# rojas-diego/tokengeex

Hardware: AMD Instinct MI355X
Metric: MB/s raw bytes encoded (and tokens/s) at 32K/64K vocab, 1/2/4/8 GPUs (higher is better)
Workload: dtype f64

## Files before the change

tokengeex_amd/_lib.py:

```python
from __future__ import annotations

import ctypes as C
import os

import numpy as np

_HERE = os.path.dirname(os.path.abspath(__file__))
LIB_PATH = os.path.join(_HERE, "libtgx.so")

OK, ERR_IO, ERR_JSON, ERR_TOKEN_ID_OOB, ERR_NO_PATH, ERR_DEVICE, ERR_Z_NOT_NORMAL, ERR_INVALID, \
    ERR_UNSUPPORTED = range(9)
MAX_TOKEN_LEN = 64
MAX_NBEST = 16
ESTEP_SNIPPET_LEN = 81920
NO_ID = 0xFFFFFFFF
LAYOUT_PAD_LEFT, LAYOUT_TRUNC_LEFT, LAYOUT_I64 = 1, 2, 4
FRONT_CRLF = 1
SPAN_CHARS = 8
SELECT_ROWS_DEVICE = 1

_vp, _u64, _u32, _i, _d = C.c_void_p, C.c_uint64, C.c_uint32, C.c_int, C.c_double
_pvp, _pu64 = C.POINTER(C.c_void_p), C.POINTER(C.c_uint64)
SYMBOLS = {
    "tgx_last_error": (C.c_char_p, []),
# ... 40 lines not shown
    "tgx_count_pairs_top": (_i, [_vp, _vp, _u64, _pvp, _pvp, _pu64, _pu64]),
    "tgx_estep": (_i, [_vp, _vp, _u64, _d, _u64, _vp, C.POINTER(C.c_double)]),
    "tgx_split_specials": (_i, [_vp, _vp, _u64, _vp, _vp, _u32, _vp, _pvp, _pvp, _pvp, _pu64]),
    "tgx_pack_segments": (_i, [_vp, _vp, _vp, _vp, _u64, _i, _vp, _vp, _pu64]),
    "tgx_normalize_segments": (_i, [_u32, _vp, _vp, _vp, _u64, _pvp, _pvp]),
    "tgx_unidata_version": (C.c_char_p, []),
    "tgx_assemble_ids": (_i, [_vp, _vp, _u64, _vp, _vp, _u32, _vp, _vp]),
    "tgx_decode_batch": (_i, [_vp, _vp, _u32, _vp, _vp, _u32, _vp, _vp, _u64, _i, _pvp, _vp, _pu64, _pu64]),
    "tgx_utf8_lossy": (_u64, [_vp, _u64, _vp]),
    "tgx_substring_df": (_i, [_i, _vp, _u64, _vp, _vp, _vp, _vp, _u64, _u32, _d, _u64, _pvp, _pvp, _pvp, _pu64, _pu64, _pu64]),
    "tgx_substring_df_top": (_i, [_i, _vp, _u64, _vp, _vp, _vp, _vp, _u64, _u32, _d, _u64, _u64, _pvp, _pvp, _pvp, _pu64, _pu64, _pu64,
                                  _pu64, C.POINTER(C.c_uint32)]),
    "tgx_generate_u01": (_d, [_u64, _u64, _u64]),
    "tgx_free": (None, [_vp]),
    "tgx_pool_trim": (None, [_i]),
    "tgx_pool_filled_bytes": (_u64, []),
    "tgx_host_alloc": (_vp, [_u64]),
    "tgx_host_free": (None, [_vp]),
    "tgx_digamma": (_d, [_d]),
    "tgx_prune_m_step": (_i, [_vp, _vp, _u32, _vp, _vp, C.POINTER(C.c_uint32)]),
    "tgx_prune_alternatives": (_i, [_vp, _vp, _vp, _vp, _u32, _vp, _vp, _pvp]),
    "tgx_model_prune_alternatives": (_i, [_vp, _vp, _vp, _pvp]),
    "tgx_prune_select": (_i, [_vp, _vp, _vp, _vp, _vp, _vp, _u32, _u64, _u32, _vp, C.POINTER(C.c_uint32)]),
    "tgx_last_kernel_times": (_i, [_vp, C.POINTER(C.c_char_p), C.POINTER(C.c_float), _i]),
    "tgx_last_algorithmic_bytes": (_u64, [_vp]),
    "tgx_last_encode_waves_per_cu": (_u32, [_vp]),
    "tgx_last_encode_redo_samples": (_u64, [_vp]),
    "tgx_model_score_values": (_u32, [_vp]),
    "tgx_last_encode_hot_values": (_u32, [_vp]),
    "tgx_last_encode_lean_items": (_u32, [_vp]),
    "tgx_last_encode_ids_in_place": (_i, [_vp]),
    "tgx_last_encode_top_table": (_i, [_vp]),
    "tgx_last_encode_long_samples": (_u64, [_vp]),
    "tgx_last_estep_pieces": (_u64, [_vp]),
    "tgx_last_estep_redo": (_u64, [_vp]),
    "tgx_last_encode_corun_cus": (_u32, [_vp]),
    "tgx_encode_corun_timeouts": (_u32, [_vp]),
    "tgx_sample_u01": (_d, [_u64, _u64, _u64, _u32]),
    "tgx_encode_batch_sample": (_i, [_vp, _vp, _vp, _u64, _d, _u64, _vp, _pvp]),
    "tgx_encode_corpus_sample": (_i, [_vp, _vp, _d, _u64, _vp, _pvp]),
    "tgx_lattice_stats_corpus": (_i, [_vp, _vp, _d, _vp, _vp, _vp, _pu64]),
    "tgx_lattice_stats_batch": (_i, [_vp, _vp, _vp, _u64, _d, _vp, _vp, _vp, _pu64]),
    "tgx_lattice_stats_host": (_i, [_vp, _vp, _vp, _u32, _vp, _vp, _u64, _d, _vp, _vp, _vp, _pu64]),
    "tgx_encode_batch_nbest": (_i, [_vp, _vp, _vp, _u64, _u32, _vp, _vp, _pvp]),
    "tgx_encode_corpus_nbest": (_i, [_vp, _vp, _u32, _vp, _vp, _pvp]),
    "tgx_result_device": (_i, [_vp]),
    "tgx_result_layout_info": (_i, [_vp, _u32, _u32, _pu64, _pu64]),
    "tgx_result_pad_device": (_i, [_vp, _u32, _u32, _u32, _u32, _u32, _vp, _vp, _vp, _vp, _pu64]),
    "tgx_result_pack_device": (_i, [_vp, _u32, _u32, _u32, _u32, _u32, _vp, _vp, _vp, _vp, _pu64]),
    "tgx_layout_pad_host": (_i, [_vp, _vp, _u64, _u32, _u32, _u32, _u32, _u32, _vp, _vp, _vp, _pu64]),
    "tgx_layout_pack_host": (_i, [_vp, _vp, _u64, _u32, _u32, _u32, _u32, _u32, _vp, _vp, _vp, _pu64]),
    "tgx_assemble_result": (_i, [_vp, _vp, _vp, _vp, _u64, _u32, _pvp]),
    "tgx_result_vocab_size": (_u32, [_vp]),
    "tgx_assemble_host": (_i, [_vp, _vp, _u64, _vp, _vp, _u64, _u32, _u32, _vp, _u64, _vp]),
    "tgx_decode_result": (_i, [_vp, _vp, _vp, _vp, _u32, _i, _vp, _pvp, _pu64, _pu64]),
    "tgx_decode_padded": (_i, [_vp, _vp, _u64, _u64, _u32, _vp, _vp, _u32, _vp, _vp, _u32, _i, _vp, _pvp, _pu64, _pu64]),
    "tgx_text_num_rows": (_u64, [_vp]),
    "tgx_text_num_bytes": (_u64, [_vp]),
    "tgx_text_num_replaced": (_u64, [_vp]),
    "tgx_text_device": (_i, [_vp]),
    "tgx_text_copy_bytes": (_i, [_vp, _vp, _u64]),
    "tgx_text_copy_offsets": (_i, [_vp, _vp, _u64]),
    "tgx_text_bytes_device": (_vp, [_vp]),
    "tgx_text_offsets_device": (_vp, [_vp]),
    "tgx_text_free": (None, [_vp]),
    "tgx_corpus_from_text": (_i, [_vp, _pvp]),
    "tgx_decode_rows_host": (_i, [_vp, _vp, _u32, _vp, _vp, _u32, _vp, _u32, _vp, _u64, _u64, _vp, _vp, _u32, _i, _pvp, _vp, _pu64,
                                  _pu64, _pu64]),
    "tgx_result_spans_device": (_i, [_vp, _vp, _vp, _vp, _u32, _u32, _vp, _vp]),
    "tgx_result_pad_spans_device": (_i, [_vp, _vp, _vp, _vp, _u32, _u32, _u32, _u32, _u32, _vp, _vp]),
    "tgx_spans_host": (_i, [_vp, _vp, _u32, _vp, _vp, _u32, _vp, _vp, _u64, _u32, _u32, _u32, _u32, _vp]),
    "tgx_result_window_info": (_i, [_vp, _u32, _u32, _u32, _u32, _u32, _pu64]),
    "tgx_result_window_pad_device": (_i, [_vp, _u32, _u32, _u32, _u32, _u32, _u32, _vp, _u64, _vp, _vp, _vp, _vp, _vp]),
    "tgx_result_window_spans_device": (_i, [_vp, _vp, _vp, _vp, _u32, _u32, _u32, _u32, _u32, _u32, _vp, _u64, _vp]),
    "tgx_layout_windows_host": (_i, [_vp, _vp, _u64, _u32, _u32, _u32, _u32, _u32, _u32, _u64, _vp, _vp, _vp, _vp, _vp, _pu64]),
    "tgx_window_spans_host": (_i, [_vp, _vp, _u32, _vp, _vp, _u32, _vp, _vp, _u64, _u32, _u32, _u32, _u32, _u32, _u64, _vp, _pu64]),
    "tgx_corpus_split_specials": (_i, [_vp, _vp, _vp, _u32, _u32, _pvp, _pvp]),
    "tgx_plan_num_samples": (_u64, [_vp]),
    "tgx_plan_num_segments": (_u64, [_vp]),
    "tgx_plan_num_encoded": (_u64, [_vp]),
    "tgx_plan_device": (_i, [_vp]),
    "tgx_plan_copy": (_i, [_vp, _vp, _u64, _vp, _u64]),
    "tgx_plan_free": (None, [_vp]),
    "tgx_assemble_result_plan": (_i, [_vp, _vp, _vp, _u32, _pvp]),
    "tgx_front_last_times": (_i, [C.POINTER(C.c_char_p), C.POINTER(C.c_float), _i]),
    "tgx_corpus_copy_text": (_i, [_vp, _vp, _u64]),
    "tgx_corpus_copy_offsets": (_i, [_vp, _vp, _u64]),
    "tgx_front_host": (_i, [_vp, _vp, _u64, _vp, _vp, _u32, _u32, _vp, _pvp, _pu64, _pvp, _pvp, _pu64]),
    "tgx_corpus_normalize": (_i, [_vp, _u32, _pvp, _pu64]),
    "tgx_normalize_host": (_i, [_u32, _vp, _vp, _u64, _pvp, _pvp, _pu64]),
    "tgx_norm_last_times": (_i, [C.POINTER(C.c_char_p), C.POINTER(C.c_float), _i]),
    "tgx_fim_u01": (_d, [_u64, _u64, _u64]),
    "tgx_result_fim": (_i, [_vp, _u32, _u32, _u32, _d, _d, _u64, _u64, _vp, _vp, _vp, _pu64, _pvp]),
    "tgx_fim_host": (_i, [_vp, _vp, _u64, _u32, _u32, _u32, _u32, _d, _d, _u64, _u64, _vp, _u64, _vp, _vp, _vp, _pu64]),
    "tgx_result_from_ids": (_i, [_i, _vp, _vp, _u64, _u32, _pvp]),
    "tgx_fim_last_times": (_i, [C.POINTER(C.c_char_p), C.POINTER(C.c_float), _i]),
    "tgx_select_last_times": (_i, [C.POINTER(C.c_char_p), C.POINTER(C.c_float), _i]),
    "tgx_result_select": (_i, [_vp, _vp, _u64, _u32, _vp, _pvp]),
    "tgx_result_lengths_device": (_i, [_vp, _vp, _vp]),
    "tgx_corpus_select": (_i, [_vp, _vp, _u64, _u32, _vp, _pvp]),
    "tgx_shuffle_key": (_u64, [_u64, _u64]),
    "tgx_shuffled_rows_device": (_i, [_i, _u64, _u64, _vp, _vp]),
    "tgx_shuffled_rows_host": (_i, [_u64, _u64, _vp]),
    "tgx_select_host": (_i, [_vp, _vp, _u64, _vp, _u64, _vp, _u64, _vp]),
    "tgx_select_text_host": (_i, [_vp, _vp, _u64, _vp, _u64, _vp, _u64, _vp]),
    "tgx_corpus_first_equal_device": (_i, [_vp, _u32, _vp, _vp, C.POINTER(C.c_uint64)]),
    "tgx_result_first_equal_device": (_i, [_vp, _u32, _vp, _vp, C.POINTER(C.c_uint64)]),
    "tgx_row_hash": (_u64, [_vp, _u64, _u64]),
    "tgx_corpus_row_hashes_device": (_i, [_vp, _u64, _vp, _vp]),
    "tgx_result_row_hashes_device": (_i, [_vp, _u64, _vp, _vp]),
    "tgx_first_equal_host": (_i, [_vp, _u32, _vp, _u64, _u32, _vp, C.POINTER(C.c_uint64), C.POINTER(C.c_uint32)]),
    "tgx_dedup_last_times": (_i, [C.POINTER(C.c_char_p), C.POINTER(C.c_float), _i]),
    "tgx_dedup_last_rounds": (_u32, []),
    "tgx_result_minhash_device": (_i, [_vp, _u32, _u32, _u64, _u32, _vp, _vp]),
    "tgx_corpus_minhash_device": (_i, [_vp, _u32, _u32, _u64, _u32, _vp, _vp]),
    "tgx_minhash_value": (_u32, [_u64, _u32, _u64]),
    "tgx_minhash_bands_device": (_i, [_i, _vp, _u64, _u32, _u32, _u64, _vp, _vp, _vp]),
    "tgx_minhash_near_first_device": (_i, [_i, _vp, _u64, _u32, _vp, _u32, _u32, _vp, _vp, C.POINTER(C.c_uint64)]),
    "tgx_minhash_host": (_i, [_vp, _u32, _vp, _u64, _u32, _u32, _u64, _vp]),
    "tgx_minhash_bands_host": (_i, [_vp, _u64, _u32, _u32, _u64, _vp, _vp]),
    "tgx_minhash_near_first_host": (_i, [_vp, _u64, _u32, _vp, _u32, _u32, _vp, C.POINTER(C.c_uint64)]),
    "tgx_minhash_last_times": (_i, [C.POINTER(C.c_char_p), C.POINTER(C.c_float), _i]),
    "tgx_gram_key": (_u64, [_vp, _u64, _u64]),
    "tgx_result_gramset_create": (_i, [_vp, _u32, _u64, _u32, _vp, _vp]),
    "tgx_corpus_gramset_create": (_i, [_vp, _u32, _u64, _u32, _vp, _vp]),
    "tgx_gramset_create_from_keys": (_i, [_i, _vp, _u64, _u32, _u32, _u64, _vp]),
    "tgx_gramset_size": (_u64, [_vp]),
    "tgx_gramset_info": (_i, [_vp, C.POINTER(C.c_uint32), C.POINTER(C.c_uint32), C.POINTER(C.c_uint64), C.POINTER(C.c_int), C.POINTER(C.c_uint32)]),
    "tgx_gramset_keys": (_i, [_vp, _vp]),
    "tgx_gramset_free": (None, [_vp]),
    "tgx_result_gram_hits_device": (_i, [_vp, _vp, _u32, _vp, _vp, _vp]),
    "tgx_corpus_gram_hits_device": (_i, [_vp, _vp, _u32, _vp, _vp, _vp]),
    "tgx_gram_keys_host": (_i, [_vp, _u32, _vp, _u64, _u32, _u64, _vp, C.POINTER(C.c_uint64)]),
    "tgx_gram_hits_host": (_i, [_vp, _u32, _vp, _u64, _u32, _u64, _vp, _u64, _vp, _vp]),
    "tgx_gram_contains_host": (_i, [_vp, _u64, _vp, _u64, _vp]),
    "tgx_gram_last_times": (_i, [C.POINTER(C.c_char_p), C.POINTER(C.c_float), _i]),
    "tgx_corpus_text_stats_device": (_i, [_vp, _u64, _u32, _vp, _vp, _vp]),
    "tgx_corpus_lines": (_i, [_vp, _u32, _vp, _vp]),
    "tgx_text_stats_host": (_i, [_vp, _vp, _u64, _u64, _u32, _vp, _vp]),
    "tgx_lines_host": (_i, [_vp, _vp, _u64, _vp, _u64, C.POINTER(C.c_uint64)]),
    "tgx_textstat_last_times": (_i, [C.POINTER(C.c_char_p), C.POINTER(C.c_float), _i]),
    "tgx_result_repeat_stats_device": (_i, [_vp, _u32, _u64, _u32, _vp, _vp, _vp]),
    "tgx_corpus_repeat_stats_device": (_i, [_vp, _u32, _u64, _u32, _vp, _vp, _vp]),
    "tgx_repeat_stats_host": (_i, [_vp, _u32, _vp, _u64, _u32, _u64, _vp, _vp]),
    "tgx_repeat_last_times": (_i, [C.POINTER(C.c_char_p), C.POINTER(C.c_float), _i]),
}

WORD_SYMBOLS = {
    "tgx_corpus_word_stats_device": (_i, [_vp, _u64, _vp, _vp, _u32, _u32, _vp, _vp, _vp]),
    "tgx_word_stats_host": (_i, [_vp, _vp, _u64, _u64, _vp, _vp, _u32, _u32, _vp, _vp]),
    "tgx_wordstat_last_times": (_i, [C.POINTER(C.c_char_p), C.POINTER(C.c_float), _i]),
}

PHRASE_SYMBOLS = {
    "tgx_phraseset_create": (_i, [_i, _vp, _vp, _u32, _u32, _u32, _vp]),
    "tgx_phraseset_info": (_i, [_vp, C.POINTER(C.c_uint32), C.POINTER(C.c_uint32), C.POINTER(C.c_uint32), C.POINTER(C.c_uint32),
                                C.POINTER(C.c_uint32), C.POINTER(C.c_int), C.POINTER(C.c_uint64)]),
    "tgx_phraseset_free": (None, [_vp]),
    "tgx_corpus_phrase_hits_device": (_i, [_vp, _vp, _u32, _vp, _vp, _vp, _vp]),
    "tgx_result_phrase_hits_device": (_i, [_vp, _vp, _u32, _vp, _vp, _vp, _vp]),
    "tgx_phrase_hits_host": (_i, [_vp, _u32, _vp, _u64, _vp, _vp, _u32, _u32, _vp, _vp, _vp]),
    "tgx_phrase_last_times": (_i, [C.POINTER(C.c_char_p), C.POINTER(C.c_float), _i]),
}


class TokenGeeXError(Exception):

    def __init__(self, message: str, status: int = -1, sample: int | None = None,
                 pos: int | None = None, length: int | None = None):
        super().__init__(message)
        self.status, self.sample, self.pos, self.length = status, sample, pos, length


def _share_torch_hip_runtime() -> None:
    import sys
    if os.environ.get("TGX_HIP_RUNTIME", "") == "system" or "torch" in sys.modules:
        return
    import importlib.util
    try:
        spec = importlib.util.find_spec("torch")
    except (ImportError, ValueError):
        return
    for root in (spec.submodule_search_locations or []) if spec else []:
        path = os.path.join(root, "lib", "libamdhip64.so")
        if os.path.exists(path):
            try:
                C.CDLL(path, mode=C.RTLD_GLOBAL)
            except OSError:
                pass
            return


def _load() -> C.CDLL:
    if not os.path.exists(LIB_PATH):
        raise ImportError(
            f"{LIB_PATH} is missing: the HIP extension is mandatory (no CPU fallback). "
            "Build it with `python tokengeex_amd/build.py`.")
    _share_torch_hip_runtime()
    lib = C.CDLL(LIB_PATH)
    for name, (res, args) in list(SYMBOLS.items()) + list(WORD_SYMBOLS.items()) + list(PHRASE_SYMBOLS.items()):
        fn = getattr(lib, name)
        fn.restype = res
        fn.argtypes = args
    if lib.tgx_abi_version() != 1:
        raise ImportError("libtgx.so ABI version mismatch")
    return lib


lib = _load()


def check(status: int) -> None:
    if status == OK:
        return
    msg = (lib.tgx_last_error() or b"").decode("utf-8", "replace")
    if status in (ERR_NO_PATH, ERR_Z_NOT_NORMAL):
        s, p, l = C.c_uint64(), C.c_uint64(), C.c_uint64()
        lib.tgx_last_error_detail(C.byref(s), C.byref(p), C.byref(l))
        raise TokenGeeXError(msg, status, s.value, p.value, l.value)
    raise TokenGeeXError(msg, status)


class _PinnedBlock:

    def __init__(self, nbytes: int):
        self.nbytes = int(nbytes)
        self.addr = lib.tgx_host_alloc(self.nbytes)
        if not self.addr:
            raise TokenGeeXError(lib.tgx_last_error().decode("utf-8", "replace"))
        self.buf = (C.c_ubyte * max(1, self.nbytes)).from_address(self.addr)

    def __del__(self):
        addr, self.addr = getattr(self, "addr", None), None
        if addr:
            lib.tgx_host_free(addr)


def pinned_empty(shape, dtype) -> np.ndarray:
    dt = np.dtype(dtype)
    n = int(np.prod(shape))
    blk = _PinnedBlock(n * dt.itemsize)
    arr = np.frombuffer(blk.buf, dtype=dt, count=n).reshape(shape)
    blk.buf._tgx_owner = blk
    return arr


def pool_trim(device: int = -1) -> None:
    lib.tgx_pool_trim(device)


def pool_filled_bytes() -> int:
    return int(lib.tgx_pool_filled_bytes())


def device_count() -> int:
    return lib.tgx_device_count()


def ptr(a: np.ndarray | None):
    return None if a is None else a.ctypes.data_as(C.c_void_p)


class Packed:

    __slots__ = ("flat", "offs")

    def __init__(self, flat: np.ndarray, offs: np.ndarray):
        self.flat, self.offs = flat, offs

    @classmethod
    def of(cls, items) -> "Packed":
        return items if isinstance(items, Packed) else cls(*pack(items))

    def __len__(self) -> int:
        return int(self.offs.shape[0]) - 1

    def take(self, idx) -> "Packed":
        idx = np.asarray(idx, dtype=np.int64)
        beg, end = self.offs[:-1][idx].astype(np.int64), self.offs[1:][idx].astype(np.int64)
        lens = end - beg
        offs = np.zeros(idx.shape[0] + 1, np.uint64)
        np.cumsum(lens, out=offs[1:])
        total = int(offs[-1])
        src = np.repeat(beg - offs[:-1].astype(np.int64), lens) + np.arange(total, dtype=np.int64)
        return Packed(self.flat[src] if total else np.zeros(0, np.uint8), offs)

    def tolist(self) -> list[bytes]:
        raw, o = self.flat.tobytes(), self.offs.tolist()
        return [raw[o[i]:o[i + 1]] for i in range(len(o) - 1)]


def pack(items) -> tuple[np.ndarray, np.ndarray]:
    if isinstance(items, Packed):
        return items.flat, items.offs
    offs = np.zeros(len(items) + 1, dtype=np.uint64)
    if len(items):
        np.cumsum(np.fromiter((len(t) for t in items), dtype=np.uint64, count=len(items)), out=offs[1:])
    flat = np.frombuffer(b"".join(items), dtype=np.uint8)
    return flat, offs


def _take(ptr_, n, ctype, dtype):
    if not ptr_ or n == 0:
        if ptr_:
            lib.tgx_free(ptr_)
        return np.zeros(0, dtype)
    a = np.ctypeslib.as_array(C.cast(ptr_, C.POINTER(ctype)), shape=(n,)).copy()
    lib.tgx_free(ptr_)
    return a


def split_specials_flat(flat: np.ndarray, offs: np.ndarray, specials: list[bytes]):
    sflat, soffs = pack(specials)
    n = offs.shape[0] - 1
    seg_offs = np.zeros(n + 1, np.uint64)
    sb, se, ss, m = C.c_void_p(), C.c_void_p(), C.c_void_p(), C.c_uint64()
    check(lib.tgx_split_specials(ptr(flat) if flat.size else None, ptr(offs), n, ptr(sflat) if sflat.size else None, ptr(soffs),
                                 len(specials), ptr(seg_offs), C.byref(sb), C.byref(se), C.byref(ss), C.byref(m)))
    k = m.value
    return seg_offs, _take(sb, k, C.c_uint64, np.uint64), _take(se, k, C.c_uint64, np.uint64), _take(ss, k, C.c_int32, np.int32)


def pack_segments(flat: np.ndarray, seg_begin: np.ndarray, seg_end: np.ndarray, seg_special, crlf: bool):
    n = seg_begin.shape[0]
    total = int((seg_end.astype(np.int64) - seg_begin.astype(np.int64)).sum()) if n else 0
    out = np.empty(max(total, 1), np.uint8)
    out_offs = np.zeros(n + 1, np.uint64)
    m = C.c_uint64()
    check(lib.tgx_pack_segments(ptr(flat) if flat.size else None, ptr(seg_begin), ptr(seg_end),
                                None if seg_special is None else ptr(seg_special), n, 1 if crlf else 0, ptr(out), ptr(out_offs),
                                C.byref(m)))
    out_offs = out_offs[: m.value + 1]
    return out[: int(out_offs[-1])], out_offs


NORMAL_FORMS = {"nfd": 0, "nfc": 1, "nfkd": 2, "nfkc": 3}


def normalize_flat(form: str, flat: np.ndarray, offs: np.ndarray):
    flat = np.ascontiguousarray(flat, dtype=np.uint8)
    offs = np.ascontiguousarray(offs, dtype=np.uint64)
    n = offs.shape[0] - 1
    beg, end = np.ascontiguousarray(offs[:-1]), np.ascontiguousarray(offs[1:])
    ot, oo = C.c_void_p(), C.c_void_p()
    check(lib.tgx_normalize_segments(NORMAL_FORMS[form], ptr(flat) if flat.size else None, ptr(beg) if n else None, ptr(end) if n else None, n,
                                     C.byref(ot), C.byref(oo)))
    out_offs = _take(oo, n + 1, C.c_uint64, np.uint64)
    return _take(ot, int(out_offs[-1]), C.c_uint8, np.uint8), out_offs


def unidata_version() -> str:
    return lib.tgx_unidata_version().decode()

# ... 1392 lines not shown

    def assemble_plan(self, segs: "NativeResult | None", plan: NativePlan, n_specials: int) -> NativeResult:
        h = C.c_void_p()
        check(lib.tgx_assemble_result_plan(self._h, None if segs is None else segs._h, plan._h, _u32_arg(n_specials, "n_specials"), C.byref(h)))
        return NativeResult(h)

    @staticmethod
    def _specials(special_flat, special_offs):
        sf = np.ascontiguousarray(special_flat, dtype=np.uint8)
        so = np.ascontiguousarray(special_offs, dtype=np.uint64)
        return sf, so, so.shape[0] - 1

    def decode_result(self, result: NativeResult, special_flat, special_offs, include_special: bool, stream: int = 0) -> "NativeText":
        sf, so, n = self._specials(special_flat, special_offs)
        h, bs, bi = C.c_void_p(), C.c_uint64(), C.c_uint64()
        st = lib.tgx_decode_result(self._h, result._h, ptr(sf) if sf.size else None, ptr(so), n, 1 if include_special else 0,
                                   stream or None, C.byref(h), C.byref(bs), C.byref(bi))
        if st != OK:
            _raise_decode(st, bs.value, bi.value)
        return NativeText(h)

    def decode_padded(self, ids_ptr: int, n_rows: int, row_len: int, i64: bool, *, mask_ptr: int = 0, lengths_ptr: int = 0,
                      skip_id: int | None = None, special_flat=(), special_offs=(0,), include_special: bool = True,
                      stream: int = 0) -> "NativeText":
        sf, so, n = self._specials(special_flat, special_offs)
        h, bs, bi = C.c_void_p(), C.c_uint64(), C.c_uint64()
        st = lib.tgx_decode_padded(self._h, ids_ptr or None, int(n_rows), int(row_len), LAYOUT_I64 if i64 else 0, mask_ptr or None,
                                   lengths_ptr or None, _id_or_none(skip_id), ptr(sf) if sf.size else None, ptr(so), n,
                                   1 if include_special else 0, stream or None, C.byref(h), C.byref(bs), C.byref(bi))
        if st != OK:
            _raise_decode(st, bs.value, bi.value)
        return NativeText(h)

    def result_spans(self, result: NativeResult, special_flat, special_offs, spans_ptr: int, *, flags: int = 0, stream: int = 0) -> None:
        sf, so, n = self._specials(special_flat, special_offs)
        check(lib.tgx_result_spans_device(self._h, result._h, ptr(sf) if sf.size else None, ptr(so), n, _u32_arg(flags, "flags"),
                                          stream or None, spans_ptr or None))

    def result_pad_spans(self, result: NativeResult, special_flat, special_offs, row_len: int, spans_ptr: int, *, bos_id: int | None = None,
                         eos_id: int | None = None, flags: int = 0, stream: int = 0) -> None:
        sf, so, n = self._specials(special_flat, special_offs)
        check(lib.tgx_result_pad_spans_device(self._h, result._h, ptr(sf) if sf.size else None, ptr(so), n, _u32_arg(row_len, "row_len"),
                                              _id_or_none(bos_id), _id_or_none(eos_id), _u32_arg(flags, "flags"), stream or None,
                                              spans_ptr or None))

    def encode_corpus_sample(self, corpus: NativeCorpus, alpha: float, seed: int, return_logz: bool = False):
        n = corpus.num_samples
        logz = np.zeros(max(n, 1), np.float64) if return_logz else None
        h = C.c_void_p()
        check(lib.tgx_encode_corpus_sample(self._h, corpus._h, float(alpha), seed & (2**64 - 1),
                                           ptr(logz) if return_logz else None, C.byref(h)))
        return (NativeResult(h), logz[:n]) if return_logz else NativeResult(h)

    def encode_batch_nbest_flat(self, flat: np.ndarray, offs: np.ndarray, nbest: int):
        flat = np.ascontiguousarray(flat, dtype=np.uint8)
        offs = np.ascontiguousarray(offs, dtype=np.uint64)
        n = offs.shape[0] - 1
        scores = np.empty(max(n * int(nbest), 1), np.float64)
        n_found = np.empty(max(n, 1), np.uint32)
        h = C.c_void_p()
        check(lib.tgx_encode_batch_nbest(self._h, ptr(flat) if flat.size else None, ptr(offs), n, int(nbest), ptr(scores),
                                         ptr(n_found), C.byref(h)))
        return NativeResult(h), scores[:n * int(nbest)], n_found[:n]

    def encode_corpus_nbest(self, corpus: NativeCorpus, nbest: int):
        n = corpus.num_samples
        scores = np.empty(max(n * int(nbest), 1), np.float64)
        n_found = np.empty(max(n, 1), np.uint32)
        h = C.c_void_p()
        check(lib.tgx_encode_corpus_nbest(self._h, corpus._h, int(nbest), ptr(scores), ptr(n_found), C.byref(h)))
        return NativeResult(h), scores[:n * int(nbest)], n_found[:n]

    def count_tokens(self, corpus: NativeCorpus, freq: np.ndarray | None = None) -> np.ndarray:
        if freq is None:
            freq = np.zeros(self.vocab_size, np.uint64)
        assert freq.dtype == np.uint64 and freq.shape[0] == self.vocab_size and freq.flags.c_contiguous
        check(lib.tgx_count_tokens(self._h, corpus._h, ptr(freq)))
        return freq

    def count_pairs(self, corpus: NativeCorpus) -> tuple[np.ndarray, np.ndarray]:
        keys, counts, n = C.c_void_p(), C.c_void_p(), C.c_uint64()
        check(lib.tgx_count_pairs(self._h, corpus._h, C.byref(keys), C.byref(counts), C.byref(n)))
        k = n.value
        ka = np.ctypeslib.as_array(C.cast(keys, C.POINTER(C.c_uint64)), shape=(max(k, 1),))[:k].copy()
        ca = np.ctypeslib.as_array(C.cast(counts, C.POINTER(C.c_uint64)), shape=(max(k, 1),))[:k].copy()
        lib.tgx_free(keys)
        lib.tgx_free(counts)
        return ka, ca

    def count_pairs_top(self, corpus: NativeCorpus, max_pairs: int) -> tuple[np.ndarray, np.ndarray, int]:
        keys, counts, n, tot = C.c_void_p(), C.c_void_p(), C.c_uint64(), C.c_uint64()
        check(lib.tgx_count_pairs_top(self._h, corpus._h, int(max_pairs), C.byref(keys), C.byref(counts),
                                      C.byref(n), C.byref(tot)))
        k = n.value
        ka = np.ctypeslib.as_array(C.cast(keys, C.POINTER(C.c_uint64)), shape=(max(k, 1),))[:k].copy()
        ca = np.ctypeslib.as_array(C.cast(counts, C.POINTER(C.c_uint64)), shape=(max(k, 1),))[:k].copy()
        lib.tgx_free(keys)
        lib.tgx_free(counts)
        return ka, ca, tot.value

    def estep(self, corpus: NativeCorpus, snippet_len: int = ESTEP_SNIPPET_LEN, dropout: float = 0.0,
              seed: int = 0, expected: np.ndarray | None = None) -> tuple[np.ndarray, float]:
        if expected is None:
            expected = np.zeros(self.vocab_size, np.float64)
        assert expected.dtype == np.float64 and expected.shape[0] == self.vocab_size
        z = C.c_double()
        check(lib.tgx_estep(self._h, corpus._h, snippet_len, float(dropout), seed & (2**64 - 1),
                            ptr(expected), C.byref(z)))
        return expected, z.value

    def common_prefix_search(self, s: bytes) -> list[tuple[int, int]]:
        buf = np.frombuffer(s, dtype=np.uint8)
        cap = len(s) + 1
        ids, lens = np.zeros(cap, np.uint32), np.zeros(cap, np.uint32)
        cnt = C.c_uint64()
        check(lib.tgx_common_prefix_search(self._h, ptr(buf) if len(s) else None, len(s), ptr(ids),
                                           ptr(lens), cap, C.byref(cnt)))
        return [(int(ids[i]), int(lens[i])) for i in range(cnt.value)]

    def last_kernel_times(self) -> dict[str, float]:
        names = (C.c_char_p * 8)()
        ms = (C.c_float * 8)()
        n = lib.tgx_last_kernel_times(self._h, names, ms, 8)
        return {names[i].decode(): float(ms[i]) for i in range(n)}

    def last_algorithmic_bytes(self) -> int:
        return lib.tgx_last_algorithmic_bytes(self._h)

    def last_encode_waves_per_cu(self) -> int:
        return lib.tgx_last_encode_waves_per_cu(self._h)

    def last_encode_redo_samples(self) -> int:
        return lib.tgx_last_encode_redo_samples(self._h)

    def score_values(self) -> int:
        return lib.tgx_model_score_values(self._h)

    def last_encode_hot_values(self) -> int:
        return lib.tgx_last_encode_hot_values(self._h)

    def last_encode_lean_items(self) -> tuple[int, int]:
        v = lib.tgx_last_encode_lean_items(self._h)
        return v & 0xFF, (v >> 8) & 0xFF

    def last_encode_lean_step(self) -> bool:
        return bool(self.last_encode_lean_items()[0] & 1)

    def last_encode_ids_in_place(self) -> bool:
        return bool(lib.tgx_last_encode_ids_in_place(self._h))

    def last_encode_top_table(self) -> bool:
        return bool(lib.tgx_last_encode_top_table(self._h))

    def last_encode_long_samples(self) -> int:
        return lib.tgx_last_encode_long_samples(self._h)

    def last_estep_pieces(self) -> int:
        return lib.tgx_last_estep_pieces(self._h)

    def last_estep_redo(self) -> int:
        return lib.tgx_last_estep_redo(self._h)

    def last_encode_corun_cus(self) -> int:
        return lib.tgx_last_encode_corun_cus(self._h)

    def encode_corun_timeouts(self) -> int:
        return lib.tgx_encode_corun_timeouts(self._h)


class FlatTrie:

    def __init__(self, tokens: list[bytes], scores):
        flat, offs = pack(tokens)
        sc = np.ascontiguousarray(scores, dtype=np.float64)
        h = C.c_void_p()
        check(lib.tgx_flat_trie_build(ptr(flat) if flat.size else None, ptr(offs), ptr(sc), len(tokens),
                                      C.byref(h)))
        self._h = h
        self._flat, self._offs, self._sc = flat, offs, sc

    def common_prefix_search8(self, s: bytes, max_hot: int = 6600):
        buf = np.frombuffer(s, dtype=np.uint8)
        cap = len(s) + 1
        ids, lens = np.zeros(cap, np.uint32), np.zeros(cap, np.uint32)
        nh, nc, cov = C.c_uint32(), C.c_uint64(), C.c_double()
        k = lib.tgx_flat_trie_search8(self._h, ptr(self._flat) if self._flat.size else None, ptr(self._offs), ptr(self._sc),
                                      max_hot, ptr(buf) if len(s) else None, len(s), ptr(ids), ptr(lens), cap,
                                      C.byref(nh), C.byref(nc), C.byref(cov))
        if k == 2**64 - 1:
            raise TokenGeeXError("8-byte records need fewer than 2^23 slots")
        return [(int(ids[i]), int(lens[i])) for i in range(k)], {"n_hot": nh.value, "n_cold": nc.value, "hot_coverage": cov.value}

    def __del__(self):
        if getattr(self, "_h", None):
            lib.tgx_flat_trie_free(self._h)
            self._h = None

    def common_prefix_search(self, s: bytes) -> list[tuple[int, int]]:
        buf = np.frombuffer(s, dtype=np.uint8)
        cap = len(s) + 1
        ids, lens = np.zeros(cap, np.uint32), np.zeros(cap, np.uint32)
        k = lib.tgx_flat_trie_search(self._h, ptr(buf) if len(s) else None, len(s), ptr(ids), ptr(lens), cap)
        return [(int(ids[i]), int(lens[i])) for i in range(k)]

    def stats(self) -> dict:
        a, b, c = C.c_uint64(), C.c_uint64(), C.c_uint32()
        lib.tgx_flat_trie_stats(self._h, C.byref(a), C.byref(b), C.byref(c))
        return {"n_slots": a.value, "n_nodes": b.value, "max_token_len": c.value,
                "fill": b.value / max(1, a.value)}

    @property
    def max_token_len(self) -> int:
        return self.stats()["max_token_len"]

    def table(self):
        n = self.stats()["n_slots"]
        check, base, tokid = np.zeros(n, np.uint32), np.zeros(n, np.uint32), np.zeros(n, np.uint32)
        lib.tgx_flat_trie_copy(self._h, ptr(check), ptr(base), ptr(tokid))
        return check, base, tokid


    def prune_alternatives(self, tokens: list[bytes], scores) -> tuple[np.ndarray, np.ndarray, np.ndarray]:
        flat, offs = pack(tokens)
        sc = np.ascontiguousarray(scores, dtype=np.float64)
        V = len(tokens)
        always_keep = np.zeros(V, np.uint8)
        alt_offs = np.zeros(V + 1, np.uint32)
        p = C.c_void_p()
        check(lib.tgx_prune_alternatives(self._h, ptr(flat) if flat.size else None, ptr(offs), ptr(sc), V,
                                         ptr(always_keep), ptr(alt_offs), C.byref(p)))
        k = int(alt_offs[V])
        ids = np.ctypeslib.as_array(C.cast(p, C.POINTER(C.c_uint32)), shape=(max(k, 1),))[:k].copy()
        lib.tgx_free(p)
        return always_keep, alt_offs, ids


def tok_hash_selftest(tokens: list[bytes]) -> tuple[int, int]:
    flat, offs = pack(tokens)
    seed, bad = C.c_uint32(), C.c_uint64()
    check(lib.tgx_tok_hash_selftest(ptr(flat) if flat.size else None, ptr(offs), len(tokens), C.byref(seed), C.byref(bad)))
    return seed.value, bad.value


def digamma(x: float) -> float:
    return lib.tgx_digamma(x)


def prune_m_step(expected: np.ndarray, keep: np.ndarray) -> tuple[np.ndarray, np.ndarray]:
    expected = np.ascontiguousarray(expected, dtype=np.float64)
    keep = np.ascontiguousarray(keep, dtype=np.uint8)
    V = expected.shape[0]
    idx, sc, n = np.zeros(max(V, 1), np.uint32), np.zeros(max(V, 1), np.float64), C.c_uint32()
    check(lib.tgx_prune_m_step(ptr(expected), ptr(keep), V, ptr(idx), ptr(sc), C.byref(n)))
    return idx[:n.value].copy(), sc[:n.value].copy()


def prune_select(freq, keep, always_keep, alt_offs, alt_ids, scores, n_samples: int,
                 pruned_size: int) -> np.ndarray:
    freq = np.ascontiguousarray(freq, dtype=np.uint64)
    keep = np.ascontiguousarray(keep, dtype=np.uint8)
    always_keep = np.ascontiguousarray(always_keep, dtype=np.uint8)
    alt_offs = np.ascontiguousarray(alt_offs, dtype=np.uint32)
    alt_ids = np.ascontiguousarray(alt_ids, dtype=np.uint32)
    scores = np.ascontiguousarray(scores, dtype=np.float64)
    V = freq.shape[0]
    out, n = np.zeros(max(V, 1), np.uint32), C.c_uint32()
    check(lib.tgx_prune_select(ptr(freq), ptr(keep), ptr(always_keep), ptr(alt_offs),
                               ptr(alt_ids) if alt_ids.size else None, ptr(scores), V, n_samples,
                               pruned_size, ptr(out), C.byref(n)))
    return out[:n.value].copy()


def dropout_u01(seed: int, sample: int, pos: int, length: int) -> float:
    return lib.tgx_dropout_u01_host(seed, sample, pos, length)


def sample_u01(seed: int, sample: int, pos: int, length: int) -> float:
    return lib.tgx_sample_u01(seed, sample, pos, length)


def sample_u01_array(seed: int, sample: np.ndarray, pos: np.ndarray, length: np.ndarray) -> np.ndarray:
    with np.errstate(over="ignore"):
        x = (np.uint64(seed & (2**64 - 1)) ^ np.uint64(0xD6E8FEB86659FD93)
             ^ (np.asarray(sample, np.uint64) * np.uint64(0x9E3779B97F4A7C15))
             ^ (np.asarray(pos, np.uint64) * np.uint64(0xC2B2AE3D27D4EB4F))
             ^ (np.asarray(length, np.uint64) * np.uint64(0x165667B19E3779F9)))
        x ^= x >> np.uint64(30)
        x *= np.uint64(0xBF58476D1CE4E5B9)
        x ^= x >> np.uint64(27)
        x *= np.uint64(0x94D049BB133111EB)
        x ^= x >> np.uint64(31)
    u = ((x >> np.uint64(11)).astype(np.float64) + 0.5) * (1.0 / 9007199254740992.0)
    return np.minimum(u, np.nextafter(1.0, 0.0))
```

tokengeex_amd/build.py:

```python
from __future__ import annotations

import os
import shutil
import subprocess
import sys

HERE = os.path.dirname(os.path.abspath(__file__))
CSRC = os.path.join(HERE, "csrc")
OUT = os.path.join(HERE, "libtgx.so")
SOURCES = ["kernels.hip", "estep.hip", "encode2.hip", "encode4l.hip", "encode5.hip", "estep4.hip", "estep4l.hip", "estep7.hip", "cuts.hip", "pairs.hip", "generate.hip", "sample.hip", "stats.hip", "nbest.hip", "layout.hip", "assemble.hip", "fim.hip", "select.hip", "dedup.hip", "minhash.hip", "gram.hip", "repeat.hip", "textstat.hip", "wordstat.hip", "phrase.hip", "decode.hip", "spans.hip", "front.hip", "norm.hip", "tgx_api.cpp", "encode_pass.cpp", "estep_pass.cpp", "lattice_pass.cpp", "result_ops.cpp", "corpus_ops.cpp", "minhash_ops.cpp", "gram_ops.cpp", "repeat_ops.cpp", "textstat_ops.cpp", "wordstat_ops.cpp", "phrase_ops.cpp", "host_twins.cpp", "trie_build.cpp", "prune_host.cpp", "frontback.cpp", "unicode_norm.cpp"]
HEADERS = ["api_internal.h", "device_internal.h", "pass_internal.h", "kernels.h", "sample.h", "stats.h", "nbest.h", "layout.h", "assemble.h", "fim.h", "select.h", "dedup.h", "minhash.h", "gram.h", "gram_walk.h", "repeat.h", "shingle_load.h", "textstat.h", "textstat_walk.h", "wordstat.h", "phrase.h", "decode.h", "spans.h", "front.h", "norm.h", "device_common.h", "lattice_walk.h", "tile_fill.h", "scan_helpers.h", "lean_gate.h", "ids_in_place.h", "encode_split.h", "encode5_layout.h", "top_table.h", "trace_body.h", "trie_build.h", "unicode_tables.h", os.path.join("..", "..", "include", "tgx.h"), os.path.join("..", "..", "include", "tgx_words.h"), os.path.join("..", "..", "include", "tgx_phrases.h")]
ARCH = "gfx950"


def _hipcc() -> str:
    for cand in (os.environ.get("HIPCC"), shutil.which("hipcc"), "/opt/rocm/bin/hipcc"):
        if cand and os.path.exists(cand):
            return cand
    raise RuntimeError("hipcc not found")


def needs_build() -> bool:
    if not os.path.exists(OUT):
        return True
    t = os.path.getmtime(OUT)
    deps = [os.path.join(CSRC, f) for f in SOURCES + HEADERS] + [os.path.abspath(__file__)]
    return any(os.path.getmtime(d) > t for d in deps)


SYNTH_OUT = os.path.join(HERE, "libtgx_synth.so")


def build_synth(force: bool = False) -> str:
    src = os.path.join(CSRC, "synth_gen.c")
    if not force and os.path.exists(SYNTH_OUT) and os.path.getmtime(SYNTH_OUT) >= os.path.getmtime(src):
        return SYNTH_OUT
    subprocess.check_call(["gcc", "-O2", "-std=c11", "-fPIC", "-shared", "-o", SYNTH_OUT + ".tmp", src, "-lm"])
    os.replace(SYNTH_OUT + ".tmp", SYNTH_OUT)
    return SYNTH_OUT


FAST_OUT = os.path.join(HERE, "_tgxfast.so")


def build_pyfast(force: bool = False) -> str:
    import sysconfig
    src = os.path.join(CSRC, "pyfast.c")
    if not force and os.path.exists(FAST_OUT) and os.path.getmtime(FAST_OUT) >= os.path.getmtime(src):
        return FAST_OUT
    inc = sysconfig.get_paths()["include"]
    subprocess.check_call(["gcc", "-O2", "-std=c11", "-fPIC", "-shared", "-pthread", "-I", inc, "-o", FAST_OUT + ".tmp", src])
    os.replace(FAST_OUT + ".tmp", FAST_OUT)
    return FAST_OUT


def build(force: bool = False, verbose: bool = False) -> str:
    from concurrent.futures import ThreadPoolExecutor
    build_synth(force)
    build_pyfast(force)
    if not force and not needs_build():
        return OUT
    objdir = os.path.join(CSRC, "build")
    os.makedirs(objdir, exist_ok=True)
    hdr_time = max(os.path.getmtime(os.path.join(CSRC, h)) for h in HEADERS)
    hdr_time = max(hdr_time, os.path.getmtime(os.path.abspath(__file__)))
    flags = [f"--offload-arch={ARCH}", "-O3", "-std=c++17", "-fPIC",
             "-ffp-contract=off",
             "-munsafe-fp-atomics",
             "-Wall", "-Wno-unused-result", "-Wno-pass-failed", "-x", "hip"]
    flags += os.environ.get("TGX_EXTRA_HIPCC_FLAGS", "").split()
    jobs = []
    objs = []
    for s in SOURCES:
        src = os.path.join(CSRC, s)
        obj = os.path.join(objdir, s + ".o")
        objs.append(obj)
        if force or not os.path.exists(obj) or os.path.getmtime(obj) < max(os.path.getmtime(src), hdr_time):
            jobs.append([_hipcc()] + flags + ["-c", src, "-o", obj])

    def run(cmd):
        if verbose:
            print(" ".join(cmd), flush=True)
        subprocess.check_call(cmd)

    with ThreadPoolExecutor(max_workers=min(6, max(1, len(jobs)))) as ex:
        list(ex.map(run, jobs))
    link = [_hipcc(), f"--offload-arch={ARCH}", "-shared", "-fPIC"] + objs + ["-o", OUT + ".tmp", "-Wl,-rpath,/opt/rocm/lib"]
    if verbose:
        print(" ".join(link), flush=True)
    subprocess.check_call(link)
    os.replace(OUT + ".tmp", OUT)
    return OUT


if __name__ == "__main__":
    print(build(force="--force" in sys.argv, verbose=True))
```

tokengeex_amd/csrc/device_internal.h:

```cpp
#pragma once

#include <hip/hip_runtime.h>

#include <cstddef>
#include <cstdint>
#include <memory>
#include <mutex>
#include <vector>

#include "../../include/tgx.h"
#include "api_internal.h"
#include "trie_build.h"

#define HIP_TRY(expr)                                                                   \
    do {                                                                                  \
        hipError_t _e = (expr);                                                           \
        if (_e != hipSuccess)                                                             \
            return fail(TGX_ERR_DEVICE, "HIP error %d (%s) at %s:%d: %s", (int)_e,        \
                        hipGetErrorString(_e), __FILE__, __LINE__, #expr);                \
    } while (0)

namespace tgx {
struct DedupRows;
}

namespace tgx::dev {

hipError_t pool_alloc(int device, size_t bytes, void** out);
void pool_free(int device, void* ptr, size_t bytes);
void pool_trim(int device);
size_t rounded(size_t bytes);
hipError_t pool_fill(int device, void* p, size_t bytes);

template <class T>
class PoolBuf {
public:
    PoolBuf() = default;
    PoolBuf(const PoolBuf&) = delete;
    PoolBuf& operator=(const PoolBuf&) = delete;
    PoolBuf(PoolBuf&& o) noexcept : device_(o.device_), ptr_(o.ptr_), bytes_(o.bytes_) { o.ptr_ = nullptr; }
    PoolBuf& operator=(PoolBuf&& o) noexcept {
        if (this != &o) {
            reset();
            device_ = o.device_;
            ptr_ = o.ptr_;
            bytes_ = o.bytes_;
            o.ptr_ = nullptr;
        }
        return *this;
    }
    ~PoolBuf() { reset(); }

    hipError_t alloc(int device, size_t bytes) {
        reset();
        void* p = nullptr;
        const hipError_t e = pool_alloc(device, bytes, &p);
        if (e != hipSuccess) return e;
        device_ = device;
        ptr_ = static_cast<T*>(p);
        bytes_ = rounded(bytes);
        return hipSuccess;
    }
    void reset() {
        if (ptr_) pool_free(device_, ptr_, bytes_);
        ptr_ = nullptr;
    }
    T* get() const { return ptr_; }
    operator T*() const { return ptr_; }

private:
    int device_ = 0;
    T* ptr_ = nullptr;
    size_t bytes_ = 0;
};

struct KernelTime {
    const char* name;
    hipEvent_t start, stop;
    bool used;
};
constexpr int kMaxTimed = 8;

struct DeviceCtrl {
    unsigned long long queue;
    unsigned long long err;
    unsigned long long queue6;
    struct Estep {
        unsigned long long queue;
        unsigned long long redo_count;
        unsigned long long queue_bwd;
        unsigned long long range_flag;
    } estep;
    unsigned long long encode_redo;
    unsigned long long longest;
    unsigned long long err_piece;
};
static_assert(offsetof(DeviceCtrl::Estep, redo_count) == 8 && offsetof(DeviceCtrl::Estep, queue_bwd) == 16 &&
                  offsetof(DeviceCtrl::Estep, range_flag) == 24 && sizeof(DeviceCtrl::Estep) == 32,
              "the E-step words are cleared by one memset");
struct HostCtrl {
    unsigned long long err;
    unsigned long long total_tokens;
};

}

using tgx::dev::DeviceCtrl;
using tgx::dev::HostCtrl;
using tgx::dev::KernelTime;
using tgx::dev::kMaxTimed;
using tgx::dev::PoolBuf;

struct tgx_model {
    int device = 0;
    uint32_t vocab_size = 0;
    uint32_t lm = 0;
    bool scores_finite = true;
    tgx::FlatTrie flat;
    void* d_trie = nullptr;
    uint32_t* d_tokid = nullptr;
    DeviceCtrl* d_ctrl = nullptr;
    HostCtrl* h_ctrl = nullptr;
    hipStream_t stream = nullptr;
    hipStream_t stream2 = nullptr;
    hipEvent_t ev_fork = nullptr, ev_join = nullptr;
    unsigned int* h_started = nullptr;
    int num_cus = 0;
    int blocks_per_cu = 0;
    std::vector<uint8_t> vocab_bytes;
    std::vector<uint64_t> vocab_offs;
    std::vector<double> vocab_scores;
    tgx::FlatTrie flat_rev;
    void* d_trie_rev = nullptr;
    bool rev_host_built = false;
    void* d_trie_w = nullptr;
    void* d_trie_rev_w = nullptr;
    uint64_t last_long_samples = 0;
    uint64_t last_estep_pieces = 0;
    uint32_t last_corun_cus = 0;
    double e7_overflow_share = 0.0;
    bool values_ranked = false;
    uint32_t corun_wait_timeouts = 0;
    uint64_t last_redo_samples = 0;
    int last_encode_waves_per_cu = 0;
    bool estep_linear_ok = false;
    tgx::TokHashTable tokhash;
    void* d_tokhash = nullptr;
    void* d_trie8 = nullptr;
    void* d_top8 = nullptr;
    bool last_encode_top = false;
    double* d_values = nullptr;
    std::vector<double> value_coverage;
    uint32_t n_values = 0, root_base8 = 0;
    uint32_t last_n_hot = 0;
    bool lean_scores_ok = false;
    bool last_ids_in_place = false;
    uint32_t last_lean_items = 0;
    bool have_trie8 = false;
    bool encode_tables_ready = false;
    bool estep_trie8_tried = false;
    uint64_t estep_calls = 0;
    bool have_wvalues = false;
    double* d_wvalues = nullptr;
    bool tokhash_host_built = false;
    void* d_trie8t = nullptr;
    double* d_wtab = nullptr;
    std::vector<uint32_t> id_of_rank;
    uint32_t n_tok7 = 0, root_base7 = 0;
    bool trie8t_tried = false, have_trie8t = false;
    uint64_t last_estep_redo = 0;
    uint8_t* d_dec_len = nullptr;
    void* d_dec_slots = nullptr;
    uint8_t* d_dec_bytes = nullptr;
    uint64_t* d_dec_offs = nullptr;
    bool decode_tables_ready = false;
    uint16_t* d_span_words = nullptr;
    bool span_words_ready = false;
    int estep_blocks_per_cu = 0;
    KernelTime timed[kMaxTimed] = {};
    int n_timed = 0;
    uint64_t last_alg_bytes = 0;
    std::mutex mu;
};

struct tgx_corpus {
    int device = 0;
    uint64_t n_samples = 0, n_bytes = 0, max_len = 0;
    std::vector<uint64_t> h_offs;
    std::vector<uint32_t> h_sorted_len;
    std::vector<uint64_t> h_sorted_cum;
    PoolBuf<uint8_t> d_text_alloc;
    uint8_t* d_text = nullptr;
    PoolBuf<uint64_t> d_offs;
    PoolBuf<uint32_t> d_order;
    PoolBuf<uint32_t> d_bp, d_tmp, d_counts, d_status;
    PoolBuf<void> d_scan_tmp;
    size_t scan_tmp_bytes = 0;
    struct EstepWork {
        uint64_t snippet_len = 0;
        std::vector<uint64_t> soffs, sbase;
        std::vector<uint32_t> ssample, order;
        PoolBuf<uint64_t> d_soffs, d_sbase;
        PoolBuf<uint32_t> d_order, d_ssample;
        uint32_t window = 0;
        uint64_t n_windows = 0;
        PoolBuf<uint32_t> d_win_snip, d_win_k;
    } es;
    std::mutex mu;
};

struct tgx_result {
    int device = 0;
    uint32_t vocab_size = 0;
    uint64_t n_samples = 0, n_tokens = 0;
    PoolBuf<uint32_t> d_ids;
    PoolBuf<uint64_t> d_offs;
    std::unique_ptr<uint32_t[]> h_ids;
    std::vector<uint64_t> h_offs;
    bool have_ids = false, have_offs = false;
};

struct tgx_plan {
    int device = 0;
    uint64_t n_samples = 0, n_segs = 0, n_enc = 0;
    uint32_t n_specials = 0;
    PoolBuf<uint64_t> d_seg_offs;
    PoolBuf<int32_t> d_special;
};

struct tgx_text {
    int device = 0;
    uint64_t n_rows = 0, n_bytes = 0, n_replaced = 0;
    PoolBuf<uint8_t> d_bytes;
    PoolBuf<uint64_t> d_offs;
};

namespace tgx::dev {

tgx_status require_device(int* n_devices = nullptr);
void time_begin(tgx_model* m, const char* name);
void time_end(tgx_model* m);

class Pass {
public:
    explicit Pass(tgx_model* m) : m_(m) {}
    Pass(const Pass&) = delete;
    Pass& operator=(const Pass&) = delete;
    ~Pass() {
        if (ok_) return;
        (void)hipStreamSynchronize(m_->stream);
        if (m_->stream2) (void)hipStreamSynchronize(m_->stream2);
    }

    template <class T>
    hipError_t alloc(size_t bytes, T** out) {
        PoolBuf<void> b;
        const hipError_t e = b.alloc(m_->device, bytes);
        *out = static_cast<T*>(b.get());
        if (e == hipSuccess) scratch_.push_back(std::move(b));
        return e;
    }
    tgx_result* new_result(uint64_t n_samples) {
        result_.reset(new tgx_result());
        result_->device = m_->device;
        result_->vocab_size = m_->vocab_size;
        result_->n_samples = n_samples;
        return result_.get();
    }
    tgx_result* release_result() { return result_.release(); }
    void adopt_result(tgx_result* r) { result_.reset(r); }
    tgx_status done() {
        ok_ = true;
        return TGX_OK;
    }

private:
    tgx_model* m_;
    bool ok_ = false;
    std::vector<PoolBuf<void>> scratch_;
    std::unique_ptr<tgx_result> result_;
};

class DeviceScope {
public:
    DeviceScope() { (void)hipGetDevice(&prev_); }
    ~DeviceScope() {
        if (prev_ >= 0) (void)hipSetDevice(prev_);
    }
    DeviceScope(const DeviceScope&) = delete;
    DeviceScope& operator=(const DeviceScope&) = delete;

private:
    int prev_ = -1;
};

hipStream_t stream_or_default(void* stream, int device);
tgx_status check_device_ptr(const char* who, const char* what, const void* p, int device, const char* owner);

class StreamGuard {
public:
    StreamGuard(int device, hipStream_t stream) : device_(device), stream_(stream) {}
    StreamGuard(const StreamGuard&) = delete;
// ... 87 lines not shown
```

tokengeex_amd/csrc/encode5.hip:

```cpp
#include <hip/hip_runtime.h>
#include <stdint.h>

#include <type_traits>

#include "device_common.h"
#include "encode5_layout.h"
#include "kernels.h"

namespace tgx {


template <int PPL>
struct WalkCtx {
    __amdgpu_buffer_rsrc_t trie;
    uint32_t s, l32;
    double dropout;
    uint64_t seed;
    bool estep_rule = false;
};

struct Res5 {
    __amdgpu_buffer_rsrc_t cold;
    uint32_t tab;
    uint32_t shift, hot_max;
    uint32_t used_off;
    uint32_t first, cap;
    bool pend;
    uint32_t pend_addr;
    double pend_val;
    __device__ __forceinline__ void complete() {
        if (pend) {
            const uint32_t e = __hip_atomic_fetch_add((__attribute__((address_space(3))) uint32_t*)(uintptr_t)used_off, 1u, __ATOMIC_RELAXED, __HIP_MEMORY_SCOPE_WORKGROUP);
            if (e < cap) {
                lds_st<double>(tab + 8u * (first + e), pend_val);
                lds_st<uint16_t>(pend_addr, (uint16_t)(first + e));
            }
        }
        pend = false;
    }
};

template <bool DROPOUT, bool LONG, bool RES, int PPL, int D, bool SKIP = false, int CK = 0, bool PK = false, bool T0 = false>
struct Walk5 {
    static_assert(CK == 0 || (!DROPOUT && !LONG && !RES && PPL >= 2 && D < CK && CK < 16), "compaction: hot and COLD builds of two to four walks per lane");
    static_assert(!T0 || (D == 1 && !DROPOUT && !LONG && !RES && !PK), "top-table entries: the first level of the hot and COLD builds");
    static __device__ __forceinline__ void run(const WalkCtx<PPL>& W, Res5& R, const uint32_t (&bytes)[PPL][4], const uint32_t (&maxd)[PPL],
                                               const uint32_t (&pg)[PPL], const uint32_t (&wlane)[PPL], bool (&alive)[PPL],
                                               uint2 (&rec)[PPL], uint32_t (&c)[PPL]) {
        static_assert(!RES || PPL == 1, "resolving walks keep one pending value per lane");
        constexpr int d = D;
        constexpr bool CUT = CK != 0 && D + 1 == CK;
        uint32_t off_cut[PPL];
        bool any = false;
#pragma unroll
        for (int g = 0; g < PPL; ++g) {
            asm("" : "+v"(rec[g].x), "+v"(rec[g].y));
            if constexpr (T0) {
                const uint32_t rank0 = rec[g].y >> 16;
                if (alive[g] && rank0 != 0u) lds_st<uint16_t>(wlane[g] | W.l32, (uint16_t)rank0);
                alive[g] = alive[g] && 1u < maxd[g];
            }
            alive[g] = alive[g] && ((rec[g].x >> 24) == c[g]);
            const uint32_t rank = rec[g].y & 0xFFFFu;
            bool term = alive[g] && rank != 0u;
            if (DROPOUT) {
                if (term && d >= 1) {
                    const double u01 = dropout_u01(W.seed, W.s, pg[g], (uint32_t)d + 1u);
                    term = W.estep_rule ? !(u01 < W.dropout) : (W.dropout < u01);
                }
            }
            if (RES) {
                if (D > 0) R.complete();
                const uint32_t addr = wlane[g] | ((W.l32 + 32u * (uint32_t)d) & 0x1E0u);
                const uint32_t idx = rank + R.shift;
                if (term) lds_st<uint16_t>(addr, (uint16_t)idx);
                R.pend = term && idx > R.hot_max && R.cap != 0u;
                if (R.pend) {
                    R.pend_val = buf_ld_f64(R.cold, (idx - R.hot_max - 1u) << 3);
                    R.pend_addr = addr;
                }
            } else if (PK) {
                if (term) lds_st<uint16_t>(((wlane[g] + 32u * (uint32_t)d) & 0x1E0u) | (wlane[g] & ~0x1E0u), (uint16_t)rank);
            } else {
                if (term) lds_st<uint16_t>(wlane[g] | ((W.l32 + 32u * (uint32_t)d) & 0x1E0u), (uint16_t)rank);
            }
            if (D + 1 < 16) {
                constexpr int e = D + 1 < 16 ? D + 1 : 15;
                c[g] = (bytes[g][e >> 2] >> ((e & 3) * 8)) & 0xFFu;
                alive[g] = alive[g] && ((uint32_t)e < maxd[g]);
                const uint32_t off = (rec[g].x ^ (c[g] << 3)) & 0xFFFFFFu;
                if (CUT) {
                    off_cut[g] = off;
                } else if (SKIP && D >= 11) {
                    if (__builtin_amdgcn_ballot_w64(alive[g]) != 0) rec[g] = buf_ld8(W.trie, alive[g] ? off : 0u);
                } else {
                    rec[g] = buf_ld8(W.trie, alive[g] ? off : 0u);
                }
            } else if (!LONG) {
                alive[g] = false;
            }
            any = any || alive[g];
        }
        if (__builtin_amdgcn_ballot_w64(any) == 0) {
            if (RES) R.complete();
            return;
        }
        if constexpr (CUT) {
            uint64_t bm[PPL];
            uint32_t base[PPL], n_alive = 0;
#pragma unroll
            for (int g = 0; g < PPL; ++g) {
                bm[g] = __builtin_amdgcn_ballot_w64(alive[g]);
                base[g] = n_alive;
                n_alive += (uint32_t)__builtin_popcountll(bm[g]);
            }
            if (n_alive <= 64u) {
                pack<1>(W, R, bytes, maxd, wlane, alive, off_cut, bm, base, n_alive);
                return;
            }
            if (PPL >= 3 && n_alive <= 128u) {
                pack<(PPL >= 3 ? 2 : 1)>(W, R, bytes, maxd, wlane, alive, off_cut, bm, base, n_alive);
                return;
            }
#pragma unroll
            for (int g = 0; g < PPL; ++g) rec[g] = buf_ld8(W.trie, alive[g] ? off_cut[g] : 0u);
            Walk5<DROPOUT, LONG, RES, PPL, D + 1, SKIP, 0, PK>::run(W, R, bytes, maxd, pg, wlane, alive, rec, c);
        } else {
            Walk5<DROPOUT, LONG, RES, PPL, D + 1, SKIP, CK, PK>::run(W, R, bytes, maxd, pg, wlane, alive, rec, c);
        }
    }

    template <int P2>
    static __device__ __forceinline__ void pack(const WalkCtx<PPL>& W, Res5& R, const uint32_t (&bytes)[PPL][4], const uint32_t (&maxd)[PPL],
                                                const uint32_t (&wlane)[PPL], const bool (&alive)[PPL], const uint32_t (&off)[PPL],
                                                const uint64_t (&bm)[PPL], const uint32_t (&base)[PPL], uint32_t n_alive) {
        constexpr int Q0 = CK >> 2;
        constexpr int NW = 2 + 4 - Q0;
        const uint32_t lane = __builtin_amdgcn_mbcnt_hi(~0u, __builtin_amdgcn_mbcnt_lo(~0u, 0u));
        uint32_t v2[P2][NW];
#pragma unroll
        for (int t = 0; t < P2; ++t)
#pragma unroll
            for (int i = 0; i < NW; ++i) v2[t][i] = 0u;
#pragma unroll
        for (int g = 0; g < PPL; ++g) {
            const uint32_t cnt = (uint32_t)__builtin_popcountll(bm[g]);
            const uint32_t below = __builtin_amdgcn_mbcnt_hi((uint32_t)(bm[g] >> 32), __builtin_amdgcn_mbcnt_lo((uint32_t)bm[g], 0u));
            const uint32_t dst = (base[g] + (alive[g] ? below : cnt + lane - below)) & 63u;
            uint32_t v[NW];
            v[0] = off[g];
            v[1] = (PK ? wlane[g] : (wlane[g] | W.l32)) | (maxd[g] << 24);
#pragma unroll
            for (int q = Q0; q < 4; ++q) v[2 + q - Q0] = bytes[g][q];
            const uint32_t t = (lane - base[g]) & 63u;
            const bool got = t < cnt;
            const bool hi = base[g] + t >= 64u;
#pragma unroll
            for (int i = 0; i < NW; ++i) {
                const uint32_t x = (uint32_t)__builtin_amdgcn_ds_permute((int)(dst << 2), (int)v[i]);
#pragma unroll
                for (int s2 = 0; s2 < P2; ++s2)
                    if (got && (P2 == 1 || (s2 == 1) == hi)) v2[s2][i] = x;
            }
        }
        WalkCtx<P2> W2{W.trie, W.s, W.l32, W.dropout, W.seed, W.estep_rule};
        uint32_t bytes2[P2][4], maxd2[P2], pg2[P2], wl2[P2], c2[P2];
        bool alive2[P2];
        uint2 rec2[P2];
#pragma unroll
        for (int s2 = 0; s2 < P2; ++s2) {
            alive2[s2] = 64u * (uint32_t)s2 + lane < n_alive;
            wl2[s2] = v2[s2][1] & 0xFFFFFFu;
            maxd2[s2] = v2[s2][1] >> 24;
            pg2[s2] = 0u;
#pragma unroll
            for (int q = 0; q < 4; ++q) bytes2[s2][q] = q < Q0 ? 0u : v2[s2][2 + (q < Q0 ? 0 : q - Q0)];
            c2[s2] = (bytes2[s2][Q0] >> ((CK & 3) * 8)) & 0xFFu;
            rec2[s2] = buf_ld8(W.trie, alive2[s2] ? v2[s2][0] : 0u);
        }
        Walk5<DROPOUT, LONG, RES, P2, CK, SKIP, 0, true>::run(W2, R, bytes2, maxd2, pg2, wl2, alive2, rec2, c2);
    }
};
template <bool DROPOUT, bool LONG, bool RES, int PPL, bool SKIP, int CK, bool PK>
struct Walk5<DROPOUT, LONG, RES, PPL, 16, SKIP, CK, PK> {
    static __device__ __forceinline__ void run(const WalkCtx<PPL>&, Res5& R, const uint32_t (&)[PPL][4], const uint32_t (&)[PPL],
                                               const uint32_t (&)[PPL], const uint32_t (&)[PPL], bool (&)[PPL], uint2 (&)[PPL],
                                               uint32_t (&)[PPL]) {
        if (RES) R.complete();
    }
};

template <int N, int LN = 0>
__device__ __forceinline__ void e5_scores_issue(uint32_t tab, const uint32_t (&iw)[8], int first, u32x2_t (&sp)[N]) {
#pragma unroll
    for (int u = 0; u < N; ++u) {
        const int v = first + u;
        if constexpr ((LN & kLeanFetch) != 0) {
            sp[u] = lds_ld<u32x2_t>((v & 1) ? word_times8<1>(iw[v >> 1]) : word_times8<0>(iw[v >> 1]));
        } else {
            const uint32_t a = (v & 1) ? ((iw[v >> 1] >> 16) << 3) : ((iw[v >> 1] & 0xFFFFu) << 3);
            sp[u] = lds_ld<u32x2_t>(tab + a);
        }
    }
}
__device__ __forceinline__ double e5_score_value(const u32x2_t& p) { return __hiloint2double((int)p.y, (int)p.x); }

template <int N, int LN = 0>
__device__ __forceinline__ void e5_scores_cold(uint32_t tab, __amdgpu_buffer_rsrc_t cold, const uint32_t (&iw)[8], int first,
                                               uint32_t hot_bytes, double (&sv)[N]) {
    uint32_t a[N];
#pragma unroll
    for (int u = 0; u < N; ++u) {
        const int v = first + u;
        if constexpr ((LN & kLeanFetch) != 0) {
            a[u] = (v & 1) ? word_times8<1>(iw[v >> 1]) : word_times8<0>(iw[v >> 1]);
            sv[u] = lds_ld<double>(a[u] < hot_bytes ? a[u] : 0u);
        } else {
            a[u] = (v & 1) ? ((iw[v >> 1] >> 16) << 3) : ((iw[v >> 1] & 0xFFFFu) << 3);
            sv[u] = lds_ld<double>(tab + (a[u] < hot_bytes ? a[u] : 0u));
        }
    }
    static_assert(N == 4 || N == 8, "e5_scores_cold: four or eight values at a time");
    if (N == 8) asm volatile("" : "+v"(sv[0]), "+v"(sv[1]), "+v"(sv[2]), "+v"(sv[3]), "+v"(sv[4 % N]), "+v"(sv[5 % N]), "+v"(sv[6 % N]), "+v"(sv[7 % N]));
    else asm volatile("" : "+v"(sv[0]), "+v"(sv[1]), "+v"(sv[2]), "+v"(sv[3]));
#pragma unroll
    for (int u = 0; u < N; ++u)
        if (a[u] >= hot_bytes) sv[u] = buf_ld_f64(cold, a[u] - hot_bytes);
}

template <bool COLD>
__device__ __forceinline__ double e5_score_one(uint32_t tab, __amdgpu_buffer_rsrc_t cold, uint32_t rank, uint32_t hot_bytes) {
    const uint32_t a = rank << 3;
    double v = lds_ld<double>(tab + ((!COLD || a < hot_bytes) ? a : 0u));
    if (COLD) {
        asm volatile("" : "+v"(v));
        if (a >= hot_bytes) v = buf_ld_f64(cold, a - hot_bytes);
    }
    return v;
}

constexpr uint32_t kFarCode = 0x80u;

__device__ __forceinline__ uint32_t e5_winner_len_m1(uint32_t code, uint32_t l) {
    return (code & kFarCode) ? (code & 31u) : ((l - code - 1u) & 15u);
}

template <int U>
__device__ __forceinline__ void relax5l_step(double sv, double& acc, uint32_t& bpv, double& far, uint32_t& fbp, uint32_t& fin, double& fval) {
    constexpr uint64_t MU = kRowLane0 << U;
    fin = sel_u32(MU, bpv, fin);
    fval = sel_f64(MU, acc, fval);
    const double best = row_bcast_f64<U>(acc);
    const double cur = sel_f64(MU, far, acc);
    const uint32_t curbp = sel_u32(MU, fbp, bpv);
    far = sel_f64(MU, -__builtin_huge_val(), far);
    const double cand = best + sv;
    const uint64_t take = __builtin_amdgcn_fcmp(cand, cur, 2 );
    asm("v_max_f64 %0, %1, %2" : "=v"(acc) : "v"(cur), "v"(cand));
    bpv = sel_imm_u32<U>(take, curbp);
}

template <bool DROPOUT>
__device__ __forceinline__ void e5_long_tail(__amdgpu_buffer_rsrc_t trie, const uint8_t* __restrict__ text16, uint32_t rec_x, bool alive,
                                             uint32_t maxd, uint32_t lane, uint32_t g, uint32_t list_off, double dropout, uint64_t seed,
                                             uint32_t s, uint32_t pg) {
    bool more = alive && maxd > 16u;
    if (__builtin_amdgcn_ballot_w64(more) == 0) return;
    struct __attribute__((packed, aligned(1))) Bytes16 { uint32_t w[4]; };
    Bytes16 b{{0u, 0u, 0u, 0u}};
    if (more) b = *reinterpret_cast<const Bytes16*>(text16);
    uint32_t x = rec_x;
#pragma unroll 1
    for (uint32_t d = 16u; d < 32u; ++d) {
        more = more && d < maxd;
        if (__builtin_amdgcn_ballot_w64(more) == 0) break;
        const uint32_t bi = d - 16u;
        const uint32_t word = (bi & 8u) ? ((bi & 4u) ? b.w[3] : b.w[2]) : ((bi & 4u) ? b.w[1] : b.w[0]);
        const uint32_t c = (word >> ((bi & 3u) * 8u)) & 0xFFu;
        const uint2 rec = buf_ld8(trie, more ? ((x ^ (c << 3)) & 0xFFFFFFu) : 0u);
        more = more && (rec.x >> 24) == c;
        const uint32_t rank = rec.y & 0xFFFFu;
        bool term = more && rank != 0u;
        if (DROPOUT) {
            if (term) term = dropout < dropout_u01(seed, s, pg, d + 1u);
        }
        if (term) {
            const uint32_t slot = __hip_atomic_fetch_add((__attribute__((address_space(3))) uint32_t*)(uintptr_t)list_off, 1u, __ATOMIC_RELAXED, __HIP_MEMORY_SCOPE_WORKGROUP);
            if (slot < kE5LongCap) lds_st<uint32_t>(list_off + 8u + slot * 4u, lane | (g << 6) | (d << 8) | (rank << 16));
        }
        x = rec.x;
    }
}

#define E5_STAMP(i)                                                    \
    if (P.stamps) {                                                    \
        __builtin_amdgcn_sched_barrier(0);                             \
        const uint64_t _now = (uint64_t)__builtin_amdgcn_s_memtime(); \
        __builtin_amdgcn_s_waitcnt(0xC07F);                            \
        __builtin_amdgcn_sched_barrier(0);                             \
        seg[i] += _now - t_last;                                       \
        t_last = _now;                                                 \
    }

template <bool DROPOUT, bool COLD, int PPL, bool LONG, int CK = 0, int LN = 0, bool CNT = false, bool TOP = false>
__global__ __launch_bounds__(1024, (PPL == 1 ? 8 : (PPL == 2 ? 6 : (PPL == 3 ? 4 : 1)))) void encode5_kernel(EncodeParams P, Encode5Params Q) {
    static_assert(!LONG || PPL == 4, "the long-token build runs four positions per lane");
    static_assert((LN == 0 && !CNT && !TOP) || (!LONG && !DROPOUT), "the long-token and dropout builds keep the kernel as it was");
    extern __shared__ __align__(16) unsigned char smem[];
    constexpr uint32_t LM = LONG ? 32 : 16;
    constexpr uint32_t SPAN = 16u * PPL;
    const uint32_t lane = threadIdx.x & 63u;
    const uint32_t l = lane & 15u, r = lane >> 4;
    const uint32_t wave = threadIdx.x >> 6;
    const uint2* __restrict__ trie = reinterpret_cast<const uint2*>(Q.trie8);
    const __amdgpu_buffer_rsrc_t trie_b = make_rsrc(Q.trie8, Q.trie_bytes);
    const __amdgpu_buffer_rsrc_t top_b = make_rsrc(TOP ? Q.top : nullptr, TOP ? kE5TopBytes : 0u);
    const uint32_t lds0 = (uint32_t)reinterpret_cast<uintptr_t>(smem);
    double* const score_tab = reinterpret_cast<double*>(smem);
    const uint32_t hot_bytes = 8u * (Q.n_hot + 1u);
    const __amdgpu_buffer_rsrc_t values = make_rsrc(reinterpret_cast<const unsigned char*>(Q.values) + hot_bytes, 8u * (Q.n_values - Q.n_hot));
    const uint2* rootc = reinterpret_cast<const uint2*>(smem + Q.root_off);
    unsigned char* wbase = smem + Q.idx_off + (size_t)wave * (PPL * kE5GroupBytes);
    {
        for (uint32_t i = threadIdx.x; i <= Q.n_hot; i += blockDim.x) score_tab[i] = Q.values[i];
        if constexpr (!TOP) {
            uint2* rw = reinterpret_cast<uint2*>(smem + Q.root_off);
            for (uint32_t i = threadIdx.x; i < 256u; i += blockDim.x) rw[i] = trie[(Q.root_base & ~255u) + i];
        }
        if (Q.started && threadIdx.x == 0u) __hip_atomic_fetch_add(Q.started, 1u, __ATOMIC_RELAXED, __HIP_MEMORY_SCOPE_SYSTEM);
        __syncthreads();
    }
    const __amdgpu_buffer_rsrc_t cold_values = values;

    uint32_t s = 0, n = 0, p0 = 0;
    uint64_t beg = 0;
    bool live = false, need_new = true;
    const double ninf = -__builtin_huge_val();
    double acc = ninf, far = ninf;
    uint32_t bpv = kNoStep, fbp = kFarCode;
    bool redo = false;
    uint32_t wn[4 * PPL + 1];
    uint32_t pk = 0, pk_j = 0;
    bool pk_dirty = false;
#pragma unroll
    for (int q = 0; q <= 4 * PPL; ++q) wn[q] = 0;
    const uint32_t my_col = r * kE5RowStride + ((l - 1u) & 15u) * 32u;
    const uint32_t wbase_off = lds0 + Q.idx_off + wave * (PPL * kE5GroupBytes);
    const uint32_t wr_off = wbase_off + r * kE5RowStride + l * 2u;
    const uint32_t col_off = wbase_off + my_col;
    const uint32_t list_off = lds0 + Q.list_off + wave * ((kE5LongBytes + 15u) & ~15u);
    uint64_t seg[5] = {0, 0, 0, 0, 0};
    uint64_t t_last = P.stamps ? (uint64_t)__builtin_amdgcn_s_memtime() : 0;
    uint32_t iters = 0;

    uint64_t local_next = 0, local_end = 0;
    for (;;) {
        {
            uint64_t k = ~0ull;
            const bool have_local = need_new && local_next < local_end;
            if (have_local) k = local_next++;
            const uint64_t kc = claim_rows_chunk(P.queue, need_new && !have_local, r, Q.claim_chunk);
            if (need_new && !have_local) {
                k = kc;
                local_next = kc + 1u;
                local_end = kc + Q.claim_chunk;
            }
            if (need_new) {
                live = k < P.n_samples;
                if (live) {
                    s = P.order[k];
                    beg = P.offs[s];
                    n = (uint32_t)(P.offs[s + 1] - beg);
                }
            }
        }
        if (need_new) {
            p0 = 0;
            acc = (l == 0u) ? 0.0 : ninf;
            bpv = kNoStep;
            pk_dirty = false;
            if (LONG) {
                far = ninf;
                fbp = kFarCode;
                redo = false;
            }
        }
        const bool fresh_row = need_new;
        need_new = false;
        if (__builtin_amdgcn_ballot_w64(live) == 0) break;
        iters++;
        E5_STAMP(0)

        const uintptr_t addr = reinterpret_cast<uintptr_t>(P.text + (live ? beg + p0 + l : 0));
        const uint32_t sh = (uint32_t)(addr & 3u);
        const uint32_t* __restrict__ wp = reinterpret_cast<const uint32_t*>(addr & ~uintptr_t(3));
        uint32_t w[4 * PPL + 1];
        if (fresh_row) {
#pragma unroll
            for (int q = 0; q <= 4 * PPL; ++q) w[q] = wp[q];
        } else {
#pragma unroll
            for (int q = 0; q <= 4 * PPL; ++q) w[q] = wn[q];
        }
        uint32_t bytes[PPL][4];
#pragma unroll
        for (int g = 0; g < PPL; ++g)
#pragma unroll
            for (int q = 0; q < 4; ++q) bytes[g][q] = __builtin_amdgcn_alignbyte(w[4 * g + q + 1], w[4 * g + q], sh);
        uint2 top_rec[TOP ? PPL : 1];
        if constexpr (TOP) {
#pragma unroll
            for (int g = 0; g < PPL; ++g) top_rec[g] = buf_ld8(top_b, word_times8<0>(bytes[g][0]));
        }

#pragma unroll
        for (int g = 0; g < PPL; ++g) {
            uint4* mine = reinterpret_cast<uint4*>(wbase + g * kE5GroupBytes + my_col);
            mine[0] = make_uint4(0, 0, 0, 0);
            mine[1] = make_uint4(0, 0, 0, 0);
        }
        if (LONG && lane == 0u) lds_st<uint32_t>(list_off, 0u);
        __builtin_amdgcn_wave_barrier();
        E5_STAMP(1)

        uint32_t pg[PPL], maxd[PPL];
        uint32_t wlane[PPL];
        bool alive[PPL];
        uint2 rec[PPL];
        uint32_t c[PPL];
#pragma unroll
        for (int g = 0; g < PPL; ++g) {
            pg[g] = p0 + 16u * g + l;
            const uint32_t rem = (live && pg[g] < n) ? (n - pg[g]) : 0u;
            maxd[g] = rem < LM ? rem : LM;
            alive[g] = maxd[g] > 0 && !(P.flags & 1u);
            wlane[g] = wr_off + g * kE5GroupBytes;
            if constexpr (!TOP) {
                c[g] = bytes[g][0] & 0xFFu;
                rec[g] = rootc[(Q.root_base ^ c[g]) & 255u];
            }
        }
        {
            uint32_t l32 = l * 32u;
            asm volatile("" : "+v"(l32));
            WalkCtx<PPL> W{trie_b, s, l32, P.dropout, P.seed};
            Res5 no_res{};
            if constexpr (TOP) {
#pragma unroll
                for (int g = 0; g < PPL; ++g) {
                    rec[g] = top_rec[g];
                    c[g] = (bytes[g][0] >> 8) & 0xFFu;
                }
                Walk5<DROPOUT, LONG, false, PPL, 1, COLD && PPL < 4, CK, false, true>::run(W, no_res, bytes, maxd, pg, wlane, alive, rec, c);
            } else {
                Walk5<DROPOUT, LONG, false, PPL, 0, COLD && PPL < 4, CK>::run(W, no_res, bytes, maxd, pg, wlane, alive, rec, c);
            }
        }
        if (LONG) {
#pragma unroll
            for (int g = 0; g < PPL; ++g)
                e5_long_tail<DROPOUT>(trie_b, P.text + (live ? beg + pg[g] + 16u : 0), rec[g].x, alive[g], maxd[g], lane, (uint32_t)g, list_off,
                                      P.dropout, P.seed, s, pg[g]);
        }
        __builtin_amdgcn_wave_barrier();
        E5_STAMP(2)
        {
            const uint32_t* __restrict__ np = wp + 4 * PPL;
#pragma unroll
            for (int q = 0; q <= 4 * PPL; ++q) wn[q] = np[q];
        }

        if (!(P.flags & 32u)) __builtin_amdgcn_s_setprio(0);
        uint32_t fin[PPL];
        bool reached[PPL];
        if (!(P.flags & 2u)) {
            uint32_t iw[8], iwn[8];
            auto load_iw = [&](int g, uint32_t (&w)[8]) {
                const u32x4_t ia = lds_ld<u32x4_t>(col_off + g * kE5GroupBytes), ib = lds_ld<u32x4_t>(col_off + g * kE5GroupBytes + 16u);
                w[0] = ia.x; w[1] = ia.y; w[2] = ia.z; w[3] = ia.w;
                w[4] = ib.x; w[5] = ib.y; w[6] = ib.z; w[7] = ib.w;
            };
            u32x2_t sa[4], sb[4];
            load_iw(0, iw);
            if (!COLD) e5_scores_issue<4, LN>(lds0, iw, 0, sa);
            uint32_t end_groups = 0;
            if (LN & kLeanStep) {
                const uint32_t g_end = (live && n - p0 < SPAN) ? ((n - p0) >> 4) : 0xFFu;
#pragma unroll
                for (int g = 0; g < PPL; ++g) end_groups |= (__builtin_amdgcn_ballot_w64(g_end == (uint32_t)g) != 0 ? 1u : 0u) << g;
            }
#pragma unroll
            for (int g = 0; g < PPL; ++g) {
                uint32_t (&cw)[8] = (g & 1) ? iwn : iw;
                uint32_t (&nw)[8] = (g & 1) ? iw : iwn;
                fin[g] = kNoStep;
                uint32_t fhi = 0xFFF00000u;
                bool slow = false;
                uint32_t n_list = 0;
                if (LONG) {
                    n_list = (uint32_t)__builtin_amdgcn_readfirstlane((int)lds_ld<uint32_t>(list_off));
                    slow = n_list != 0u || __builtin_amdgcn_ballot_w64((uint32_t)((uint64_t)__double_as_longlong(far) >> 32) != 0xFFF00000u) != 0;
                }
                if (LONG && slow) {
                    auto rank_of = [&](int u) { return (u & 1) ? (cw[u >> 1] >> 16) : (cw[u >> 1] & 0xFFFFu); };
                    double fval = ninf;
                    relax5l_step<0>(e5_score_one<COLD>(lds0, cold_values, rank_of(0), hot_bytes), acc, bpv, far, fbp, fin[g], fval);
                    relax5l_step<1>(e5_score_one<COLD>(lds0, cold_values, rank_of(1), hot_bytes), acc, bpv, far, fbp, fin[g], fval);
                    relax5l_step<2>(e5_score_one<COLD>(lds0, cold_values, rank_of(2), hot_bytes), acc, bpv, far, fbp, fin[g], fval);
                    relax5l_step<3>(e5_score_one<COLD>(lds0, cold_values, rank_of(3), hot_bytes), acc, bpv, far, fbp, fin[g], fval);
                    relax5l_step<4>(e5_score_one<COLD>(lds0, cold_values, rank_of(4), hot_bytes), acc, bpv, far, fbp, fin[g], fval);
                    relax5l_step<5>(e5_score_one<COLD>(lds0, cold_values, rank_of(5), hot_bytes), acc, bpv, far, fbp, fin[g], fval);
                    relax5l_step<6>(e5_score_one<COLD>(lds0, cold_values, rank_of(6), hot_bytes), acc, bpv, far, fbp, fin[g], fval);
                    relax5l_step<7>(e5_score_one<COLD>(lds0, cold_values, rank_of(7), hot_bytes), acc, bpv, far, fbp, fin[g], fval);
                    relax5l_step<8>(e5_score_one<COLD>(lds0, cold_values, rank_of(8), hot_bytes), acc, bpv, far, fbp, fin[g], fval);
                    relax5l_step<9>(e5_score_one<COLD>(lds0, cold_values, rank_of(9), hot_bytes), acc, bpv, far, fbp, fin[g], fval);
                    relax5l_step<10>(e5_score_one<COLD>(lds0, cold_values, rank_of(10), hot_bytes), acc, bpv, far, fbp, fin[g], fval);
                    relax5l_step<11>(e5_score_one<COLD>(lds0, cold_values, rank_of(11), hot_bytes), acc, bpv, far, fbp, fin[g], fval);
                    relax5l_step<12>(e5_score_one<COLD>(lds0, cold_values, rank_of(12), hot_bytes), acc, bpv, far, fbp, fin[g], fval);
                    relax5l_step<13>(e5_score_one<COLD>(lds0, cold_values, rank_of(13), hot_bytes), acc, bpv, far, fbp, fin[g], fval);
                    relax5l_step<14>(e5_score_one<COLD>(lds0, cold_values, rank_of(14), hot_bytes), acc, bpv, far, fbp, fin[g], fval);
                    relax5l_step<15>(e5_score_one<COLD>(lds0, cold_values, rank_of(15), hot_bytes), acc, bpv, far, fbp, fin[g], fval);
                    const uint32_t cnt = n_list < kE5LongCap ? n_list : kE5LongCap;
#pragma unroll 1
                    for (uint32_t i = 0; i < cnt; ++i) {
                        const uint32_t e = (uint32_t)__builtin_amdgcn_readfirstlane((int)lds_ld<uint32_t>(list_off + 8u + i * 4u));
                        if (((e >> 6) & 3u) != (uint32_t)g) continue;
                        const uint32_t src = e & 63u, d = (e >> 8) & 31u;
                        const double score = e5_score_one<COLD>(lds0, cold_values, e >> 16, hot_bytes);
                        const double cand = readlane_f64(fval, src) + score;
                        const uint32_t tt = (src & 15u) + d + 1u;
                        const bool mine = (lane >> 4) == (src >> 4) && l == (tt & 15u);
                        const bool to_far = tt >= 32u;
                        const double curv = to_far ? far : acc;
                        const uint32_t curc = to_far ? fbp : bpv;
                        const bool longer = !(curc & kFarCode) || d > (curc & 31u);
                        const bool take = mine && (cand > curv || (cand == curv && longer));
                        if (take && to_far) {
                            far = cand;
                            fbp = kFarCode | d;
                        }
                        if (take && !to_far) {
                            acc = cand;
                            bpv = kFarCode | d;
                        }
                    }
                    reached[g] = fval > ninf;
                    if (g + 1 < PPL) {
                        load_iw(g + 1, nw);
                        if (!COLD) e5_scores_issue<4>(lds0, nw, 0, sa);
                    }
                    continue;
                }
                if constexpr (LN == 0 && !CNT) {
                    if (COLD) {
                        double sv[8], sw[8];
                        e5_scores_cold<8>(lds0, cold_values, cw, 0, hot_bytes, sv);
                        e5_scores_cold<8>(lds0, cold_values, cw, 8, hot_bytes, sw);
                        if (g + 1 < PPL) load_iw(g + 1, nw);
                        relax5_step<0>(sv[0], acc, bpv, fin[g], fhi);
                        relax5_step<1>(sv[1], acc, bpv, fin[g], fhi);
                        relax5_step<2>(sv[2], acc, bpv, fin[g], fhi);
                        relax5_step<3>(sv[3], acc, bpv, fin[g], fhi);
                        relax5_step<4>(sv[4], acc, bpv, fin[g], fhi);
                        relax5_step<5>(sv[5], acc, bpv, fin[g], fhi);
                        relax5_step<6>(sv[6], acc, bpv, fin[g], fhi);
                        relax5_step<7>(sv[7], acc, bpv, fin[g], fhi);
                        relax5_step<8>(sw[0], acc, bpv, fin[g], fhi);
                        relax5_step<9>(sw[1], acc, bpv, fin[g], fhi);
                        relax5_step<10>(sw[2], acc, bpv, fin[g], fhi);
                        relax5_step<11>(sw[3], acc, bpv, fin[g], fhi);
                        relax5_step<12>(sw[4], acc, bpv, fin[g], fhi);
                        relax5_step<13>(sw[5], acc, bpv, fin[g], fhi);
                        relax5_step<14>(sw[6], acc, bpv, fin[g], fhi);
                        relax5_step<15>(sw[7], acc, bpv, fin[g], fhi);
                    } else {
                        e5_scores_issue<4>(lds0, cw, 4, sb);
                        if (g + 1 < PPL) load_iw(g + 1, nw);
                        relax5_step<0>(e5_score_value(sa[0]), acc, bpv, fin[g], fhi);
                        relax5_step<1>(e5_score_value(sa[1]), acc, bpv, fin[g], fhi);
                        relax5_step<2>(e5_score_value(sa[2]), acc, bpv, fin[g], fhi);
                        relax5_step<3>(e5_score_value(sa[3]), acc, bpv, fin[g], fhi);
                        e5_scores_issue<4>(lds0, cw, 8, sa);
                        relax5_step<4>(e5_score_value(sb[0]), acc, bpv, fin[g], fhi);
                        relax5_step<5>(e5_score_value(sb[1]), acc, bpv, fin[g], fhi);
                        relax5_step<6>(e5_score_value(sb[2]), acc, bpv, fin[g], fhi);
                        relax5_step<7>(e5_score_value(sb[3]), acc, bpv, fin[g], fhi);
                        e5_scores_issue<4>(lds0, cw, 12, sb);
                        relax5_step<8>(e5_score_value(sa[0]), acc, bpv, fin[g], fhi);
                        relax5_step<9>(e5_score_value(sa[1]), acc, bpv, fin[g], fhi);
                        relax5_step<10>(e5_score_value(sa[2]), acc, bpv, fin[g], fhi);
                        relax5_step<11>(e5_score_value(sa[3]), acc, bpv, fin[g], fhi);
                        if (g + 1 < PPL) e5_scores_issue<4>(lds0, nw, 0, sa);
                        relax5_step<12>(e5_score_value(sb[0]), acc, bpv, fin[g], fhi);
                        relax5_step<13>(e5_score_value(sb[1]), acc, bpv, fin[g], fhi);
                        relax5_step<14>(e5_score_value(sb[2]), acc, bpv, fin[g], fhi);
                        relax5_step<15>(e5_score_value(sb[3]), acc, bpv, fin[g], fhi);
                    }
                    reached[g] = fhi != 0xFFF00000u;
                } else {
                    const bool full = !(LN & kLeanStep) || ((end_groups >> g) & 1u) != 0u;
#define E5_STEP(U, SV)                                                   \
        if (FULL) relax5_step<U, LN, CNT>(SV, acc, bpv, fin[g], fhi);         \
        else relax5_lean_step<U, LN, CNT>(SV, acc, bpv, fin[g]);
                    auto steps = [&](auto full_tag) {
                        constexpr bool FULL = decltype(full_tag)::value;
                        if (COLD) {
                            double sv[8], sw[8];
                            e5_scores_cold<8, LN>(lds0, cold_values, cw, 0, hot_bytes, sv);
                            e5_scores_cold<8, LN>(lds0, cold_values, cw, 8, hot_bytes, sw);
                            if (g + 1 < PPL) load_iw(g + 1, nw);
                            E5_STEP(0, sv[0]) E5_STEP(1, sv[1]) E5_STEP(2, sv[2]) E5_STEP(3, sv[3])
                            E5_STEP(4, sv[4]) E5_STEP(5, sv[5]) E5_STEP(6, sv[6]) E5_STEP(7, sv[7])
                            E5_STEP(8, sw[0]) E5_STEP(9, sw[1]) E5_STEP(10, sw[2]) E5_STEP(11, sw[3])
                            E5_STEP(12, sw[4]) E5_STEP(13, sw[5]) E5_STEP(14, sw[6]) E5_STEP(15, sw[7])
                        } else {
                            e5_scores_issue<4, LN>(lds0, cw, 4, sb);
                            if (g + 1 < PPL) load_iw(g + 1, nw);
                            E5_STEP(0, e5_score_value(sa[0])) E5_STEP(1, e5_score_value(sa[1]))
                            E5_STEP(2, e5_score_value(sa[2])) E5_STEP(3, e5_score_value(sa[3]))
                            e5_scores_issue<4, LN>(lds0, cw, 8, sa);
                            E5_STEP(4, e5_score_value(sb[0])) E5_STEP(5, e5_score_value(sb[1]))
                            E5_STEP(6, e5_score_value(sb[2])) E5_STEP(7, e5_score_value(sb[3]))
// ... 443 lines not shown

        uint32_t pg[PPL], pgh[PPL], maxd[PPL], wlane[PPL], c[PPL];
        bool alive[PPL];
        uint2 rec[PPL];
#pragma unroll
        for (int g = 0; g < PPL; ++g) {
            pg[g] = p0 + 16u * g + l;
            pgh[g] = (uint32_t)sbase + pg[g];
            const uint32_t rem = (live && pg[g] < n) ? (n - pg[g]) : 0u;
            maxd[g] = rem < LM ? rem : LM;
            alive[g] = maxd[g] > 0;
            wlane[g] = wr_off + g * kE5GroupBytes;
            c[g] = bytes[g][0] & 0xFFu;
            rec[g] = rootc[(Q.root_base ^ c[g]) & 255u];
        }
        {
            uint32_t l32 = l * 32u;
            asm volatile("" : "+v"(l32));
            WalkCtx<PPL> W{trie_b, smp, l32, P.dropout, P.seed, true};
            Res5 no_res{};
            Walk5<DROPOUT, false, false, PPL, 0>::run(W, no_res, bytes, maxd, pgh, wlane, alive, rec, c);
        }
        __builtin_amdgcn_wave_barrier();
        {
            const uint32_t* __restrict__ np = wp + 4 * PPL;
#pragma unroll
            for (int q = 0; q <= 4 * PPL; ++q) wn[q] = np[q];
        }

#pragma unroll
        for (int g = 0; g < PPL; ++g) {
            uint32_t iw[8];
            {
                const u32x4_t ia = lds_ld<u32x4_t>(col_off + g * kE5GroupBytes), ib = lds_ld<u32x4_t>(col_off + g * kE5GroupBytes + 16u);
                iw[0] = ia.x; iw[1] = ia.y; iw[2] = ia.z; iw[3] = ia.w;
                iw[4] = ib.x; iw[5] = ib.y; iw[6] = ib.z; iw[7] = ib.w;
            }
            double sv[8], sw[8];
            if (COLD) {
                e5_scores_cold<8>(lds0, cold_values, iw, 0, hot_bytes, sv);
                e5_scores_cold<8>(lds0, cold_values, iw, 8, hot_bytes, sw);
            } else {
                u32x2_t sa[8], sb[8];
                e5_scores_issue<8>(lds0, iw, 0, sa);
                e5_scores_issue<8>(lds0, iw, 8, sb);
#pragma unroll
                for (int u = 0; u < 8; ++u) {
                    sv[u] = e5_score_value(sa[u]);
                    sw[u] = e5_score_value(sb[u]);
                }
            }
            double fin = 0.0;
            e4l_fwd_step<0>(sv[0], acc, fin);
            e4l_fwd_step<1>(sv[1], acc, fin);
            e4l_fwd_step<2>(sv[2], acc, fin);
            e4l_fwd_step<3>(sv[3], acc, fin);
            e4l_fwd_step<4>(sv[4], acc, fin);
            e4l_fwd_step<5>(sv[5], acc, fin);
            e4l_fwd_step<6>(sv[6], acc, fin);
            e4l_fwd_step<7>(sv[7], acc, fin);
            e4l_fwd_step<8>(sw[0], acc, fin);
            e4l_fwd_step<9>(sw[1], acc, fin);
            e4l_fwd_step<10>(sw[2], acc, fin);
            e4l_fwd_step<11>(sw[3], acc, fin);
            e4l_fwd_step<12>(sw[4], acc, fin);
            e4l_fwd_step<13>(sw[5], acc, fin);
            e4l_fwd_step<14>(sw[6], acc, fin);
            e4l_fwd_step<15>(sw[7], acc, fin);
            if (live && pg[g] <= n) {
                P.alpha[beg + s + pg[g]] = fin;
                if (!(fin > 0.0 && fin <= 1.7976931348623157e308)) atomicMax(P.range_flag, 1ULL);
                if (l == 0u) P.alpha_exp[ebase + (pg[g] >> 4)] = erow;
                if (pg[g] == n) {
                    const double z = log(fin) + (double)erow * 0.6931471805599453;
                    P.zarr[s] = z;
                    zsum += z;
                    const double az = fabs(z);
                    if (!(az >= 2.2250738585072014e-308 && az <= 1.7976931348623157e308)) atomicMin(P.err_snip, (unsigned long long)s);
                }
            }
            const int e = row_max_exponent(acc);
            if (e > -100000) {
                acc = ldexp(acc, -e);
                erow += e;
            }
        }
        __builtin_amdgcn_wave_barrier();
        if (live) {
            if (n - p0 < SPAN) need_new = true;
            else p0 += SPAN;
        }
    }
    if (zsum != 0.0) atomicAdd(P.logz_sum, zsum);
}

typedef void (*estep5_fn)(Estep4Params, Encode5Params);
static estep5_fn pick_estep5(bool dropout, bool cold, int ppl) {
#define TGX_E5F(D, C)                                                                        \
    (ppl == 1 ? estep5_fwd_kernel<D, C, 1> : ppl == 2 ? estep5_fwd_kernel<D, C, 2> : ppl == 3 ? estep5_fwd_kernel<D, C, 3> : estep5_fwd_kernel<D, C, 4>)
    if (dropout) return cold ? TGX_E5F(true, true) : TGX_E5F(true, false);
    return cold ? TGX_E5F(false, true) : TGX_E5F(false, false);
#undef TGX_E5F
}
hipError_t estep5_waves_per_simd(bool dropout, bool cold, int ppl, int* out) {
    hipFuncAttributes attr;
    hipError_t e = hipFuncGetAttributes(&attr, reinterpret_cast<const void*>(pick_estep5(dropout, cold, ppl)));
    if (e != hipSuccess) return e;
    const int regs = (attr.numRegs + 7) & ~7;
    *out = regs > 0 ? (512 / regs > 8 ? 8 : 512 / regs) : 8;
    return hipSuccess;
}
hipError_t launch_estep5_fwd(const Estep4Params& p, Encode5Params q, bool cold, int ppl, int waves, uint32_t blocks, hipStream_t stream) {
    const uint32_t lds = encode5_lds_layout(q.n_hot, false, waves, ppl, &q.list_off, &q.root_off, &q.idx_off);
    if (lds > 160u * 1024u || q.n_hot > q.n_values || (!cold && q.n_hot != q.n_values) || ppl < 1 || ppl > 4) return hipErrorInvalidValue;
    estep5_fn fn = pick_estep5(p.dropout > 0.0, cold, ppl);
    hipError_t e = hipFuncSetAttribute(reinterpret_cast<const void*>(fn), hipFuncAttributeMaxDynamicSharedMemorySize, 160 * 1024);
    if (e != hipSuccess) return e;
    hipLaunchKernelGGL(fn, dim3(blocks), dim3(64u * (uint32_t)waves), lds, stream, p, q);
    return hipGetLastError();
}

typedef void (*encode5_fn)(EncodeParams, Encode5Params);
#ifdef TGX_E5_LEAN_ITEMS
constexpr int kE5LeanHot = TGX_E5_LEAN_ITEMS, kE5LeanCold = TGX_E5_LEAN_ITEMS, kE5LeanCold3 = TGX_E5_LEAN_ITEMS;
constexpr int kE6Lean = kLeanFetch;
#else
constexpr int kE5LeanHot = kLeanFetch;
constexpr int kE5LeanCold = kLeanFetch;
constexpr int kE5LeanCold3 = kLeanStep | kLeanBcast | kLeanFetch;
constexpr int kE6Lean = kLeanFetch;
#endif
static_assert(kE5LeanHot > 0 && kE5LeanHot <= 7 && kE5LeanCold > 0 && kE5LeanCold <= 7 && kE5LeanCold3 > 0 && kE5LeanCold3 <= 7,
              "a mask of kLeanStep, kLeanBcast, kLeanFetch");
constexpr int lean_without_step(int items) { return items & ~kLeanStep; }
bool encode5_has_lean(bool dropout, bool long_tokens) { return !dropout && !long_tokens; }
int encode5_lean_items(bool cold, int ppl, bool step_ok) {
    const int items = cold ? (ppl == 3 ? kE5LeanCold3 : kE5LeanCold) : kE5LeanHot;
    return step_ok ? items : lean_without_step(items);
}
int encode6_lean_items() { return kE6Lean; }
#ifdef TGX_E5_CNT
constexpr bool kE5CntHot = TGX_E5_CNT != 0, kE5CntHot2 = TGX_E5_CNT != 0, kE5CntCold = TGX_E5_CNT != 0, kE5CntCold3 = TGX_E5_CNT != 0;
#else
constexpr bool kE5CntHot = true;
constexpr bool kE5CntHot2 = true;
constexpr bool kE5CntCold = true;
constexpr bool kE5CntCold3 = true;
#endif
bool encode5_counts(bool dropout, bool cold, int ppl, bool long_tokens) {
    if (dropout || long_tokens) return false;
    return cold ? (ppl == 3 ? kE5CntCold3 : kE5CntCold) : (ppl == 2 ? kE5CntHot2 : kE5CntHot);
}
bool encode5_has_top(bool dropout, bool long_tokens) { return !dropout && !long_tokens; }
static encode5_fn pick_encode5(bool dropout, bool cold, int ppl, bool long_tokens, int compact, bool lean, bool step_ok, bool count, bool top) {
    if (long_tokens) {
        if (cold) return dropout ? encode5_kernel<true, true, 4, true> : encode5_kernel<false, true, 4, true>;
        return dropout ? encode5_kernel<true, false, 4, true> : encode5_kernel<false, false, 4, true>;
    }
    if (dropout) {
        if (cold) {
            if (ppl == 1) return encode5_kernel<true, true, 1, false>;
            if (ppl == 2) return encode5_kernel<true, true, 2, false>;
            if (ppl == 3) return encode5_kernel<true, true, 3, false>;
            return encode5_kernel<true, true, 4, false>;
        }
        if (ppl == 1) return encode5_kernel<true, false, 1, false>;
        if (ppl == 2) return encode5_kernel<true, false, 2, false>;
        if (ppl == 3) return encode5_kernel<true, false, 3, false>;
        return encode5_kernel<true, false, 4, false>;
    }
#define TGX_E5K(C, PL, LN, CN, T) \
    (compact == 4 ? encode5_kernel<false, C, PL, false, 4, LN, CN, T> : compact == 5 ? encode5_kernel<false, C, PL, false, 5, LN, CN, T> \
     : compact == 6 ? encode5_kernel<false, C, PL, false, 6, LN, CN, T> : compact == 7 ? encode5_kernel<false, C, PL, false, 7, LN, CN, T> \
     : compact == 8 ? encode5_kernel<false, C, PL, false, 8, LN, CN, T> : encode5_kernel<false, C, PL, false, 0, LN, CN, T>)
#define TGX_E5L(LNH, LNC, LNC3, CN, T) \
    if (cold) { \
        if (ppl == 1) return encode5_kernel<false, true, 1, false, 0, LNC, CN && kE5CntCold, T>; \
        if (ppl == 2) return TGX_E5K(true, 2, LNC, CN && kE5CntCold, T); \
        if (ppl == 3) return TGX_E5K(true, 3, LNC3, CN && kE5CntCold3, T); \
        return TGX_E5K(true, 4, LNC, CN && kE5CntCold, T); \
    } \
    if (ppl == 1) return encode5_kernel<false, false, 1, false, 0, LNH, CN && kE5CntHot, T>; \
    if (ppl == 2) return TGX_E5K(false, 2, LNH, CN && kE5CntHot2, T); \
    if (ppl == 3) return TGX_E5K(false, 3, LNH, CN && kE5CntHot, T); \
    return TGX_E5K(false, 4, LNH, CN && kE5CntHot, T);
#define TGX_E5C(CN, T) \
    if (lean && step_ok) { \
        TGX_E5L(kE5LeanHot, kE5LeanCold, kE5LeanCold3, CN, T) \
    } \
    if (lean) {   \
        TGX_E5L(lean_without_step(kE5LeanHot), lean_without_step(kE5LeanCold), lean_without_step(kE5LeanCold3), CN, T) \
    } \
    TGX_E5L(0, 0, 0, CN, T)
#define TGX_E5T(CN) \
    if (top) { \
        TGX_E5C(CN, true) \
    } \
    TGX_E5C(CN, false)
    if (count) {
        TGX_E5T(true)
    }
    TGX_E5T(false)
#undef TGX_E5T
#undef TGX_E5C
#undef TGX_E5L
#undef TGX_E5K
}


hipError_t encode5_waves_per_simd(bool dropout, bool cold, int ppl, bool long_tokens, int compact, bool lean, bool step_ok, bool count, bool top, int* out) {
    hipFuncAttributes attr;
    hipError_t e = hipFuncGetAttributes(&attr, reinterpret_cast<const void*>(pick_encode5(dropout, cold, ppl, long_tokens, compact, lean && encode5_has_lean(dropout, long_tokens), step_ok,
                                                                                             count && encode5_counts(dropout, cold, ppl, long_tokens),
                                                                                             top && encode5_has_top(dropout, long_tokens))));
    if (e != hipSuccess) return e;
    const int regs = (attr.numRegs + 7) & ~7;
    *out = regs > 0 ? (512 / regs > 8 ? 8 : 512 / regs) : 8;
    return hipSuccess;
}

uint32_t encode6_lds_layout(uint32_t n_hot, uint32_t pool, uint32_t* root_off, uint32_t* ctrl_off, uint32_t* ring_off) {
    const uint32_t score_bytes = 8u * (1u + 4u * kE6Slots * pool + n_hot);
    const uint32_t ro = (score_bytes + 15u) & ~15u;
    const uint32_t co = ro + 2048u;
    const uint32_t go = (co + 4u * (uint32_t)sizeof(E6Ctrl) + 511u) & ~511u;
    if (root_off) *root_off = ro;
    if (ctrl_off) *ctrl_off = co;
    if (ring_off) *ring_off = go;
    return go + 4u * kE6Slots * kE5GroupBytes;
}
uint32_t encode6_pool_total(uint32_t pool) { return 4u * kE6Slots * pool; }
uint32_t encode6_max_hot(uint32_t budget, uint32_t pool) {
    const uint32_t fixed = encode6_lds_layout(0u, pool, nullptr, nullptr, nullptr) + 512u;
    return budget > fixed + 64u ? (budget - fixed) / 8u : 0u;
}
static hipError_t lean_lds_check(const void* fn) {
    hipFuncAttributes attr;
    const hipError_t e = hipFuncGetAttributes(&attr, fn);
    if (e != hipSuccess) return e;
    return attr.sharedSizeBytes == 0 ? hipSuccess : hipErrorInvalidValue;
}

hipError_t launch_encode6(const EncodeParams& p, Encode5Params q, bool cold, bool lean, uint32_t blocks, hipStream_t stream) {
    q.ring_slots = kE6Slots;
    if (!cold) q.pool = 0u;
    const uint32_t lds = encode6_lds_layout(q.n_hot, q.pool, &q.root_off, &q.ctrl_off, &q.ring_off);
    if (lds > 160u * 1024u || q.n_hot > q.n_values || (!cold && q.n_hot != q.n_values) ||
        (uint64_t)q.n_values + 4ull * kE6Slots * q.pool > 65535ull)
        return hipErrorInvalidValue;
    lean = lean && encode5_has_lean(p.dropout > 0.0, false);
    auto fn = cold ? (p.dropout > 0.0 ? encode6_kernel<true, true> : lean ? encode6_kernel<false, true, kE6Lean> : encode6_kernel<false, true>)
                   : (p.dropout > 0.0 ? encode6_kernel<true, false> : lean ? encode6_kernel<false, false, kE6Lean> : encode6_kernel<false, false>);
    hipError_t e = hipFuncSetAttribute(reinterpret_cast<const void*>(fn), hipFuncAttributeMaxDynamicSharedMemorySize, 160 * 1024);
    if (e != hipSuccess) return e;
    if (lean && (e = lean_lds_check(reinterpret_cast<const void*>(fn))) != hipSuccess) return e;
    hipLaunchKernelGGL(fn, dim3(blocks), dim3(64u * (1u + 4u * kE6Walkers)), lds, stream, p, q);
    return hipGetLastError();
}

hipError_t launch_encode5(const EncodeParams& p, Encode5Params q, bool cold, int ppl, bool long_tokens, int compact, bool lean, bool step_ok, bool count,
                          bool top, int waves, uint32_t blocks, uint32_t min_lds, hipStream_t stream) {
    if (top && (!encode5_has_top(p.dropout > 0.0, long_tokens) || !q.top)) return hipErrorInvalidValue;
    uint32_t lds = encode5_lds_layout(q.n_hot, long_tokens, waves, ppl, &q.list_off, &q.root_off, &q.idx_off, top);
    if (lds > 160u * 1024u || q.n_hot > q.n_values || (!cold && q.n_hot != q.n_values) || (long_tokens && ppl != 4) ||
        (compact != 0 && (compact < 4 || compact > 8)))
        return hipErrorInvalidValue;
    lean = lean && encode5_has_lean(p.dropout > 0.0, long_tokens);
    if (count && !encode5_counts(p.dropout > 0.0, cold, ppl, long_tokens)) return hipErrorInvalidValue;
    encode5_fn fn = pick_encode5(p.dropout > 0.0, cold, ppl, long_tokens, compact, lean, step_ok, count, top);
    hipError_t e = hipFuncSetAttribute(reinterpret_cast<const void*>(fn), hipFuncAttributeMaxDynamicSharedMemorySize, 160 * 1024);
    if (e != hipSuccess) return e;
    if (lean && (e = lean_lds_check(reinterpret_cast<const void*>(fn))) != hipSuccess) return e;
    if (lds < min_lds && min_lds <= 160u * 1024u) lds = min_lds;
    hipLaunchKernelGGL(fn, dim3(blocks), dim3(64u * (uint32_t)waves), lds, stream, p, q);
    return hipGetLastError();
}

}
```

tokengeex_amd/csrc/encode_pass.cpp:

```cpp
#include <hip/hip_runtime.h>

#include <algorithm>
#include <chrono>
#include <condition_variable>
#include <cstdio>
#include <cstdlib>
#include <cstring>
#include <mutex>
#include <numeric>
#include <string>
#include <thread>
#include <vector>

#include "../../include/tgx.h"
#include "api_internal.h"
#include "device_internal.h"
#include "pass_internal.h"
#include "kernels.h"
#include "encode_split.h"
#include "ids_in_place.h"
#include "top_table.h"
#include "trie_build.h"

using namespace tgx::host;
using namespace tgx::dev;

namespace {

constexpr int kE5CompactDepth = 5;

uint32_t grid_blocks(const tgx_model* m, uint64_t n_samples) {
    const uint64_t wpb = tgx::encode_waves_per_block(m->lm);
    uint64_t want = (n_samples + wpb - 1) / wpb;
    uint64_t cap = (uint64_t)m->num_cus * (uint64_t)std::max(1, m->blocks_per_cu);
    return (uint32_t)std::max<uint64_t>(1, std::min(want, cap));
}

tgx_status ensure_value_ranks(tgx_model* m, const tgx_corpus* c) {
    if (m->values_ranked || !m->have_trie8 || !c->n_bytes) return TGX_OK;
    m->values_ranked = true;
    const char* vr = knob("TGX_VALUE_RANK");
    if (vr && strcmp(vr, "model") == 0) return TGX_OK;
    if (m->n_values <= tgx::encode5_max_hot(false, 13, 3, 160u * 1024u) && !(vr && strcmp(vr, "counts") == 0)) return TGX_OK;
    tgx::HostPhases hp("ensure_value_ranks");
    HIP_TRY(hipSetDevice(m->device));
    const uint32_t nv = m->n_values, chunk = 65536u;
    const uint64_t stride = std::max<uint64_t>(chunk, (c->n_bytes + 63) / 64);
    const size_t cb = ((size_t)nv + 1) * 4 + 256;
    Pass pass(m);
    unsigned int* d_cnt = nullptr;
    uint32_t* d_perm = nullptr;
    if (pass.alloc(cb, &d_cnt) != hipSuccess || pass.alloc(cb, &d_perm) != hipSuccess)
        return fail(TGX_ERR_DEVICE, "out of device memory (value counts)");
    std::vector<unsigned int> cnt((size_t)nv + 1, 0u);
    std::vector<double> values((size_t)nv + 1), wvalues;
    bool ok = hipMemsetAsync(d_cnt, 0, cb, m->stream) == hipSuccess &&
              tgx::launch_value_count(c->d_text, c->n_bytes, chunk, stride, m->d_trie8, (uint32_t)m->flat.table.size(), m->root_base8, nv,
                                      std::max<uint32_t>(1, m->flat.max_token_len), d_cnt, (uint32_t)m->num_cus, m->stream) == hipSuccess &&
              hipMemcpyAsync(cnt.data(), d_cnt, ((size_t)nv + 1) * 4, hipMemcpyDeviceToHost, m->stream) == hipSuccess &&
              hipMemcpyAsync(values.data(), m->d_values, ((size_t)nv + 1) * 8, hipMemcpyDeviceToHost, m->stream) == hipSuccess;
    if (ok && m->have_wvalues) {
        wvalues.resize((size_t)nv + 1);
        ok = hipMemcpyAsync(wvalues.data(), m->d_wvalues, ((size_t)nv + 1) * 8, hipMemcpyDeviceToHost, m->stream) == hipSuccess;
    }
    if (!ok || hipStreamSynchronize(m->stream) != hipSuccess)
        return fail(TGX_ERR_DEVICE, "value count pass failed: %s", hipGetErrorString(hipGetLastError()));
    hp.mark("value counts");
    std::vector<uint32_t> order(nv);
    for (uint32_t r = 0; r < nv; r++) order[r] = r + 1u;
    std::stable_sort(order.begin(), order.end(), [&](uint32_t a, uint32_t b) { return cnt[a] > cnt[b]; });
    std::vector<uint32_t> perm((size_t)nv + 1, 0u);
    std::vector<double> v2((size_t)nv + 1), w2(wvalues.size());
    v2[0] = values[0];
    if (!w2.empty()) w2[0] = wvalues[0];
    unsigned long long total = 0, run = 0;
    for (uint32_t r = 0; r < nv; r++) total += cnt[order[r]];
    std::vector<double> cov((size_t)nv + 1, 0.0);
    for (uint32_t r = 0; r < nv; r++) {
        perm[order[r]] = r + 1u;
        v2[r + 1u] = values[order[r]];
        if (!w2.empty()) w2[r + 1u] = wvalues[order[r]];
        run += cnt[order[r]];
        cov[r + 1u] = total ? (double)run / (double)total : 1.0;
    }
    cov[nv] = 1.0;
    ok = hipMemcpyAsync(d_perm, perm.data(), ((size_t)nv + 1) * 4, hipMemcpyHostToDevice, m->stream) == hipSuccess &&
         tgx::launch_rank_remap(m->d_trie8, (uint32_t)m->flat.table.size(), d_perm, tgx::kTrie8RankMask, m->stream) == hipSuccess &&
         (!m->d_top8 || tgx::launch_rank_remap_top(m->d_top8, d_perm, m->stream) == hipSuccess) &&
         hipMemcpyAsync(m->d_values, v2.data(), ((size_t)nv + 1) * 8, hipMemcpyHostToDevice, m->stream) == hipSuccess &&
         (w2.empty() || hipMemcpyAsync(m->d_wvalues, w2.data(), ((size_t)nv + 1) * 8, hipMemcpyHostToDevice, m->stream) == hipSuccess) &&
         hipStreamSynchronize(m->stream) == hipSuccess;
    if (!ok) return fail(TGX_ERR_DEVICE, "value re-rank failed: %s", hipGetErrorString(hipGetLastError()));
    m->value_coverage = std::move(cov);
    hp.mark("re-rank");
    return pass.done();
}

}

namespace tgx::dev {

tgx::EncodeParams base_encode_params(const tgx_model* m, const tgx_corpus* c, uint64_t seed) {
    tgx::EncodeParams p{};
    p.text = c->d_text;
    p.offs = c->d_offs;
    p.order = c->d_order;
    p.n_samples = c->n_samples;
    p.trie = m->d_trie;
    p.tokid = m->d_tokid;
    p.root_base = m->flat.table[0].base & ~tgx::kTerminalBit;
    p.lm = m->lm;
    p.n_slots = (uint32_t)m->flat.table.size();
    p.bp = c->d_bp;
    p.tmp = c->d_tmp;
    p.counts = c->d_counts;
    p.status = c->d_status;
    p.bp8 = reinterpret_cast<uint8_t*>(c->d_bp.get());
    p.tokhash = m->d_tokhash;
    p.tokhash_mask = m->tokhash.mask;
    p.tokhash_seed = m->tokhash.seed;
    p.err_sample = &m->d_ctrl->err;
    p.queue = &m->d_ctrl->queue;
    p.seed = seed;
    p.trace_carry = (c->n_samples && c->n_bytes / c->n_samples < 2048) ? 1u : 0u;
    p.trace_stride = tgx::kTraceStride;
    return p;
}

tgx_status check_no_path(tgx_model* m, const tgx_corpus* c) {
    unsigned long long bad = m->h_ctrl->err;
    if (bad == ~0ULL) return TGX_OK;
    if (bad & tgx::kErrCorruptBp)
        return fail(TGX_ERR_DEVICE, "internal error: corrupt back-pointer (sample or text byte %llu)",
                    (unsigned long long)(bad & ~tgx::kErrCorruptBp));
    if (bad & tgx::kErrCountMismatch)
        return fail(TGX_ERR_DEVICE, "internal error: the token count of sample %llu differs between the relaxation and the trace",
                    (unsigned long long)(bad & ~tgx::kErrCountMismatch));
    uint64_t n = c->h_offs[bad + 1] - c->h_offs[bad];
    set_error_detail(bad, n, n);
    return fail(TGX_ERR_NO_PATH, "no path to position %llu/%llu", (unsigned long long)n,
                (unsigned long long)n);
}

}

namespace {

tgx_status redo_long_matches(tgx_model* m, tgx_corpus* c, const tgx::EncodeParams& p) {
    unsigned long long n_redo = 0;
    HIP_TRY(hipMemcpyAsync(&n_redo, &m->d_ctrl->encode_redo, 8, hipMemcpyDeviceToHost, m->stream));
    HIP_TRY(hipStreamSynchronize(m->stream));
    if (n_redo > c->n_samples) return fail(TGX_ERR_DEVICE, "redo list longer than the batch");
    m->last_redo_samples = n_redo;
    if (n_redo) {
        tgx::EncodeParams q = p;
        q.order = c->d_counts;
        q.n_samples = n_redo;
        HIP_TRY(hipMemsetAsync(&m->d_ctrl->queue, 0x00, 8, m->stream));
        time_begin(m, "encode2_kernel");
        HIP_TRY(tgx::launch_encode2(q, (uint32_t)m->num_cus, true, m->stream));
        time_end(m);
    }
    return TGX_OK;
}

tgx_status scan_ids_offsets(tgx_model* m, tgx_corpus* c, tgx_result* r, const char* what, bool with_err);

struct Encode6Choice {
    int e6_bpc;
    uint32_t n_hot6;
    uint32_t pool6;
    bool cold6;
    bool e6_usable;
};
Encode6Choice choose_encode6(const tgx_model* m) {
    int e6_bpc = 2;
    if (const char* e = knob("TGX_E6_BPC")) e6_bpc = std::min(4, std::max(1, atoi(e)));
    uint32_t n_hot6 = std::min(m->n_values, tgx::encode6_max_hot(160u * 1024u / (uint32_t)e6_bpc, 0u));
    uint32_t pool6 = 0;
    bool e6_usable = true;
    if (n_hot6 < m->n_values) {
        pool6 = 128;
        if (const char* e = knob("TGX_E6_POOL")) pool6 = (uint32_t)std::min(192, std::max(0, atoi(e)));
        if ((uint64_t)m->n_values + tgx::encode6_pool_total(pool6) > 65535ull) {
            pool6 = 0;
            e6_usable = knob("TGX_E6_POOL") != nullptr || knob("TGX_LONG_THRESHOLD") != nullptr;
        }
        n_hot6 = std::min(m->n_values, tgx::encode6_max_hot(160u * 1024u / (uint32_t)e6_bpc, pool6));
    }
    n_hot6 = knob_cap_hot("TGX_E5_HOT", n_hot6);
    const bool cold6 = n_hot6 < m->n_values;
    return Encode6Choice{e6_bpc, n_hot6, pool6, cold6, e6_usable};
}

tgx::EncodeSplit split_long_samples(const tgx_model* m, const tgx_corpus* c, const Encode6Choice& e6) {
    tgx::EncodeSplitQuery sq{};
    sq.sorted_len = c->h_sorted_len.data();
    sq.sorted_cum = c->h_sorted_cum.data();
    sq.n_samples = c->n_samples;
    sq.n_bytes = c->n_bytes;
    sq.max_len = c->max_len;
    sq.num_cus = m->num_cus;
    sq.cold6 = e6.cold6;
    sq.e6_bpc = e6.e6_bpc;
    sq.values_fit = m->n_values <= tgx::encode5_max_hot(false, 8, 4, 160u * 1024u);
    sq.corun_timeouts = m->corun_wait_timeouts != 0;
    if (const char* e = knob("TGX_LONG_THRESHOLD")) {
        sq.threshold_set = true;
        sq.threshold = (uint64_t)std::max(0ll, atoll(e));
    }
    if (const char* e = knob("TGX_CORUN")) {
        sq.corun_set = true;
        sq.corun = atoi(e);
    }
    return tgx::encode_split(sq);
}

struct Encode5Geometry {
    int ppl, bpc, waves;
    int per_simd;
    bool cold;
    uint32_t n_hot;
    uint32_t blocks5;
    int compact;
    bool lean, step_ok;
    bool in_place;
    bool top;
};
constexpr bool kE5Top14Waves = true;
tgx_status choose_encode5(const tgx_model* m, const tgx_corpus* c, const tgx::EncodeParams& p, bool long_tokens, uint64_t n_long,
                          uint32_t corun_cus, bool have_result, Encode5Geometry* out) {
    const double dropout = p.dropout;
    const int cus5 = m->num_cus - (int)corun_cus;
    const uint64_t rest_n = c->n_samples - n_long;
    const uint64_t rest_bytes = c->n_bytes - (n_long ? c->h_sorted_cum[n_long - 1] : 0);
    const uint64_t rest_max = rest_n ? c->h_sorted_len[n_long] : 0;
    int ppl = 4, bpc = 1, hot_waves = 16;
    int compact = kE5CompactDepth;
    if (const char* e = knob("TGX_E5_COMPACT")) compact = (strcmp(e, "off") == 0 || atoi(e) == 0) ? 0 : std::min(8, std::max(4, atoi(e)));
    bool lean = tgx::encode5_has_lean(dropout > 0.0, long_tokens);
    if (const char* e = knob("TGX_E5_LEAN")) lean = lean && atoi(e) != 0;
    const bool step_ok = m->lean_scores_ok;
    bool top = tgx::encode5_has_top(dropout > 0.0, long_tokens) && m->d_top8 != nullptr;
    if (const char* e = knob("TGX_E5_TOP")) top = top && atoi(e) != 0;
    const uint32_t lds_cu = 160u * 1024u;
    tgx::IdsInPlaceQuery iq{};
    iq.rows5 = true;
    iq.long_tokens = long_tokens;
    iq.dropout = dropout > 0.0;
    iq.n_long = n_long;
    iq.build_counts = true;
    iq.max_len = c->max_len;
    iq.switched_on = !(knob("TGX_IDS_IN_PLACE") && atoi(knob("TGX_IDS_IN_PLACE")) == 0);
    iq.diagnostics = p.flags != 0u || (debug_on() && getenv("TGX_STAMPS") != nullptr);
    const bool want_count = have_result && tgx::ids_in_place(iq);
    {
        int ps4 = 0;
        HIP_TRY(tgx::encode5_waves_per_simd(dropout > 0.0, false, 4, long_tokens, compact, lean, step_ok, want_count, top, &ps4));
        hot_waves = std::min(16, ps4 * 4);
        const int least = long_tokens ? 12 : 13;
        while (hot_waves >= least && m->n_values > tgx::encode5_max_hot(long_tokens, hot_waves, 4, lds_cu, top)) hot_waves--;
        if (hot_waves < least) {
            hot_waves = 0;
            if (!long_tokens) {
                if (top && kE5Top14Waves && m->n_values <= tgx::encode5_max_hot(false, 14, 3, lds_cu, top)) {
                    ppl = 3;
                    hot_waves = 14;
                } else if (m->n_values <= tgx::encode5_max_hot(false, 13, 3, lds_cu, top)) {
                    ppl = 3;
                    hot_waves = 13;
                } else if (m->n_values <= tgx::encode5_max_hot(false, 16, 2, lds_cu, top)) {
                    ppl = 2;
                } else {
                    ppl = 3;
                }
            }
        }
    }
    int balance_waves = 0;
    if (rest_max > 0) {
        const uint64_t rows_bal = (rest_bytes + rest_max - 1) / rest_max;
        const uint64_t wb = (rows_bal + 4ull * (uint64_t)cus5 - 1) / (4ull * (uint64_t)cus5);
        if (wb <= 10) {
            balance_waves = (int)std::max<uint64_t>(4, wb);
            ppl = 4;
            hot_waves = 0;
        }
    }
    if (const char* e = long_tokens ? nullptr : knob("TGX_PPL")) {
        const int v = atoi(e);
        if (v >= 1 && v <= 4) {
            ppl = v;
            bpc = ppl >= 3 ? 1 : 2;
        }
    }
    knob_int("TGX_BPC", 1, 8, &bpc);
    const uint32_t budget = 160u * 1024u / (uint32_t)bpc;
    bool cold = false;
    int per_simd = 0;
    HIP_TRY(tgx::encode5_waves_per_simd(dropout > 0.0, false, ppl, long_tokens, compact, lean, step_ok, want_count, top, &per_simd));
    int waves = std::min(16, (per_simd / bpc) * 4);
    if ((ppl == 4 || ppl == 3) && bpc == 1 && hot_waves > 0) waves = std::min(waves, hot_waves);
    if (m->n_values > tgx::encode5_max_hot(long_tokens, waves, ppl, budget, top)) {
        cold = true;
        HIP_TRY(tgx::encode5_waves_per_simd(dropout > 0.0, true, ppl, long_tokens, compact, lean, step_ok, want_count, top, &per_simd));
        waves = std::min(16, (per_simd / bpc) * 4);
    }
    if (balance_waves > 0 && ppl == 4 && bpc == 1) waves = std::min(waves, balance_waves);
    waves = waves_for_units(waves, rest_n, (uint64_t)cus5 * bpc);
    knob_int("TGX_WAVES", 1, 16, &waves);
    while (waves > 1 && tgx::encode5_max_hot(long_tokens, waves, ppl, budget, top) < 16u) waves--;
    uint32_t n_hot = std::min(m->n_values, tgx::encode5_max_hot(long_tokens, waves, ppl, budget, top));
    n_hot = knob_cap_hot("TGX_E5_HOT", n_hot);
    cold = n_hot < m->n_values;
    iq.build_counts = tgx::encode5_counts(dropout > 0.0, cold, ppl, long_tokens);
    const bool in_place = want_count && tgx::ids_in_place(iq);
    const uint64_t rows_per_block = 4 * (uint64_t)waves;
    const uint32_t blocks5 = (uint32_t)std::max<uint64_t>(
        1, std::min<uint64_t>((rest_n + rows_per_block - 1) / rows_per_block, (uint64_t)cus5 * bpc));
    *out = Encode5Geometry{ppl, bpc, waves, per_simd, cold, n_hot, blocks5, compact, lean, step_ok, in_place, top};
    return TGX_OK;
}

tgx_status trace_rows5(tgx_model* m, tgx_corpus* c, tgx::EncodeParams& p, bool long_tokens, bool in_place, Pass& pass, tgx_result* r) {
    const uint32_t blocks_t = trace_blocks(m, c->n_samples);
    if (in_place) {
        const tgx_status st = scan_ids_offsets(m, c, r, "encode", false);
        if (st != TGX_OK) return st;
        time_begin(m, "trace_kernel");
        HIP_TRY(tgx::launch_trace_in_place(p, tgx::TraceInPlace{r->d_offs, r->d_ids}, blocks_t, m->stream));
        time_end(m);
        m->last_ids_in_place = true;
        return TGX_OK;
    }
    Stamps stamps_t;
    if (!long_tokens) stamps_t = stamps_begin(m, pass, '2', (size_t)blocks_t * 4);
    p.stamps = stamps_t.d;
    time_begin(m, long_tokens ? "trace32_kernel" : "trace_kernel");
    if (long_tokens) HIP_TRY(tgx::launch_trace32(p, blocks_t, true, m->stream));
    else HIP_TRY(tgx::launch_trace(p, blocks_t, m->stream));
    time_end(m);
    if (stamps_t.d) stamps_report(m, stamps_t, 0, "trace stamps", "window", {"setup", "loads", "hops", "append+lookups", "-"});
    p.stamps = nullptr;
    return TGX_OK;
}

tgx_status encode_rows5(tgx_model* m, tgx_corpus* c, tgx::EncodeParams& p, bool long_tokens, Pass& pass, tgx_result* r) {
    tgx_status st = ensure_value_ranks(m, c);
    if (st != TGX_OK) return st;
    m->last_redo_samples = 0;
    const Encode6Choice e6 = choose_encode6(m);
    tgx::EncodeSplit split;
    if (c->n_samples && !long_tokens && e6.e6_usable) split = split_long_samples(m, c, e6);
    const uint64_t n_long = split.n_long;
    const uint32_t corun_cus = split.corun_cus;
    Encode5Geometry g;
    if ((st = choose_encode5(m, c, p, long_tokens, n_long, corun_cus, r != nullptr, &g)) != TGX_OK) return st;
    m->last_n_hot = g.n_hot;
    m->last_encode_top = g.top && c->n_samples - n_long != 0;
    if (!g.in_place) {
        if ((st = ensure_scratch(c, true)) != TGX_OK) return st;
        p.tmp = c->d_tmp;
    }
    const uint64_t rest_n = c->n_samples - n_long;
    m->last_lean_items = !g.lean ? 0u : ((rest_n ? (uint32_t)tgx::encode5_lean_items(g.cold, g.ppl, g.step_ok) : 0u) |
                                         (n_long ? (uint32_t)tgx::encode6_lean_items() << 8 : 0u));
    m->last_encode_waves_per_cu = std::min(g.bpc, g.per_simd / ((g.waves + 3) / 4)) * g.waves;
    tgx::Encode5Params q{};
    q.trie8 = m->d_trie8;
    q.trie_bytes = (uint32_t)(m->flat.table.size() * sizeof(tgx::Trie8Rec));
    q.values = m->d_values;
    q.root_base = m->root_base8;
    q.top = m->d_top8;
    q.n_values = m->n_values;
    q.n_hot = g.n_hot;
    q.claim_chunk = claim_chunk_for(c->n_bytes, c->n_samples);
    if (const char* e = knob("TGX_CLAIM_CHUNK")) q.claim_chunk = (uint32_t)std::min(64, std::max(1, atoi(e)));
    m->last_long_samples = n_long;
    m->last_corun_cus = n_long ? corun_cus : 0u;
    tgx::EncodeParams p6 = p;
    tgx::Encode5Params q6 = q;
    uint32_t blocks6 = 0;
    if (n_long) {
        p6.n_samples = n_long;
        blocks6 = (uint32_t)std::min<uint64_t>((n_long + 3) / 4, (uint64_t)(corun_cus ? (int)corun_cus : m->num_cus) * (uint64_t)e6.e6_bpc);
        q6.n_hot = e6.n_hot6;
        q6.pool = e6.cold6 ? e6.pool6 : 0u;
        if (!corun_cus) {
            time_begin(m, "encode6_kernel");
            HIP_TRY(tgx::launch_encode6(p6, q6, e6.cold6, g.lean, blocks6, m->stream));
            time_end(m);
            HIP_TRY(hipMemsetAsync(&m->d_ctrl->queue, 0x00, 8, m->stream));
        } else {
            if (!m->stream2) {
                HIP_TRY(hipStreamCreateWithFlags(&m->stream2, hipStreamNonBlocking));
                HIP_TRY(hipEventCreateWithFlags(&m->ev_fork, hipEventDisableTiming));
                HIP_TRY(hipEventCreateWithFlags(&m->ev_join, hipEventDisableTiming));
                HIP_TRY(hipHostMalloc((void**)&m->h_started, 64, hipHostMallocMapped | hipHostMallocPortable));
            }
            *reinterpret_cast<volatile unsigned int*>(m->h_started) = 0u;
            q.started = m->h_started;
            p6.queue = &m->d_ctrl->queue6;
            HIP_TRY(hipMemsetAsync(&m->d_ctrl->queue6, 0x00, 8, m->stream));
            HIP_TRY(hipEventRecord(m->ev_fork, m->stream));
            HIP_TRY(hipStreamWaitEvent(m->stream2, m->ev_fork, 0));
        }
        p.order = c->d_order + n_long;
        p.n_samples = c->n_samples - n_long;
    }
    const Stamps stamps5 = stamps_begin(m, pass, '1', (size_t)g.blocks5 * (size_t)g.waves);
    p.stamps = stamps5.d;
    time_begin(m, "encode5_kernel");
    {
        if (long_tokens) {
            p.redo_count = &m->d_ctrl->encode_redo;
            p.redo_list = c->d_counts;
            HIP_TRY(hipMemsetAsync(&m->d_ctrl->encode_redo, 0x00, 8, m->stream));
        }
        const hipError_t le = tgx::launch_encode5(p, q, g.cold, g.ppl, long_tokens, g.compact, g.lean, g.step_ok, g.in_place, g.top, g.waves, g.blocks5, corun_cus && n_long ? 84u * 1024u : 0u, m->stream);
        if (le != hipSuccess) return fail(TGX_ERR_DEVICE, "encode5 launch failed: %s", hipGetErrorString(le));
    }
    bool joined = false, joined_slot = false;
    if (n_long && corun_cus) {
        const bool slot = m->n_timed + 1 < kMaxTimed;
        if (slot) {
            KernelTime& tb = m->timed[m->n_timed + 1];
            tb.name = "encode6_kernel";
            tb.used = true;
            (void)hipEventRecord(tb.start, m->stream2);
        }
        {
            const auto t0 = std::chrono::steady_clock::now();
            volatile unsigned int* started = m->h_started;
            bool timed_out = false;
            while (*started < g.blocks5 && !(timed_out = std::chrono::steady_clock::now() - t0 >= std::chrono::milliseconds(2))) {
            }
            if (timed_out && *started < g.blocks5) m->corun_wait_timeouts++;
        }
        const hipError_t l6 = tgx::launch_encode6(p6, q6, e6.cold6, g.lean, blocks6, m->stream2);
        if (slot) (void)hipEventRecord(m->timed[m->n_timed + 1].stop, m->stream2);
        (void)hipEventRecord(m->ev_join, m->stream2);
        if (l6 != hipSuccess) return fail(TGX_ERR_DEVICE, "encode6 launch failed: %s", hipGetErrorString(l6));
        joined = true;
        joined_slot = slot;
    }
    time_end(m);
    if (joined) {
        if (joined_slot) m->n_timed++;
        HIP_TRY(hipStreamWaitEvent(m->stream, m->ev_join, 0));
    }
    if (stamps5.d) stamps_report(m, stamps5, g.ppl, "encode5 stamps", "iteration", {"switch", "text+reset", "walk", "relax", "store"});
    p.stamps = nullptr;
    if (long_tokens) {
        const tgx_status rst = redo_long_matches(m, c, p);
        if (rst != TGX_OK) return rst;
    }
    p.order = c->d_order;
    p.n_samples = c->n_samples;
    return trace_rows5(m, c, p, long_tokens, g.in_place, pass, r);
}

tgx_status encode_rows4(tgx_model* m, tgx_corpus* c, tgx::EncodeParams& p, Pass& pass) {
    const double dropout = p.dropout;
    int ppl = 1, waves = 10, bpc = 2;
    const double gbps4[3] = {60.0, 50.0, 34.0}, chain4_ms[3] = {13.5, 10.7, 9.1};
    auto cost4 = [&](double bytes, double longest, int* ppl_out) {
        double best_t = 0;
        int best_ppl = 1;
        for (int i = 0; i < 3; i++) {
            const double t = std::max(bytes / (gbps4[i] * 1e9), longest / 65536.0 * chain4_ms[i] * 1e-3);
            if (i == 0 || t < best_t * 0.95) {
                best_t = t;
                best_ppl = 1 << i;
            }
        }
        if (ppl_out) *ppl_out = best_ppl;
        return best_t;
    };
    m->last_long_samples = 0;
    m->last_redo_samples = 0;
    cost4((double)c->n_bytes, c->n_samples ? (double)c->h_sorted_len[0] : 0.0, &ppl);
    if (const char* e = knob("TGX_PPL")) {
        const int v = atoi(e);
        if (v == 1 || v == 2 || v == 4) ppl = v;
    }
    if (ppl == 2) { waves = 5; bpc = 2; }
    if (ppl == 4) { waves = 5; bpc = 1; }
    knob_int("TGX_WAVES", 1, 16, &waves);
    knob_int("TGX_BPC", 1, 8, &bpc);
    bool root = ppl == 1;
    if (const char* e = knob("TGX_ROOT")) root = root && atoi(e) != 0;
    while (waves > 1 && tgx::encode4_lds_bytes(waves, ppl, root) > (160u * 1024u) / (uint32_t)bpc) waves--;
    {
        int per_simd = 0;
        HIP_TRY(tgx::encode4_waves_per_simd(dropout > 0.0, ppl, root, &per_simd));
        if (bpc * ((waves + 3) / 4) > per_simd && ppl == 1) {
            waves = 4;
            bpc = std::min(5, per_simd);
            root = false;
            HIP_TRY(tgx::encode4_waves_per_simd(dropout > 0.0, ppl, root, &per_simd));
        }
        m->last_encode_waves_per_cu = std::min(bpc * ((waves + 3) / 4), per_simd) * 4 >= bpc * waves
                                          ? bpc * waves
                                          : per_simd / ((waves + 3) / 4) * waves;
    }
    const uint64_t rows_per_block = 4 * (uint64_t)waves;
    const uint32_t blocks4 = (uint32_t)std::max<uint64_t>(
        1, std::min<uint64_t>((p.n_samples + rows_per_block - 1) / rows_per_block, (uint64_t)m->num_cus * bpc));
    Stamps stamps4;
    if (dropout <= 0.0 && ppl == 1) stamps4 = stamps_begin(m, pass, '1', (size_t)blocks4 * (size_t)waves);
    p.stamps = stamps4.d;
    time_begin(m, "encode4_kernel");
    HIP_TRY(tgx::launch_encode4(p, ppl, waves, blocks4, root, m->stream));
    time_end(m);
    if (stamps4.d) stamps_report(m, stamps4, 0, "stamps", "iteration", {"switch", "text", "walk", "relax", "store"});
    p.stamps = nullptr;
    p.order = c->d_order;
    p.n_samples = c->n_samples;
    time_begin(m, "trace_kernel");
    HIP_TRY(tgx::launch_trace(p, trace_blocks(m, c->n_samples), m->stream));
    time_end(m);
    return TGX_OK;
}

tgx_status encode_rows2(tgx_model* m, tgx_corpus* c, tgx::EncodeParams& p, bool rows2) {
    m->last_redo_samples = 0;
    if (!rows2) {
        p.redo_count = &m->d_ctrl->encode_redo;
        p.redo_list = c->d_counts;
        HIP_TRY(hipMemsetAsync(&m->d_ctrl->encode_redo, 0x00, 8, m->stream));
        time_begin(m, "encode4l_kernel");
        HIP_TRY(tgx::launch_encode4l(p, (uint32_t)m->num_cus, m->stream));
        time_end(m);
        const tgx_status rst = redo_long_matches(m, c, p);
        if (rst != TGX_OK) return rst;
    } else {
        time_begin(m, "encode2_kernel");
        HIP_TRY(tgx::launch_encode2(p, (uint32_t)m->num_cus, false, m->stream));
        time_end(m);
    }
    time_begin(m, "trace32_kernel");
    HIP_TRY(tgx::launch_trace32(p, trace_blocks(m, c->n_samples), !rows2, m->stream));
    time_end(m);
    return TGX_OK;
}

tgx_status encode_fused(tgx_model* m, tgx_corpus* c, const tgx::EncodeParams& p) {
    time_begin(m, "encode_kernel");
    HIP_TRY(tgx::launch_encode(p, grid_blocks(m, c->n_samples), m->stream));
    time_end(m);
    return TGX_OK;
}

tgx_status run_encode_kernel(tgx_model* m, tgx_corpus* c, double dropout, uint64_t seed, Pass& pass, tgx_result* r) {
    m->last_ids_in_place = false;
    tgx_status st = ensure_scratch(c, false);
    if (st != TGX_OK) return st;
    HIP_TRY(hipMemsetAsync(&m->d_ctrl->queue, 0x00, 8, m->stream));
    HIP_TRY(hipMemsetAsync(&m->d_ctrl->err, 0xFF, 8, m->stream));
    tgx::EncodeParams p = base_encode_params(m, c, seed);
    p.dropout = dropout;
    if (const char* e = knob("TGX_TRACE_CARRY")) p.trace_carry = atoi(e) ? 1u : 0u;
    if (const char* e = knob("TGX_TRACE_STRIDE")) p.trace_stride = (uint32_t)std::min(3, std::max(0, atoi(e)));
    p.flags = debug_flags();
    const char* force = knob("TGX_PATH");
    const bool use4 = m->lm <= 16 && m->scores_finite && m->d_tokhash && !(force && strcmp(force, "fused") == 0);
    const bool use2 = !use4 && m->lm <= 32 && m->scores_finite && m->d_tokhash && !(force && strcmp(force, "fused") == 0);
    const bool long_tokens = m->lm > 16;
    const bool use5 = (use4 || use2) && m->have_trie8 &&
                      !(force && (strcmp(force, "rows4") == 0 || strcmp(force, "rows2") == 0 || strcmp(force, "rows4l") == 0));
    if (debug_on())
        fprintf(stderr, "[tgx] encode: S=%llu N=%llu lm=%u path=%s slots=%zu root_base=%u values=%u\n",
                (unsigned long long)c->n_samples, (unsigned long long)c->n_bytes, p.lm, use4 ? (use5 ? "rows5" : "rows4") : (use2 ? "rows2" : "fused"),
                m->flat.table.size(), p.root_base, m->n_values);
    m->last_lean_items = 0;
    m->last_encode_top = false;
    if (use5) return encode_rows5(m, c, p, long_tokens, pass, r);
    if ((st = ensure_scratch(c, true)) != TGX_OK) return st;
    p.tmp = c->d_tmp;
    if (use4) return encode_rows4(m, c, p, pass);
    if (use2) return encode_rows2(m, c, p, force && strcmp(force, "rows2") == 0);
    return encode_fused(m, c, p);
}

tgx_status scan_ids_offsets(tgx_model* m, tgx_corpus* c, tgx_result* r, const char* what, bool with_err) {
    const uint64_t S = c->n_samples;
    if (!c->d_scan_tmp) {
        if (tgx::scan_temp_bytes(S, &c->scan_tmp_bytes) != hipSuccess) return fail(TGX_ERR_DEVICE, "scan temp-size query failed");
        if (c->scan_tmp_bytes && c->d_scan_tmp.alloc(m->device, c->scan_tmp_bytes) != hipSuccess)
            return fail(TGX_ERR_DEVICE, "out of device memory (scan)");
    }
    time_begin(m, "scan_counts_kernel");
    if (tgx::launch_scan(c->d_counts, r->d_offs, S, c->d_scan_tmp, c->scan_tmp_bytes, m->stream) != hipSuccess)
        return fail(TGX_ERR_DEVICE, "scan launch failed");
    time_end(m);
    if ((with_err && hipMemcpyAsync(&m->h_ctrl->err, &m->d_ctrl->err, 8, hipMemcpyDeviceToHost, m->stream) != hipSuccess) ||
        hipMemcpyAsync(&m->h_ctrl->total_tokens, r->d_offs + S, 8, hipMemcpyDeviceToHost, m->stream) != hipSuccess ||
        hipStreamSynchronize(m->stream) != hipSuccess)
        return fail(TGX_ERR_DEVICE, "%s pass failed: %s", what, hipGetErrorString(hipGetLastError()));
    if (with_err) {
        const tgx_status st = check_no_path(m, c);
        if (st != TGX_OK) return st;
    }
    r->n_tokens = m->h_ctrl->total_tokens;
    if (r->n_tokens > c->n_bytes) return fail(TGX_ERR_DEVICE, "internal error: %s pass counted more tokens than bytes", what);
    if (r->d_ids.alloc(m->device, (size_t)r->n_tokens * 4 + 256) != hipSuccess)
        return fail(TGX_ERR_DEVICE, "out of device memory (result ids)");
    return TGX_OK;
}

}

tgx_status tgx::dev::compact_ids(tgx_model* m, tgx_corpus* c, tgx_result* r, const char* what) {
    const uint64_t S = c->n_samples;
    const tgx_status sst = scan_ids_offsets(m, c, r, what, true);
    if (sst != TGX_OK) return sst;
    tgx::CompactParams cp{};
    cp.offs = c->d_offs;
    cp.order = c->d_order;
    cp.n_samples = S;
    cp.tmp = c->d_tmp;
    cp.out_offs = r->d_offs;
    cp.ids = r->d_ids;
    const bool rows = S && r->n_tokens / S < 128;
    const uint64_t units = rows ? 16 : 4;
    const uint32_t blocks = (uint32_t)std::max<uint64_t>(1, std::min<uint64_t>((S + units - 1) / units, (uint64_t)m->num_cus * 8));
    time_begin(m, "compact_kernel");
    if (tgx::launch_compact(cp, blocks, rows, m->stream) != hipSuccess) return fail(TGX_ERR_DEVICE, "compact launch failed");
    time_end(m);
    return TGX_OK;
}
tgx_status tgx::dev::ensure_encode_tables(tgx_model* m) {
    if (m->encode_tables_ready) return TGX_OK;
    HIP_TRY(hipSetDevice(m->device));
    tgx::HostPhases hp("ensure_encode_tables");
    const bool want_hash = m->lm <= 32 && m->scores_finite;
    const bool want_trie8 = m->lm <= 32 && m->scores_finite && m->flat.table.size() <= tgx::kTrie8MaxSlots;
    std::thread hash_builder;
    if (want_hash && !m->tokhash_host_built)
        hash_builder = std::thread([m]() { tgx::build_tok_hash(m->vocab_bytes.data(), m->vocab_offs.data(), m->vocab_size, &m->tokhash); });
    tgx::Trie8 t8;
    if (want_trie8) tgx::build_trie8(m->flat, m->vocab_offs.data(), m->vocab_scores.data(), &t8);
    if (hash_builder.joinable()) hash_builder.join();
    hp.mark("trie8 | tok hash");
    if (want_hash && m->tokhash.ok && !m->d_tokhash) {
        const size_t hb = m->tokhash.slots.size() * sizeof(tgx::TokHashEntry);
        HIP_TRY(hipMalloc(&m->d_tokhash, hb));
        HIP_TRY(hipMemcpyAsync(m->d_tokhash, m->tokhash.slots.data(), hb, hipMemcpyHostToDevice, m->stream));
    }
    if (want_trie8 && t8.ok && m->d_tokhash) {
        const size_t ns = t8.rec.size();
        if (!m->d_trie8) HIP_TRY(hipMalloc(&m->d_trie8, ns * sizeof(tgx::Trie8Rec)));
        if (!m->d_values) HIP_TRY(hipMalloc((void**)&m->d_values, t8.values.size() * 8));
        HIP_TRY(hipMemcpy(m->d_trie8, t8.rec.data(), ns * sizeof(tgx::Trie8Rec), hipMemcpyHostToDevice));
        HIP_TRY(hipMemcpy(m->d_values, t8.values.data(), t8.values.size() * 8, hipMemcpyHostToDevice));
        const tgx_status tst = upload_top_table(m, t8.rec.data(), ns, t8.root_base);
        if (tst != TGX_OK) return tst;
        m->n_values = (uint32_t)t8.values.size() - 1u;
        m->value_coverage = std::move(t8.coverage);
        m->root_base8 = t8.root_base;
        m->have_trie8 = true;
    }
    HIP_TRY(hipStreamSynchronize(m->stream));
    hp.mark("uploads");
    m->encode_tables_ready = true;
    return TGX_OK;
}

tgx_status tgx::dev::upload_top_table(tgx_model* m, const tgx::Trie8Rec* rec, size_t n_slots, uint32_t root_base) {
    std::vector<tgx::Trie8Rec> top;
    tgx::build_top_table(rec, n_slots, root_base, &top);
    if (!m->d_top8) HIP_TRY(hipMalloc(&m->d_top8, top.size() * sizeof(tgx::Trie8Rec)));
    HIP_TRY(hipMemcpy(m->d_top8, top.data(), top.size() * sizeof(tgx::Trie8Rec), hipMemcpyHostToDevice));
    return TGX_OK;
}


tgx_status tgx::dev::encode_corpus_locked(tgx_model* m, tgx_corpus* c, double dropout, uint64_t seed,
                                          tgx_result** out) {
    HIP_TRY(hipSetDevice(m->device));
    {
        const tgx_status est = ensure_encode_tables(m);
        if (est != TGX_OK) return est;
    }
    m->n_timed = 0;
    const uint64_t S = c->n_samples;

    Pass pass(m);
    tgx_result* r = pass.new_result(S);
    if (r->d_offs.alloc(m->device, (size_t)(S + 1) * 8) != hipSuccess)
        return fail(TGX_ERR_DEVICE, "out of device memory (result offsets)");
    tgx_status st = run_encode_kernel(m, c, dropout, seed, pass, r);
    if (st != TGX_OK) return st;
    if (m->last_ids_in_place) {
        if (hipMemcpyAsync(&m->h_ctrl->err, &m->d_ctrl->err, 8, hipMemcpyDeviceToHost, m->stream) != hipSuccess ||
            hipStreamSynchronize(m->stream) != hipSuccess)
            return fail(TGX_ERR_DEVICE, "encode pass failed: %s", hipGetErrorString(hipGetLastError()));
        st = check_no_path(m, c);
        if (st != TGX_OK) return st;
    } else {
        st = compact_ids(m, c, r, "encode");
        if (st != TGX_OK) return st;
        if (hipStreamSynchronize(m->stream) != hipSuccess)
            return fail(TGX_ERR_DEVICE, "compact failed: %s", hipGetErrorString(hipGetLastError()));
    }
    m->last_alg_bytes = c->n_bytes + 4 * r->n_tokens + 16 * (S + 1);
    *out = pass.release_result();
    return pass.done();
}

tgx_status tgx_encode_corpus(tgx_model* m, tgx_corpus* c, double dropout, uint64_t seed,
                             tgx_result** out) {
    if (!m || !c || !out) return fail(TGX_ERR_INVALID, "tgx_encode_corpus: NULL argument");
    *out = nullptr;
    if (m->device != c->device) return fail(TGX_ERR_INVALID, "model and corpus on different devices");
    std::lock_guard<std::mutex> lk(m->mu);
    std::lock_guard<std::mutex> lkc(c->mu);
    return encode_corpus_locked(m, c, dropout, seed, out);
}

tgx_status tgx_encode_batch(tgx_model* m, const uint8_t* text, const uint64_t* offs,
                            uint64_t n_samples, double dropout, uint64_t seed, tgx_result** out) {
    if (!m || !out) return fail(TGX_ERR_INVALID, "tgx_encode_batch: NULL argument");
    *out = nullptr;
    return on_uploaded_batch(m, text, offs, n_samples, [&](tgx_corpus* c) { return tgx_encode_corpus(m, c, dropout, seed, out); });
}

tgx_status tgx_encode_batch_host(tgx_model* m, const uint8_t* text, const uint64_t* offs, uint64_t n_samples, double dropout,
                                 uint64_t seed, uint32_t* ids_out, uint64_t ids_cap, uint64_t* offs_out, uint64_t* n_tokens) {
// ... 89 lines not shown
            }
            tgx_result* r = nullptr;
            const auto t0 = std::chrono::steady_clock::now();
            const tgx_status st = tgx_encode_corpus(m, c, dropout, seed, &r);
            tgx_corpus_free(c);
            stamp("kernels", k, t0);
            std::lock_guard<std::mutex> lk(mu);
            cs[k].corpus = nullptr;
            if (st != TGX_OK) {
                set_error(st, cut[k]);
                return;
            }
            cs[k].result = r;
            cs[k].tokens = r->n_tokens;
            cs[k].stage = 2;
            cv.notify_all();
        }
    });
    uint64_t base = 0;
    for (size_t k = 0; k < C; k++) {
        tgx_result* r = nullptr;
        {
            std::unique_lock<std::mutex> lk(mu);
            cv.wait(lk, [&]() { return abort_all || cs[k].stage >= 2; });
            if (cs[k].stage < 2) break;
            r = cs[k].result;
        }
        const uint64_t lo = cut[k], hi = cut[k + 1];
        const auto t0 = std::chrono::steady_clock::now();
        tgx_status st2 = TGX_OK;
        if (base + r->n_tokens > ids_cap) {
            st2 = fail(TGX_ERR_INVALID, "tgx_encode_batch_host: ids_out holds %llu ids, the batch has more", (unsigned long long)ids_cap);
        } else {
            if (r->n_tokens) st2 = tgx_result_copy_ids(r, ids_out + base, r->n_tokens);
            if (st2 == TGX_OK) {
                std::vector<uint64_t> lo_offs(hi - lo + 1);
                st2 = tgx_result_copy_offsets(r, lo_offs.data(), hi - lo + 1);
                for (uint64_t i = 0; i <= hi - lo && st2 == TGX_OK; i++) offs_out[lo + i] = base + lo_offs[i];
            }
        }
        base += r->n_tokens;
        stamp("download", k, t0);
        if (st2 == TGX_OK) tgx_result_free(r);
        std::lock_guard<std::mutex> lk(mu);
        if (st2 != TGX_OK) {
            g_err_sample = 0;
            set_error(st2, 0);
            break;
        }
        cs[k].result = nullptr;
        cs[k].stage = 3;
        downloaded = k + 1;
        cv.notify_all();
    }
    {
        std::lock_guard<std::mutex> lk(mu);
        if (downloaded < C && first_err == TGX_OK) abort_all = true;
        cv.notify_all();
    }
    uploader.join();
    encoder.join();
    for (size_t k = 0; k < C; k++) {
        if (cs[k].result) tgx_result_free(cs[k].result);
        if (cs[k].corpus) tgx_corpus_free(cs[k].corpus);
    }
    if (first_err != TGX_OK) {
        g_err_msg = err_msg;
        g_err_sample = err_sample;
        g_err_pos = err_pos;
        g_err_len = err_len;
        return first_err;
    }
    uint64_t total = 0;
    for (size_t k = 0; k < C; k++) total += cs[k].tokens;
    *n_tokens = total;
    m->last_alg_bytes = N + 4 * total + 16 * (n_samples + 1);
    return TGX_OK;
}

tgx_status tgx_encode_batch_multi(tgx_model* const* models, uint32_t n_models, const uint8_t* text, const uint64_t* offs,
                                  uint64_t n_samples, double dropout, uint64_t seed, uint32_t* ids_out, uint64_t ids_cap,
                                  uint64_t* offs_out, uint64_t* n_tokens) {
    if (!models || n_models == 0 || !offs_out || !n_tokens || (n_samples && !offs)) return fail(TGX_ERR_INVALID, "tgx_encode_batch_multi: NULL argument");
    for (uint32_t k = 0; k < n_models; k++)
        if (!models[k]) return fail(TGX_ERR_INVALID, "tgx_encode_batch_multi: NULL model handle");
    *n_tokens = 0;
    offs_out[0] = 0;
    if (n_samples == 0) return TGX_OK;
    const uint64_t N = offs[n_samples] - offs[0];
    if (ids_cap < N) return fail(TGX_ERR_INVALID, "tgx_encode_batch_multi: ids_out must hold one id per input byte (%llu), it holds %llu",
                                 (unsigned long long)N, (unsigned long long)ids_cap);
    std::vector<uint64_t> cut(n_models + 1, n_samples);
    cut[0] = 0;
    for (uint32_t k = 1; k < n_models; k++) {
        const uint64_t want = offs[0] + N / n_models * k;
        cut[k] = (uint64_t)(std::lower_bound(offs, offs + n_samples, want) - offs);
        cut[k] = std::max(cut[k], cut[k - 1]);
    }
    struct Shard {
        tgx_status st = TGX_OK;
        uint64_t tokens = 0;
        std::string msg;
        uint64_t es = 0, ep = 0, el = 0;
        std::vector<uint64_t> lo;
    };
    std::vector<Shard> sh(n_models);
    std::vector<std::thread> th;
    for (uint32_t k = 0; k < n_models; k++) {
        th.emplace_back([&, k]() {
            Shard& S = sh[k];
            const uint64_t a = cut[k], b = cut[k + 1];
            if (b == a) return;
            S.lo.assign(b - a + 1, 0);
            const uint64_t region = offs[a] - offs[0];
            S.st = tgx_encode_batch_host(models[k], text, offs + a, b - a, dropout, seed, ids_out + region, ids_cap - region, S.lo.data(), &S.tokens);
            if (S.st != TGX_OK) {
                S.msg = g_err_msg;
                S.es = g_err_sample + a;
                S.ep = g_err_pos;
                S.el = g_err_len;
            }
        });
    }
    for (std::thread& t : th) t.join();
    for (uint32_t k = 0; k < n_models; k++)
        if (sh[k].st != TGX_OK) {
            g_err_msg = sh[k].msg;
            g_err_sample = sh[k].es;
            g_err_pos = sh[k].ep;
            g_err_len = sh[k].el;
            return sh[k].st;
        }
    uint64_t base = 0;
    for (uint32_t k = 0; k < n_models; k++) {
        const uint64_t a = cut[k], b = cut[k + 1];
        if (b == a) continue;
        const uint64_t region = offs[a] - offs[0];
        if (region != base && sh[k].tokens) memmove(ids_out + base, ids_out + region, sh[k].tokens * sizeof(uint32_t));
        for (uint64_t i = 0; i <= b - a; i++) offs_out[a + i] = base + sh[k].lo[i];
        base += sh[k].tokens;
    }
    *n_tokens = base;
    return TGX_OK;
}


uint32_t tgx_last_encode_waves_per_cu(const tgx_model* m) { return m ? (uint32_t)m->last_encode_waves_per_cu : 0u; }
uint64_t tgx_last_encode_redo_samples(const tgx_model* m) { return m ? m->last_redo_samples : 0; }
uint64_t tgx_last_encode_long_samples(const tgx_model* m) { return m ? m->last_long_samples : 0; }
uint32_t tgx_last_encode_corun_cus(const tgx_model* m) { return m ? m->last_corun_cus : 0; }
uint32_t tgx_encode_corun_timeouts(const tgx_model* m) { return m ? m->corun_wait_timeouts : 0; }
uint32_t tgx_last_encode_hot_values(const tgx_model* m) { return m ? m->last_n_hot : 0u; }
int tgx_last_encode_top_table(const tgx_model* m) { return m && m->last_encode_top ? 1 : 0; }
uint32_t tgx_last_encode_lean_items(const tgx_model* m) { return m ? m->last_lean_items : 0u; }
int tgx_last_encode_ids_in_place(const tgx_model* m) { return (m && m->last_ids_in_place) ? 1 : 0; }
```

tokengeex_amd/csrc/kernels.h:

```cpp
#pragma once
#include <hip/hip_runtime.h>
#include <stdint.h>

#include "decode.h"
#include "encode5_layout.h"
#include "fim.h"
#include "spans.h"

namespace tgx {

constexpr uint32_t kTraceStride = 2;

struct EncodeParams {
    const uint8_t* text;
    const uint64_t* offs;
    const uint32_t* order;
    uint64_t n_samples;
    const void* trie;
    const uint32_t* tokid;
    uint32_t root_base;
    uint32_t n_slots;
    uint32_t lm;
    uint32_t* bp;
    uint32_t* tmp;
// ... 99 lines not shown
    int32_t* alpha_exp;
    double* expected_slot;
    uint32_t n_slots_rev, n_replicas;
    uint32_t n_hot;
    double* logz_sum;
    unsigned long long* err_snip;
    uint32_t flags;
    unsigned long long* range_flag;
    unsigned long long* queue_fwd;
    unsigned long long* queue_bwd;
    double dropout;
    uint64_t seed;
};
struct CutParams {
    const uint8_t* text;
    const uint64_t* soffs;
    const uint32_t* snip_sample;
    const uint64_t* snip_base;
    const uint32_t* win_snip;
    const uint32_t* win_k;
    uint64_t n_windows;
    uint32_t window;
    const void* trie;
    uint32_t root;
    uint32_t lmx;
    double dropout;
    uint64_t seed;
    uint64_t* bound;
    uint32_t* flag;
};
hipError_t launch_cut_windows(const CutParams& p, hipStream_t stream);
hipError_t launch_cut_scatter(const CutParams& p, const uint64_t* pos, uint64_t n_bytes, uint64_t* poffs, uint32_t* psample,
                              uint64_t* pbase, uint32_t* psnip, hipStream_t stream);
hipError_t launch_piece_len(const uint64_t* poffs, const uint64_t* n_pieces, uint32_t* len, uint32_t* idx, unsigned long long* longest,
                            uint64_t cap, hipStream_t stream);
hipError_t piece_sort_temp_bytes(uint64_t n, size_t* bytes);
hipError_t piece_sort(void* temp, size_t temp_bytes, const uint32_t* len_in, uint32_t* len_out, const uint32_t* idx_in, uint32_t* idx_out,
                      uint64_t n, hipStream_t stream);
hipError_t launch_piece_z_check(const double* zarr, const uint32_t* psnip, uint64_t n_pieces, double* zsnip, uint64_t n_snips,
                                unsigned long long* err_snip, hipStream_t stream);

struct Estep7Work {
    const uint64_t* soffs;
    const uint32_t* order;
    uint64_t n_snips;
    const uint32_t* snip_sample;
    const uint64_t* snip_base;
    const uint32_t* snip_of;
    double* zsnip;
    double* logz_sum;
    unsigned long long* range_flag;
    unsigned long long* queue;
    unsigned long long* redo_count;
    uint64_t* redo_offs;
    uint32_t* redo_sample;
    uint64_t* redo_base;
    uint32_t* redo_snip;
    uint64_t redo_cap;
};
struct Estep7Params {
    const uint8_t* text;
    const Estep7Work* work;
    Estep7Work host_work;
    const void* trie8t;
    uint32_t n_slots;
    uint32_t root_base;
    const double* wtab;
    uint32_t n_tok;
    uint32_t ovf_limit;
    uint32_t n_hot;
    double* expected;
    double dropout;
    uint64_t seed;
    uint32_t claim_chunk;
    uint32_t root_off, zero_off, idx_off;
    uint32_t flags;
    unsigned long long* stamps;
};
struct Estep7RedoParams {
    const uint8_t* text;
    const uint64_t* redo_offs;
    const uint32_t* redo_sample;
    const uint64_t* redo_base;
    const uint32_t* redo_snip;
    uint64_t n_redo;
    const uint64_t* tbase;
    const void* trie8t;
    uint32_t n_slots;
    uint32_t root_base;
    const double* wtab;
    uint32_t n_tok, n_hot;
    double* expected;
    double* zsnip;
    double* logz_sum;
    unsigned long long* range_flag;
    unsigned long long* queue;
    double* alpha;
    int32_t* aexp;
    unsigned char* mscratch;
    double dropout;
    uint64_t seed;
    uint32_t root_off, zero_off, idx_off;
};
uint32_t estep7_redo_max_hot(bool wide);
hipError_t launch_estep7_redo(Estep7RedoParams p, bool wide, uint32_t num_cus, hipStream_t stream);
uint32_t estep7_lds_layout(uint32_t n_hot, bool wide, int waves, int ppl, uint32_t* root_off, uint32_t* zero_off, uint32_t* idx_off);
uint32_t estep7_max_hot(bool wide, int waves, int ppl, uint32_t budget);
hipError_t estep7_waves_per_simd(bool dropout, bool cold, bool wide, int ppl, int* out);
hipError_t launch_estep7(Estep7Params p, bool wide, int ppl, int waves, uint32_t blocks, hipStream_t stream);
hipError_t launch_match_count(const uint8_t* text, uint64_t n_bytes, uint32_t chunk, uint64_t stride, const void* trie8t, uint32_t n_slots,
                              uint32_t root_base, uint32_t n_tok, unsigned int* counts, uint32_t num_cus, hipStream_t stream);
hipError_t launch_value_count(const uint8_t* text, uint64_t n_bytes, uint32_t chunk, uint64_t stride, const void* trie8, uint32_t n_slots,
                              uint32_t root_base, uint32_t n_values, uint32_t max_len, unsigned int* counts, uint32_t num_cus, hipStream_t stream);
hipError_t launch_rank_remap(void* trie8t, uint32_t n_slots, const uint32_t* perm, uint32_t rank_mask, hipStream_t stream);
hipError_t launch_rank_remap_top(void* top, const uint32_t* perm, hipStream_t stream);
hipError_t launch_snip_z_check(const double* zsnip, uint64_t n_snips, unsigned long long* err_snip, hipStream_t stream);
hipError_t launch_piece_z_add(const double* zarr, const uint32_t* psnip, const uint32_t* order, uint64_t n_order, double* zsnip, hipStream_t stream);

hipError_t estep4_prepare();
hipError_t launch_estep4_fwd(const Estep4Params& p, uint32_t num_cus, hipStream_t stream);
hipError_t launch_estep4_bwd(const Estep4Params& p, uint32_t num_cus, hipStream_t stream);
hipError_t estep4l_prepare();
hipError_t launch_estep4l_fwd(const Estep4Params& p, int ppl, bool long_tokens, uint32_t num_cus, hipStream_t stream);
hipError_t launch_estep4l_bwd(const Estep4Params& p, int ppl, bool long_tokens, uint32_t num_cus, uint32_t groups_wanted, hipStream_t stream);
hipError_t launch_estep4_reduce(const double* rep, double* out, uint32_t n_slots, uint32_t n_replicas,
                                hipStream_t stream);

uint32_t estep_lds_bytes_per_block(uint32_t lm);
uint32_t estep_waves_per_block(uint32_t lm);
hipError_t estep_max_blocks_per_cu(uint32_t lm, int* out);
hipError_t launch_estep(const EstepParams& p, uint32_t blocks, hipStream_t stream);

uint32_t encode_lds_bytes_per_block(uint32_t lm);
uint32_t encode_waves_per_block(uint32_t lm);
hipError_t encode_max_blocks_per_cu(uint32_t lm, int* out);
hipError_t launch_encode(const EncodeParams& p, uint32_t blocks, hipStream_t stream);
uint32_t encode4_group_bytes();
hipError_t encode4_waves_per_simd(bool dropout, int ppl, bool root, int* out);
hipError_t launch_encode4(const EncodeParams& p, int ppl, int waves, uint32_t blocks, bool root, hipStream_t stream);
uint32_t encode4_lds_bytes(int waves, int ppl, bool root);
hipError_t launch_trace(const EncodeParams& p, uint32_t blocks, hipStream_t stream);
struct TraceInPlace {
    const uint64_t* out_offs;
    uint32_t* ids;
};
hipError_t launch_trace_in_place(const EncodeParams& p, const TraceInPlace& o, uint32_t blocks, hipStream_t stream);
constexpr unsigned long long kErrCorruptBp = 1ULL << 62;
constexpr unsigned long long kErrCountMismatch = 1ULL << 61;
bool encode5_has_lean(bool dropout, bool long_tokens);
int encode5_lean_items(bool cold, int ppl, bool step_ok);
int encode6_lean_items();
bool encode5_counts(bool dropout, bool cold, int ppl, bool long_tokens);
bool encode5_has_top(bool dropout, bool long_tokens);
hipError_t encode5_waves_per_simd(bool dropout, bool cold, int ppl, bool long_tokens, int compact, bool lean, bool step_ok, bool count, bool top, int* out);
uint32_t encode6_lds_layout(uint32_t n_hot, uint32_t pool, uint32_t* root_off, uint32_t* ctrl_off, uint32_t* ring_off);
uint32_t encode6_max_hot(uint32_t budget, uint32_t pool);
uint32_t encode6_pool_total(uint32_t pool);
hipError_t estep5_waves_per_simd(bool dropout, bool cold, int ppl, int* out);
hipError_t launch_estep5_fwd(const struct Estep4Params& p, Encode5Params q, bool cold, int ppl, int waves, uint32_t blocks, hipStream_t stream);
hipError_t launch_encode6(const EncodeParams& p, Encode5Params q, bool cold, bool lean, uint32_t blocks, hipStream_t stream);
hipError_t launch_encode5(const EncodeParams& p, Encode5Params q, bool cold, int ppl, bool long_tokens, int compact, bool lean, bool step_ok, bool count,
                          bool top, int waves, uint32_t blocks, uint32_t min_lds, hipStream_t stream);
hipError_t launch_encode2(const EncodeParams& p, uint32_t num_cus, bool permuted, hipStream_t stream);
hipError_t launch_trace32(const EncodeParams& p, uint32_t blocks, bool permuted, hipStream_t stream);
hipError_t launch_encode4l(const EncodeParams& p, uint32_t num_cus, hipStream_t stream);
hipError_t scan_temp_bytes(uint64_t n, size_t* bytes);
hipError_t launch_scan(uint32_t* counts, uint64_t* offsets, uint64_t n, void* temp, size_t temp_bytes, hipStream_t stream);
hipError_t launch_compact(const CompactParams& p, uint32_t blocks, bool rows, hipStream_t stream);

struct LayoutParams {
    const uint32_t* ids;
    const uint64_t* offs;
    uint64_t n_rows;
    uint32_t len;
    uint32_t pad, bos, eos;
    uint32_t flags;
    void* out;
    uint8_t* mask;
    int32_t* lengths;
    int32_t* doc;
    int32_t* pos;
    unsigned long long* counter;
};
hipError_t launch_layout_max_row(const uint64_t* offs, uint64_t n_rows, unsigned long long* max_out, hipStream_t stream);
hipError_t launch_layout_pad(const LayoutParams& p, hipStream_t stream);
hipError_t launch_layout_pack(const LayoutParams& p, uint64_t n_stream, uint64_t n_out, hipStream_t stream);
struct WindowParams {
    LayoutParams base;
    const uint64_t* wo;
    uint32_t stride;
    int32_t* window_row;
    int32_t* window_first;
};
hipError_t launch_layout_window_count(const uint64_t* offs, uint64_t n_rows, uint32_t room, uint32_t step, uint32_t* counts,
                                      unsigned long long* max_out, hipStream_t stream);
hipError_t launch_layout_windows(const WindowParams& q, uint64_t n_windows, hipStream_t stream);

struct AssembleParams {
    const uint32_t* ids;
    const uint64_t* offs;
    const uint64_t* seg_offs;
    const int32_t* seg_special;
    uint64_t* rank;
    uint64_t* starts;
    uint64_t n_segs, n_samples;
    uint64_t n_out;
    uint32_t vocab_size;
    uint32_t* out_ids;
    uint64_t* out_offs;
};
hipError_t assemble_scan_temp_bytes(uint64_t n_segs, size_t* bytes);
hipError_t launch_assemble_ranks(int32_t* seg_special, uint64_t* rank, uint64_t n_segs, void* temp, size_t temp_bytes, hipStream_t stream);
hipError_t launch_assemble_starts(const AssembleParams& p, hipStream_t stream);
hipError_t launch_assemble_fill(const AssembleParams& p, hipStream_t stream);

struct FimParams {
    const uint32_t* ids;
    const uint64_t* offs;
    uint64_t n_rows;
    FimArgs f;
    uint64_t n_out;
    uint32_t* out_ids;
    uint64_t* out_offs;
};
hipError_t fim_scan_temp_bytes(uint64_t n_rows, size_t* bytes);
hipError_t launch_fim_offsets(const FimParams& p, void* temp, size_t temp_bytes, hipStream_t stream);
hipError_t launch_fim_fill(const FimParams& p, hipStream_t stream);
hipError_t launch_fim_info(const FimParams& p, uint8_t* mode, uint64_t* cuts, hipStream_t stream);

struct SelectParams {
    const void* data;
    const uint64_t* offs;
    uint64_t n_src;
    const int64_t* rows;
    uint64_t n_rows;
    uint64_t* out_offs;
    uint64_t n_out;
    void* out;
};
hipError_t select_scan_temp_bytes(uint64_t n_rows, size_t* bytes);
hipError_t launch_select_check(const SelectParams& p, unsigned long long* bad, hipStream_t stream);
hipError_t launch_select_offsets(const SelectParams& p, void* temp, size_t temp_bytes, hipStream_t stream);
hipError_t launch_select_fill_ids(const SelectParams& p, hipStream_t stream);
hipError_t launch_select_fill_text(const SelectParams& p, hipStream_t stream);
hipError_t launch_select_lengths(const uint64_t* offs, uint64_t n_src, int64_t* lengths, hipStream_t stream);
hipError_t shuffle_sort_temp_bytes(uint64_t n, size_t* bytes);
hipError_t launch_shuffled_rows(uint64_t n, uint64_t seed, uint64_t* keys_in, uint64_t* keys_out, int64_t* vals_in, int64_t* rows, void* temp,
                                size_t temp_bytes, hipStream_t stream);

struct DecodeParams {
    DecodeTables tab;
    DecodeSrc src;
    uint32_t* meta;
    uint64_t* starts;
    uint64_t* specials;
    unsigned long long* bad_pos;
    unsigned long long* n_replaced;
    unsigned long long* n_specials_live;
    uint64_t n_raw;
    uint8_t* raw;
    uint32_t* flags;
    uint32_t* codes;
    uint64_t* row_offs;
    uint64_t* gpos;
    uint8_t* out;
};
hipError_t decode_scan_temp_bytes(uint64_t n, size_t* bytes);
hipError_t launch_decode_meta(const DecodeParams& p, void* temp, size_t temp_bytes, hipStream_t stream);
hipError_t launch_decode_specials(const DecodeParams& p, void* temp, size_t temp_bytes, hipStream_t stream);
hipError_t launch_decode_fill(const DecodeParams& p, hipStream_t stream);
hipError_t launch_decode_rows(const DecodeParams& p, hipStream_t stream);
hipError_t launch_decode_utf8(const DecodeParams& p, hipStream_t stream);
hipError_t decode_expand_temp_bytes(uint64_t n_groups, size_t* bytes);
hipError_t launch_decode_positions(const DecodeParams& p, void* temp, size_t temp_bytes, hipStream_t stream);
hipError_t launch_decode_expand(const DecodeParams& p, hipStream_t stream);

struct SpanParams {
    SpanTables tab;
    const uint32_t* ids;
    const uint64_t* offs;
    uint64_t n_rows, n;
    uint32_t* vals;
    uint64_t* sums;
    unsigned long long* row_max;
    uint32_t len;
    uint32_t bos, eos;
    uint32_t flags;
    void* out;
};
hipError_t span_scan_temp_bytes(uint64_t n, size_t* bytes);
hipError_t launch_span_sums(const SpanParams& p, void* temp, size_t temp_bytes, hipStream_t stream);
hipError_t launch_span_row_max(const SpanParams& p, hipStream_t stream);
hipError_t launch_span_flat(const SpanParams& p, hipStream_t stream);
hipError_t launch_span_pad(const SpanParams& p, hipStream_t stream);
hipError_t launch_span_windows(const SpanParams& p, const uint64_t* wo, uint32_t stride, uint64_t n_windows, hipStream_t stream);

}
```

Baseline: 75650.

## Assign consecutive positions per lane in encode5 top-table walks

Adds a SEQ variant of the encode5 kernel in which each lane handles PPL consecutive text positions instead of positions strided by 16. A lane now loads a narrower window of dwords and derives each position's bytes by byte-aligning a shared stream, and the LDS slots it writes are remapped to match. The aim is fewer global loads and registers per lane and better locality. The cost is different LDS bank and write patterns, an extra template dimension with more kernel instantiations, and reliance on slack padding after the text. It is on by default for the hot builds and for cold PPL 3, and an environment knob can override it.

```diff
diff --git a/include/tgx_encode_info.h b/include/tgx_encode_info.h
--- /dev/null
+++ b/include/tgx_encode_info.h
@@ -0,0 +1,16 @@
+#ifndef TGX_ENCODE_INFO_H
+#define TGX_ENCODE_INFO_H
+
+#include "tgx.h"
+
+#ifdef __cplusplus
+extern "C" {
+#endif
+
+int tgx_last_encode_seq_walks(const tgx_model *m);
+
+#ifdef __cplusplus
+}
+#endif
+
+#endif
diff --git a/tokengeex_amd/_lib.py b/tokengeex_amd/_lib.py
--- a/tokengeex_amd/_lib.py
+++ b/tokengeex_amd/_lib.py
@@ -216,6 +216,9 @@
     "tgx_wordstat_last_times": (_i, [C.POINTER(C.c_char_p), C.POINTER(C.c_float), _i]),
 }
 
+ENCODE_INFO_SYMBOLS = {
+    "tgx_last_encode_seq_walks": (_i, [_vp]),
+}
 PHRASE_SYMBOLS = {
     "tgx_phraseset_create": (_i, [_i, _vp, _vp, _u32, _u32, _u32, _vp]),
     "tgx_phraseset_info": (_i, [_vp, C.POINTER(C.c_uint32), C.POINTER(C.c_uint32), C.POINTER(C.c_uint32), C.POINTER(C.c_uint32),
@@ -262,7 +265,7 @@
             "Build it with `python tokengeex_amd/build.py`.")
     _share_torch_hip_runtime()
     lib = C.CDLL(LIB_PATH)
-    for name, (res, args) in list(SYMBOLS.items()) + list(WORD_SYMBOLS.items()) + list(PHRASE_SYMBOLS.items()):
+    for name, (res, args) in list(SYMBOLS.items()) + list(WORD_SYMBOLS.items()) + list(PHRASE_SYMBOLS.items()) + list(ENCODE_INFO_SYMBOLS.items()):
         fn = getattr(lib, name)
         fn.restype = res
         fn.argtypes = args
@@ -1961,6 +1964,9 @@
     def last_encode_top_table(self) -> bool:
         return bool(lib.tgx_last_encode_top_table(self._h))
 
+    def last_encode_seq_walks(self) -> bool:
+        return bool(lib.tgx_last_encode_seq_walks(self._h))
+
     def last_encode_long_samples(self) -> int:
         return lib.tgx_last_encode_long_samples(self._h)
 
diff --git a/tokengeex_amd/build.py b/tokengeex_amd/build.py
--- a/tokengeex_amd/build.py
+++ b/tokengeex_amd/build.py
@@ -9,7 +9,7 @@
 CSRC = os.path.join(HERE, "csrc")
 OUT = os.path.join(HERE, "libtgx.so")
 SOURCES = ["kernels.hip", "estep.hip", "encode2.hip", "encode4l.hip", "encode5.hip", "estep4.hip", "estep4l.hip", "estep7.hip", "cuts.hip", "pairs.hip", "generate.hip", "sample.hip", "stats.hip", "nbest.hip", "layout.hip", "assemble.hip", "fim.hip", "select.hip", "dedup.hip", "minhash.hip", "gram.hip", "repeat.hip", "textstat.hip", "wordstat.hip", "phrase.hip", "decode.hip", "spans.hip", "front.hip", "norm.hip", "tgx_api.cpp", "encode_pass.cpp", "estep_pass.cpp", "lattice_pass.cpp", "result_ops.cpp", "corpus_ops.cpp", "minhash_ops.cpp", "gram_ops.cpp", "repeat_ops.cpp", "textstat_ops.cpp", "wordstat_ops.cpp", "phrase_ops.cpp", "host_twins.cpp", "trie_build.cpp", "prune_host.cpp", "frontback.cpp", "unicode_norm.cpp"]
-HEADERS = ["api_internal.h", "device_internal.h", "pass_internal.h", "kernels.h", "sample.h", "stats.h", "nbest.h", "layout.h", "assemble.h", "fim.h", "select.h", "dedup.h", "minhash.h", "gram.h", "gram_walk.h", "repeat.h", "shingle_load.h", "textstat.h", "textstat_walk.h", "wordstat.h", "phrase.h", "decode.h", "spans.h", "front.h", "norm.h", "device_common.h", "lattice_walk.h", "tile_fill.h", "scan_helpers.h", "lean_gate.h", "ids_in_place.h", "encode_split.h", "encode5_layout.h", "top_table.h", "trace_body.h", "trie_build.h", "unicode_tables.h", os.path.join("..", "..", "include", "tgx.h"), os.path.join("..", "..", "include", "tgx_words.h"), os.path.join("..", "..", "include", "tgx_phrases.h")]
+HEADERS = ["api_internal.h", "device_internal.h", "pass_internal.h", "kernels.h", "sample.h", "stats.h", "nbest.h", "layout.h", "assemble.h", "fim.h", "select.h", "dedup.h", "minhash.h", "gram.h", "gram_walk.h", "repeat.h", "shingle_load.h", "textstat.h", "textstat_walk.h", "wordstat.h", "phrase.h", "decode.h", "spans.h", "front.h", "norm.h", "device_common.h", "lattice_walk.h", "tile_fill.h", "scan_helpers.h", "lean_gate.h", "ids_in_place.h", "encode_split.h", "encode5_layout.h", "encode5_seq.h", "top_table.h", "trace_body.h", "trie_build.h", "unicode_tables.h", os.path.join("..", "..", "include", "tgx.h"), os.path.join("..", "..", "include", "tgx_words.h"), os.path.join("..", "..", "include", "tgx_phrases.h"), os.path.join("..", "..", "include", "tgx_encode_info.h")]
 ARCH = "gfx950"
 
 
diff --git a/tokengeex_amd/csrc/device_internal.h b/tokengeex_amd/csrc/device_internal.h
--- a/tokengeex_amd/csrc/device_internal.h
+++ b/tokengeex_amd/csrc/device_internal.h
@@ -148,6 +148,7 @@
     void* d_tokhash = nullptr;
     void* d_trie8 = nullptr;
     void* d_top8 = nullptr;
+    bool last_encode_seq = false;
     bool last_encode_top = false;
     double* d_values = nullptr;
     std::vector<double> value_coverage;
diff --git a/tokengeex_amd/csrc/encode5.hip b/tokengeex_amd/csrc/encode5.hip
--- a/tokengeex_amd/csrc/encode5.hip
+++ b/tokengeex_amd/csrc/encode5.hip
@@ -5,6 +5,7 @@
 
 #include "device_common.h"
 #include "encode5_layout.h"
+#include "encode5_seq.h"
 #include "kernels.h"
 
 namespace tgx {
@@ -43,7 +44,7 @@
 template <bool DROPOUT, bool LONG, bool RES, int PPL, int D, bool SKIP = false, int CK = 0, bool PK = false, bool T0 = false>
 struct Walk5 {
     static_assert(CK == 0 || (!DROPOUT && !LONG && !RES && PPL >= 2 && D < CK && CK < 16), "compaction: hot and COLD builds of two to four walks per lane");
-    static_assert(!T0 || (D == 1 && !DROPOUT && !LONG && !RES && !PK), "top-table entries: the first level of the hot and COLD builds");
+    static_assert(!T0 || (D == 1 && !DROPOUT && !LONG && !RES), "top-table entries: the first level of the hot and COLD builds");
     static __device__ __forceinline__ void run(const WalkCtx<PPL>& W, Res5& R, const uint32_t (&bytes)[PPL][4], const uint32_t (&maxd)[PPL],
                                                const uint32_t (&pg)[PPL], const uint32_t (&wlane)[PPL], bool (&alive)[PPL],
                                                uint2 (&rec)[PPL], uint32_t (&c)[PPL]) {
@@ -57,7 +58,7 @@
             asm("" : "+v"(rec[g].x), "+v"(rec[g].y));
             if constexpr (T0) {
                 const uint32_t rank0 = rec[g].y >> 16;
-                if (alive[g] && rank0 != 0u) lds_st<uint16_t>(wlane[g] | W.l32, (uint16_t)rank0);
+                if (alive[g] && rank0 != 0u) lds_st<uint16_t>(PK ? wlane[g] : (wlane[g] | W.l32), (uint16_t)rank0);
                 alive[g] = alive[g] && 1u < maxd[g];
             }
             alive[g] = alive[g] && ((rec[g].x >> 24) == c[g]);
@@ -302,10 +303,13 @@
         t_last = _now;                                                 \
     }
 
-template <bool DROPOUT, bool COLD, int PPL, bool LONG, int CK = 0, int LN = 0, bool CNT = false, bool TOP = false>
+template <bool DROPOUT, bool COLD, int PPL, bool LONG, int CK = 0, int LN = 0, bool CNT = false, bool TOP = false, bool SEQ = false>
 __global__ __launch_bounds__(1024, (PPL == 1 ? 8 : (PPL == 2 ? 6 : (PPL == 3 ? 4 : 1)))) void encode5_kernel(EncodeParams P, Encode5Params Q) {
     static_assert(!LONG || PPL == 4, "the long-token build runs four positions per lane");
     static_assert((LN == 0 && !CNT && !TOP) || (!LONG && !DROPOUT), "the long-token and dropout builds keep the kernel as it was");
+    static_assert(!SEQ || (TOP && PPL >= 2), "consecutive walks: the top-table builds at two to four positions per lane");
+    constexpr int NWD = SEQ ? e5_seq_dwords(PPL) : 4 * PPL + 1;
+    typedef const __attribute__((address_space(1))) uint32_t* gtext_t;
     extern __shared__ __align__(16) unsigned char smem[];
     constexpr uint32_t LM = LONG ? 32 : 16;
     constexpr uint32_t SPAN = 16u * PPL;
@@ -339,11 +343,11 @@
     double acc = ninf, far = ninf;
     uint32_t bpv = kNoStep, fbp = kFarCode;
     bool redo = false;
-    uint32_t wn[4 * PPL + 1];
+    uint32_t wn[NWD];
     uint32_t pk = 0, pk_j = 0;
     bool pk_dirty = false;
 #pragma unroll
-    for (int q = 0; q <= 4 * PPL; ++q) wn[q] = 0;
+    for (int q = 0; q < NWD; ++q) wn[q] = 0;
     const uint32_t my_col = r * kE5RowStride + ((l - 1u) & 15u) * 32u;
     const uint32_t wbase_off = lds0 + Q.idx_off + wave * (PPL * kE5GroupBytes);
     const uint32_t wr_off = wbase_off + r * kE5RowStride + l * 2u;
@@ -391,22 +395,33 @@
         iters++;
         E5_STAMP(0)
 
-        const uintptr_t addr = reinterpret_cast<uintptr_t>(P.text + (live ? beg + p0 + l : 0));
+        const uintptr_t addr = reinterpret_cast<uintptr_t>(P.text + (live ? beg + p0 + (SEQ ? (uint32_t)PPL * l : l) : 0));
         const uint32_t sh = (uint32_t)(addr & 3u);
         const uint32_t* __restrict__ wp = reinterpret_cast<const uint32_t*>(addr & ~uintptr_t(3));
-        uint32_t w[4 * PPL + 1];
+        const gtext_t gp = reinterpret_cast<gtext_t>(addr & ~uintptr_t(3));
+        uint32_t w[NWD];
         if (fresh_row) {
 #pragma unroll
-            for (int q = 0; q <= 4 * PPL; ++q) w[q] = wp[q];
+            for (int q = 0; q < NWD; ++q) w[q] = SEQ ? gp[q] : wp[q];
         } else {
 #pragma unroll
-            for (int q = 0; q <= 4 * PPL; ++q) w[q] = wn[q];
+            for (int q = 0; q < NWD; ++q) w[q] = wn[q];
         }
         uint32_t bytes[PPL][4];
-#pragma unroll
-        for (int g = 0; g < PPL; ++g)
-#pragma unroll
-            for (int q = 0; q < 4; ++q) bytes[g][q] = __builtin_amdgcn_alignbyte(w[4 * g + q + 1], w[4 * g + q], sh);
+        if constexpr (SEQ) {
+            uint32_t v[kE5SeqStream];
+#pragma unroll
+            for (int q = 0; q < kE5SeqStream; ++q) v[q] = __builtin_amdgcn_alignbyte(q + 1 < NWD ? w[q + 1 < NWD ? q + 1 : 0] : 0u, w[q], sh);
+#pragma unroll
+            for (int g = 0; g < PPL; ++g)
+#pragma unroll
+                for (int q = 0; q < 4; ++q) bytes[g][q] = g == 0 ? v[q] : __builtin_amdgcn_alignbyte(v[q + 1], v[q], (uint32_t)g);
+        } else {
+#pragma unroll
+            for (int g = 0; g < PPL; ++g)
+#pragma unroll
+                for (int q = 0; q < 4; ++q) bytes[g][q] = __builtin_amdgcn_alignbyte(w[4 * g + q + 1], w[4 * g + q], sh);
+        }
         uint2 top_rec[TOP ? PPL : 1];
         if constexpr (TOP) {
 #pragma unroll
@@ -431,10 +446,12 @@
 #pragma unroll
         for (int g = 0; g < PPL; ++g) {
             pg[g] = p0 + 16u * g + l;
-            const uint32_t rem = (live && pg[g] < n) ? (n - pg[g]) : 0u;
+            const uint32_t pw = SEQ ? p0 + e5_seq_pos(PPL, l, (uint32_t)g) : pg[g];
+            const uint32_t rem = (live && pw < n) ? (n - pw) : 0u;
             maxd[g] = rem < LM ? rem : LM;
             alive[g] = maxd[g] > 0 && !(P.flags & 1u);
-            wlane[g] = wr_off + g * kE5GroupBytes;
+            wlane[g] = SEQ ? wbase_off + e5_seq_base(e5_seq_pos(PPL, l, (uint32_t)g), r) : wr_off + g * kE5GroupBytes;
+            if constexpr (SEQ) asm volatile("" : "+v"(wlane[g]));
             if constexpr (!TOP) {
                 c[g] = bytes[g][0] & 0xFFu;
                 rec[g] = rootc[(Q.root_base ^ c[g]) & 255u];
@@ -451,7 +468,7 @@
                     rec[g] = top_rec[g];
                     c[g] = (bytes[g][0] >> 8) & 0xFFu;
                 }
-                Walk5<DROPOUT, LONG, false, PPL, 1, COLD && PPL < 4, CK, false, true>::run(W, no_res, bytes, maxd, pg, wlane, alive, rec, c);
+                Walk5<DROPOUT, LONG, false, PPL, 1, COLD && PPL < 4, CK, SEQ, true>::run(W, no_res, bytes, maxd, pg, wlane, alive, rec, c);
             } else {
                 Walk5<DROPOUT, LONG, false, PPL, 0, COLD && PPL < 4, CK>::run(W, no_res, bytes, maxd, pg, wlane, alive, rec, c);
             }
@@ -466,8 +483,9 @@
         E5_STAMP(2)
         {
             const uint32_t* __restrict__ np = wp + 4 * PPL;
-#pragma unroll
-            for (int q = 0; q <= 4 * PPL; ++q) wn[q] = np[q];
+            const gtext_t gn = gp + 4 * PPL;
+#pragma unroll
+            for (int q = 0; q < NWD; ++q) wn[q] = SEQ ? gn[q] : np[q];
         }
 
         if (!(P.flags & 32u)) __builtin_amdgcn_s_setprio(0);
@@ -1217,7 +1235,23 @@
     return cold ? (ppl == 3 ? kE5CntCold3 : kE5CntCold) : (ppl == 2 ? kE5CntHot2 : kE5CntHot);
 }
 bool encode5_has_top(bool dropout, bool long_tokens) { return !dropout && !long_tokens; }
-static encode5_fn pick_encode5(bool dropout, bool cold, int ppl, bool long_tokens, int compact, bool lean, bool step_ok, bool count, bool top) {
+#ifdef TGX_E5_SEQ_ALL
+constexpr bool kE5SeqHot2 = TGX_E5_SEQ_ALL != 0, kE5SeqHot3 = TGX_E5_SEQ_ALL != 0, kE5SeqHot4 = TGX_E5_SEQ_ALL != 0;
+constexpr bool kE5SeqCold2 = TGX_E5_SEQ_ALL != 0, kE5SeqCold3 = TGX_E5_SEQ_ALL != 0, kE5SeqCold4 = TGX_E5_SEQ_ALL != 0;
+#else
+constexpr bool kE5SeqHot3 = true;
+constexpr bool kE5SeqHot2 = true;
+constexpr bool kE5SeqHot4 = true;
+constexpr bool kE5SeqCold3 = true;
+constexpr bool kE5SeqCold2 = false;
+constexpr bool kE5SeqCold4 = false;
+#endif
+bool encode5_has_seq(bool dropout, int ppl, bool long_tokens, bool top) { return top && encode5_has_top(dropout, long_tokens) && ppl >= 2 && ppl <= 4; }
+bool encode5_seq(bool dropout, bool cold, int ppl, bool long_tokens, bool top) {
+    if (!encode5_has_seq(dropout, ppl, long_tokens, top)) return false;
+    return cold ? (ppl == 2 ? kE5SeqCold2 : ppl == 3 ? kE5SeqCold3 : kE5SeqCold4) : (ppl == 2 ? kE5SeqHot2 : ppl == 3 ? kE5SeqHot3 : kE5SeqHot4);
+}
+static encode5_fn pick_encode5(bool dropout, bool cold, int ppl, bool long_tokens, int compact, bool lean, bool step_ok, bool count, bool top, bool seq) {
     if (long_tokens) {
         if (cold) return dropout ? encode5_kernel<true, true, 4, true> : encode5_kernel<false, true, 4, true>;
         return dropout ? encode5_kernel<true, false, 4, true> : encode5_kernel<false, false, 4, true>;
@@ -1234,34 +1268,37 @@
         if (ppl == 3) return encode5_kernel<true, false, 3, false>;
         return encode5_kernel<true, false, 4, false>;
     }
-#define TGX_E5K(C, PL, LN, CN, T) \
-    (compact == 4 ? encode5_kernel<false, C, PL, false, 4, LN, CN, T> : compact == 5 ? encode5_kernel<false, C, PL, false, 5, LN, CN, T> \
-     : compact == 6 ? encode5_kernel<false, C, PL, false, 6, LN, CN, T> : compact == 7 ? encode5_kernel<false, C, PL, false, 7, LN, CN, T> \
-     : compact == 8 ? encode5_kernel<false, C, PL, false, 8, LN, CN, T> : encode5_kernel<false, C, PL, false, 0, LN, CN, T>)
-#define TGX_E5L(LNH, LNC, LNC3, CN, T) \
+#define TGX_E5K(C, PL, LN, CN, T, S) \
+    (compact == 4 ? encode5_kernel<false, C, PL, false, 4, LN, CN, T, S> : compact == 5 ? encode5_kernel<false, C, PL, false, 5, LN, CN, T, S> \
+     : compact == 6 ? encode5_kernel<false, C, PL, false, 6, LN, CN, T, S> : compact == 7 ? encode5_kernel<false, C, PL, false, 7, LN, CN, T, S> \
+     : compact == 8 ? encode5_kernel<false, C, PL, false, 8, LN, CN, T, S> : encode5_kernel<false, C, PL, false, 0, LN, CN, T, S>)
+#define TGX_E5L(LNH, LNC, LNC3, CN, T, S) \
     if (cold) { \
         if (ppl == 1) return encode5_kernel<false, true, 1, false, 0, LNC, CN && kE5CntCold, T>; \
-        if (ppl == 2) return TGX_E5K(true, 2, LNC, CN && kE5CntCold, T); \
-        if (ppl == 3) return TGX_E5K(true, 3, LNC3, CN && kE5CntCold3, T); \
-        return TGX_E5K(true, 4, LNC, CN && kE5CntCold, T); \
+        if (ppl == 2) return TGX_E5K(true, 2, LNC, CN && kE5CntCold, T, S); \
+        if (ppl == 3) return TGX_E5K(true, 3, LNC3, CN && kE5CntCold3, T, S); \
+        return TGX_E5K(true, 4, LNC, CN && kE5CntCold, T, S); \
     } \
     if (ppl == 1) return encode5_kernel<false, false, 1, false, 0, LNH, CN && kE5CntHot, T>; \
-    if (ppl == 2) return TGX_E5K(false, 2, LNH, CN && kE5CntHot2, T); \
-    if (ppl == 3) return TGX_E5K(false, 3, LNH, CN && kE5CntHot, T); \
-    return TGX_E5K(false, 4, LNH, CN && kE5CntHot, T);
-#define TGX_E5C(CN, T) \
+    if (ppl == 2) return TGX_E5K(false, 2, LNH, CN && kE5CntHot2, T, S); \
+    if (ppl == 3) return TGX_E5K(false, 3, LNH, CN && kE5CntHot, T, S); \
+    return TGX_E5K(false, 4, LNH, CN && kE5CntHot, T, S);
+#define TGX_E5C(CN, T, S) \
     if (lean && step_ok) { \
-        TGX_E5L(kE5LeanHot, kE5LeanCold, kE5LeanCold3, CN, T) \
+        TGX_E5L(kE5LeanHot, kE5LeanCold, kE5LeanCold3, CN, T, S) \
     } \
     if (lean) {   \
-        TGX_E5L(lean_without_step(kE5LeanHot), lean_without_step(kE5LeanCold), lean_without_step(kE5LeanCold3), CN, T) \
+        TGX_E5L(lean_without_step(kE5LeanHot), lean_without_step(kE5LeanCold), lean_without_step(kE5LeanCold3), CN, T, S) \
     } \
-    TGX_E5L(0, 0, 0, CN, T)
+    TGX_E5L(0, 0, 0, CN, T, S)
 #define TGX_E5T(CN) \
+    if (top && seq) { \
+        TGX_E5C(CN, true, true) \
+    } \
     if (top) { \
-        TGX_E5C(CN, true) \
+        TGX_E5C(CN, true, false) \
     } \
-    TGX_E5C(CN, false)
+    TGX_E5C(CN, false, false)
     if (count) {
         TGX_E5T(true)
     }
@@ -1273,11 +1310,12 @@
 }
 
 
-hipError_t encode5_waves_per_simd(bool dropout, bool cold, int ppl, bool long_tokens, int compact, bool lean, bool step_ok, bool count, bool top, int* out) {
+hipError_t encode5_waves_per_simd(bool dropout, bool cold, int ppl, bool long_tokens, int compact, bool lean, bool step_ok, bool count, bool top, bool seq, int* out) {
     hipFuncAttributes attr;
     hipError_t e = hipFuncGetAttributes(&attr, reinterpret_cast<const void*>(pick_encode5(dropout, cold, ppl, long_tokens, compact, lean && encode5_has_lean(dropout, long_tokens), step_ok,
                                                                                              count && encode5_counts(dropout, cold, ppl, long_tokens),
-                                                                                             top && encode5_has_top(dropout, long_tokens))));
+                                                                                             top && encode5_has_top(dropout, long_tokens),
+                                                                                             seq && encode5_has_seq(dropout, ppl, long_tokens, top))));
     if (e != hipSuccess) return e;
     const int regs = (attr.numRegs + 7) & ~7;
     *out = regs > 0 ? (512 / regs > 8 ? 8 : 512 / regs) : 8;
@@ -1324,7 +1362,8 @@
 }
 
 hipError_t launch_encode5(const EncodeParams& p, Encode5Params q, bool cold, int ppl, bool long_tokens, int compact, bool lean, bool step_ok, bool count,
-                          bool top, int waves, uint32_t blocks, uint32_t min_lds, hipStream_t stream) {
+                          bool top, bool seq, int waves, uint32_t blocks, uint32_t min_lds, hipStream_t stream) {
+    if (seq && !encode5_has_seq(p.dropout > 0.0, ppl, long_tokens, top)) return hipErrorInvalidValue;
     if (top && (!encode5_has_top(p.dropout > 0.0, long_tokens) || !q.top)) return hipErrorInvalidValue;
     uint32_t lds = encode5_lds_layout(q.n_hot, long_tokens, waves, ppl, &q.list_off, &q.root_off, &q.idx_off, top);
     if (lds > 160u * 1024u || q.n_hot > q.n_values || (!cold && q.n_hot != q.n_values) || (long_tokens && ppl != 4) ||
@@ -1332,7 +1371,7 @@
         return hipErrorInvalidValue;
     lean = lean && encode5_has_lean(p.dropout > 0.0, long_tokens);
     if (count && !encode5_counts(p.dropout > 0.0, cold, ppl, long_tokens)) return hipErrorInvalidValue;
-    encode5_fn fn = pick_encode5(p.dropout > 0.0, cold, ppl, long_tokens, compact, lean, step_ok, count, top);
+    encode5_fn fn = pick_encode5(p.dropout > 0.0, cold, ppl, long_tokens, compact, lean, step_ok, count, top, seq);
     hipError_t e = hipFuncSetAttribute(reinterpret_cast<const void*>(fn), hipFuncAttributeMaxDynamicSharedMemorySize, 160 * 1024);
     if (e != hipSuccess) return e;
     if (lean && (e = lean_lds_check(reinterpret_cast<const void*>(fn))) != hipSuccess) return e;
diff --git a/tokengeex_amd/csrc/encode5_seq.h b/tokengeex_amd/csrc/encode5_seq.h
--- /dev/null
+++ b/tokengeex_amd/csrc/encode5_seq.h
@@ -0,0 +1,28 @@
+#pragma once
+#include <stdint.h>
+
+#include "encode5_layout.h"
+
+namespace tgx {
+
+constexpr uint32_t e5_seq_pos(int ppl, uint32_t l, uint32_t j) { return (uint32_t)ppl * l + j; }
+constexpr uint32_t e5_seq_base(uint32_t q, uint32_t r) { return (q >> 4) * kE5GroupBytes + r * kE5RowStride + (q & 15u) * 34u; }
+constexpr uint32_t e5_seq_entry(uint32_t base, uint32_t d) { return ((base + 32u * d) & 0x1E0u) | (base & ~0x1E0u); }
+
+constexpr int e5_seq_dwords(int ppl) { return (3 + ppl + 15 + 3) / 4; }
+constexpr int kE5SeqStream = 5;
+constexpr uint32_t e5_seq_alignbyte(uint32_t hi, uint32_t lo, uint32_t sh) {
+    return (uint32_t)((((uint64_t)hi << 32) | lo) >> (8u * (sh & 3u)));
+}
+constexpr uint32_t e5_seq_stream(const uint32_t* w, int n_dwords, int q, uint32_t sh) {
+    return e5_seq_alignbyte(q + 1 < n_dwords ? w[q + 1] : 0u, w[q], sh);
+}
+constexpr uint32_t e5_seq_walk_word(const uint32_t* v, uint32_t j, int q) { return j == 0u ? v[q] : e5_seq_alignbyte(v[q + 1], v[q], j); }
+constexpr uint32_t e5_seq_advance(int ppl) { return 16u * (uint32_t)ppl; }
+constexpr uint32_t e5_seq_reach(int ppl) { return e5_seq_advance(ppl) + (uint32_t)ppl * 15u + 4u * (uint32_t)e5_seq_dwords(ppl); }
+constexpr uint32_t kE5TextSlack = 256;
+static_assert(e5_seq_reach(2) <= kE5TextSlack && e5_seq_reach(3) <= kE5TextSlack && e5_seq_reach(4) <= kE5TextSlack,
+              "the SEQ windows and their prefetch stay inside the slack behind the text");
+static_assert(e5_seq_dwords(2) == 5 && e5_seq_dwords(3) == 6 && e5_seq_dwords(4) == 6, "five or six dwords per window");
+
+}
diff --git a/tokengeex_amd/csrc/encode_pass.cpp b/tokengeex_amd/csrc/encode_pass.cpp
--- a/tokengeex_amd/csrc/encode_pass.cpp
+++ b/tokengeex_amd/csrc/encode_pass.cpp
@@ -13,6 +13,7 @@
 #include <vector>
 
 #include "../../include/tgx.h"
+#include "../../include/tgx_encode_info.h"
 #include "api_internal.h"
 #include "device_internal.h"
 #include "pass_internal.h"
@@ -226,6 +227,7 @@
     bool lean, step_ok;
     bool in_place;
     bool top;
+    bool seq;
 };
 constexpr bool kE5Top14Waves = true;
 tgx_status choose_encode5(const tgx_model* m, const tgx_corpus* c, const tgx::EncodeParams& p, bool long_tokens, uint64_t n_long,
@@ -243,6 +245,12 @@
     const bool step_ok = m->lean_scores_ok;
     bool top = tgx::encode5_has_top(dropout > 0.0, long_tokens) && m->d_top8 != nullptr;
     if (const char* e = knob("TGX_E5_TOP")) top = top && atoi(e) != 0;
+    int seq_knob = -1;
+    if (const char* e = knob("TGX_E5_SEQ")) seq_knob = atoi(e) != 0 ? 1 : 0;
+    auto seq_for = [&](bool cold_, int ppl_) {
+        if (seq_knob == 0) return false;
+        return seq_knob == 1 ? tgx::encode5_has_seq(dropout > 0.0, ppl_, long_tokens, top) : tgx::encode5_seq(dropout > 0.0, cold_, ppl_, long_tokens, top);
+    };
     const uint32_t lds_cu = 160u * 1024u;
     tgx::IdsInPlaceQuery iq{};
     iq.rows5 = true;
@@ -256,7 +264,7 @@
     const bool want_count = have_result && tgx::ids_in_place(iq);
     {
         int ps4 = 0;
-        HIP_TRY(tgx::encode5_waves_per_simd(dropout > 0.0, false, 4, long_tokens, compact, lean, step_ok, want_count, top, &ps4));
+        HIP_TRY(tgx::encode5_waves_per_simd(dropout > 0.0, false, 4, long_tokens, compact, lean, step_ok, want_count, top, seq_for(false, 4), &ps4));
         hot_waves = std::min(16, ps4 * 4);
         const int least = long_tokens ? 12 : 13;
         while (hot_waves >= least && m->n_values > tgx::encode5_max_hot(long_tokens, hot_waves, 4, lds_cu, top)) hot_waves--;
@@ -298,12 +306,12 @@
     const uint32_t budget = 160u * 1024u / (uint32_t)bpc;
     bool cold = false;
     int per_simd = 0;
-    HIP_TRY(tgx::encode5_waves_per_simd(dropout > 0.0, false, ppl, long_tokens, compact, lean, step_ok, want_count, top, &per_simd));
+    HIP_TRY(tgx::encode5_waves_per_simd(dropout > 0.0, false, ppl, long_tokens, compact, lean, step_ok, want_count, top, seq_for(false, ppl), &per_simd));
     int waves = std::min(16, (per_simd / bpc) * 4);
     if ((ppl == 4 || ppl == 3) && bpc == 1 && hot_waves > 0) waves = std::min(waves, hot_waves);
     if (m->n_values > tgx::encode5_max_hot(long_tokens, waves, ppl, budget, top)) {
         cold = true;
-        HIP_TRY(tgx::encode5_waves_per_simd(dropout > 0.0, true, ppl, long_tokens, compact, lean, step_ok, want_count, top, &per_simd));
+        HIP_TRY(tgx::encode5_waves_per_simd(dropout > 0.0, true, ppl, long_tokens, compact, lean, step_ok, want_count, top, seq_for(true, ppl), &per_simd));
         waves = std::min(16, (per_simd / bpc) * 4);
     }
     if (balance_waves > 0 && ppl == 4 && bpc == 1) waves = std::min(waves, balance_waves);
@@ -318,7 +326,7 @@
     const uint64_t rows_per_block = 4 * (uint64_t)waves;
     const uint32_t blocks5 = (uint32_t)std::max<uint64_t>(
         1, std::min<uint64_t>((rest_n + rows_per_block - 1) / rows_per_block, (uint64_t)cus5 * bpc));
-    *out = Encode5Geometry{ppl, bpc, waves, per_simd, cold, n_hot, blocks5, compact, lean, step_ok, in_place, top};
+    *out = Encode5Geometry{ppl, bpc, waves, per_simd, cold, n_hot, blocks5, compact, lean, step_ok, in_place, top, seq_for(cold, ppl)};
     return TGX_OK;
 }
 
@@ -358,6 +366,7 @@
     if ((st = choose_encode5(m, c, p, long_tokens, n_long, corun_cus, r != nullptr, &g)) != TGX_OK) return st;
     m->last_n_hot = g.n_hot;
     m->last_encode_top = g.top && c->n_samples - n_long != 0;
+    m->last_encode_seq = g.seq && c->n_samples - n_long != 0;
     if (!g.in_place) {
         if ((st = ensure_scratch(c, true)) != TGX_OK) return st;
         p.tmp = c->d_tmp;
@@ -417,7 +426,7 @@
             p.redo_list = c->d_counts;
             HIP_TRY(hipMemsetAsync(&m->d_ctrl->encode_redo, 0x00, 8, m->stream));
         }
-        const hipError_t le = tgx::launch_encode5(p, q, g.cold, g.ppl, long_tokens, g.compact, g.lean, g.step_ok, g.in_place, g.top, g.waves, g.blocks5, corun_cus && n_long ? 84u * 1024u : 0u, m->stream);
+        const hipError_t le = tgx::launch_encode5(p, q, g.cold, g.ppl, long_tokens, g.compact, g.lean, g.step_ok, g.in_place, g.top, g.seq, g.waves, g.blocks5, corun_cus && n_long ? 84u * 1024u : 0u, m->stream);
         if (le != hipSuccess) return fail(TGX_ERR_DEVICE, "encode5 launch failed: %s", hipGetErrorString(le));
     }
     bool joined = false, joined_slot = false;
@@ -575,6 +584,7 @@
                 m->flat.table.size(), p.root_base, m->n_values);
     m->last_lean_items = 0;
     m->last_encode_top = false;
+    m->last_encode_seq = false;
     if (use5) return encode_rows5(m, c, p, long_tokens, pass, r);
     if ((st = ensure_scratch(c, true)) != TGX_OK) return st;
     p.tmp = c->d_tmp;
@@ -970,5 +980,6 @@
 uint32_t tgx_encode_corun_timeouts(const tgx_model* m) { return m ? m->corun_wait_timeouts : 0; }
 uint32_t tgx_last_encode_hot_values(const tgx_model* m) { return m ? m->last_n_hot : 0u; }
 int tgx_last_encode_top_table(const tgx_model* m) { return m && m->last_encode_top ? 1 : 0; }
+int tgx_last_encode_seq_walks(const tgx_model* m) { return m && m->last_encode_seq ? 1 : 0; }
 uint32_t tgx_last_encode_lean_items(const tgx_model* m) { return m ? m->last_lean_items : 0u; }
 int tgx_last_encode_ids_in_place(const tgx_model* m) { return (m && m->last_ids_in_place) ? 1 : 0; }
diff --git a/tokengeex_amd/csrc/kernels.h b/tokengeex_amd/csrc/kernels.h
--- a/tokengeex_amd/csrc/kernels.h
+++ b/tokengeex_amd/csrc/kernels.h
@@ -275,7 +275,9 @@
 int encode6_lean_items();
 bool encode5_counts(bool dropout, bool cold, int ppl, bool long_tokens);
 bool encode5_has_top(bool dropout, bool long_tokens);
-hipError_t encode5_waves_per_simd(bool dropout, bool cold, int ppl, bool long_tokens, int compact, bool lean, bool step_ok, bool count, bool top, int* out);
+bool encode5_seq(bool dropout, bool cold, int ppl, bool long_tokens, bool top);
+bool encode5_has_seq(bool dropout, int ppl, bool long_tokens, bool top);
+hipError_t encode5_waves_per_simd(bool dropout, bool cold, int ppl, bool long_tokens, int compact, bool lean, bool step_ok, bool count, bool top, bool seq, int* out);
 uint32_t encode6_lds_layout(uint32_t n_hot, uint32_t pool, uint32_t* root_off, uint32_t* ctrl_off, uint32_t* ring_off);
 uint32_t encode6_max_hot(uint32_t budget, uint32_t pool);
 uint32_t encode6_pool_total(uint32_t pool);
@@ -283,7 +285,7 @@
 hipError_t launch_estep5_fwd(const struct Estep4Params& p, Encode5Params q, bool cold, int ppl, int waves, uint32_t blocks, hipStream_t stream);
 hipError_t launch_encode6(const EncodeParams& p, Encode5Params q, bool cold, bool lean, uint32_t blocks, hipStream_t stream);
 hipError_t launch_encode5(const EncodeParams& p, Encode5Params q, bool cold, int ppl, bool long_tokens, int compact, bool lean, bool step_ok, bool count,
-                          bool top, int waves, uint32_t blocks, uint32_t min_lds, hipStream_t stream);
+                          bool top, bool seq, int waves, uint32_t blocks, uint32_t min_lds, hipStream_t stream);
 hipError_t launch_encode2(const EncodeParams& p, uint32_t num_cus, bool permuted, hipStream_t stream);
 hipError_t launch_trace32(const EncodeParams& p, uint32_t blocks, bool permuted, hipStream_t stream);
 hipError_t launch_encode4l(const EncodeParams& p, uint32_t num_cus, hipStream_t stream);
```

New measurement: 75820, median of 6. About the same (+0.2%).
